# BharathMasetty/DPG-SLAM

Hardware: AMD Instinct MI355X
Metric: ICP edges/sec + ms/GN-iter on 5k-node/20k-edge synthetic graph, 1->8 GPU (higher is better)
Workload: dtype fp32 (ICP) + fp64 (GN)

## Files before the change

dpg-slam_amd/csrc/dpg_chol.h:

```cpp
#ifndef DPG_CHOL_H
#define DPG_CHOL_H

#include <stdint.h>

#include <vector>

struct dpg_chol_opts {
    int32_t max_supernode_cols = 64;
    double relax_fraction = 0.3;
    int32_t order = 0;
    int32_t merge_single = 0;
    int32_t fused = 1;
    int32_t solve_stage = -1;
    int32_t solve_maxseg = -1;
    int32_t solve_dinv = 0;
    int32_t solve_inv_cols = 0;
};

struct dpg_chol_sym {
    int64_t n = 0;
    int32_t ns = 0;
    int32_t n_levels = 0;
    int32_t max_front = 0;
    double flops = 0.0;
    std::vector<int32_t> perm, pos;
    std::vector<int32_t> sn_c0;
    std::vector<int32_t> sn_of;
    std::vector<int64_t> sn_rows_ptr;
    std::vector<int32_t> sn_rows;
    std::vector<int32_t> sn_parent;
    std::vector<int32_t> sn_level;
    std::vector<int32_t> level_ptr;
    std::vector<int32_t> level_list;
    std::vector<int64_t> child_ptr;
    std::vector<int32_t> child_list;
    std::vector<int32_t> relmap;
    std::vector<int64_t> front_off;
};

int dpg_chol_symbolic(int64_t n, const int32_t* pair_lo, const int32_t* pair_hi, int64_t n_pairs,
                      const dpg_chol_opts* opts, dpg_chol_sym* S);
int dpg_chol_order(int64_t n, const int32_t* pair_lo, const int32_t* pair_hi, int64_t n_pairs,
                   std::vector<int32_t>& perm, std::vector<std::vector<int32_t>>& pat, bool md = false);
int dpg_chol_order_nd(int64_t n, const int32_t* pair_lo, const int32_t* pair_hi, int64_t n_pairs, int32_t leaf,
                      std::vector<int32_t>& perm, std::vector<std::vector<int32_t>>& pat);
int dpg_chol_order_nd_sep(int64_t n, const int32_t* pair_lo, const int32_t* pair_hi, int64_t n_pairs, int32_t leaf,
                          int32_t starts, int32_t bal, int32_t score, bool cover, std::vector<int32_t>& perm,
                          std::vector<std::vector<int32_t>>& pat, bool par = false, int32_t refine = 0);
int dpg_chol_nd_refine(int64_t n, const int32_t* pair_lo, const int32_t* pair_hi, int64_t n_pairs, int32_t bal,
                       int32_t score, int32_t refine, std::vector<int32_t>& side);
int dpg_chol_sym_from_patterns(int64_t n, const std::vector<int32_t>& perm, const std::vector<std::vector<int32_t>>& pat,
                               const dpg_chol_opts* opts, dpg_chol_sym* S);
double dpg_chol_critical_path_us(const dpg_chol_sym& S);
int dpg_chol_sym_from_csr(int64_t n, const int32_t* perm, const int64_t* cp, const int32_t* prow,
                          const dpg_chol_opts* opts, dpg_chol_sym* S);

struct dpg_chol_incsym {
    int64_t n = 0, words = 0;
    std::vector<int32_t> perm, pos;
    std::vector<uint64_t> bits;
    int64_t swords = 0;
    std::vector<uint64_t> summ;
    std::vector<int32_t> parent;
    int64_t nnz = 0;
    std::vector<int64_t> cp;
    std::vector<int32_t> rows, rows_tmp;
    std::vector<std::pair<int32_t, int32_t>> added;
};
int dpg_incsym_reset(dpg_chol_incsym* I, int64_t n, const int32_t* pair_lo, const int32_t* pair_hi, int64_t n_pairs,
                     const dpg_chol_opts* opts = nullptr);
int dpg_incsym_order(int64_t n, const int32_t* pair_lo, const int32_t* pair_hi, int64_t n_pairs,
                     std::vector<int32_t>& perm, std::vector<std::vector<int32_t>>& pat,
                     const dpg_chol_opts* opts = nullptr, bool concurrent = false);
void dpg_incsym_init(dpg_chol_incsym* I, int64_t n, std::vector<int32_t>& perm, std::vector<std::vector<int32_t>>& pat);
void dpg_incsym_append(dpg_chol_incsym* I, int64_t k);
int64_t dpg_incsym_add_edge(dpg_chol_incsym* I, int32_t a, int32_t b);
int dpg_incsym_derive(dpg_chol_incsym* I, const dpg_chol_opts* opts, dpg_chol_sym* S);


int dpg_chol_create_sym(void** h, int64_t n, const int32_t* pair_lo, const int32_t* pair_hi, int64_t n_pairs,
                        dpg_chol_sym* S, const dpg_chol_opts* opts = nullptr);
int dpg_chol_create_sym_plan(void** h, int64_t n, const int32_t* pair_lo, const int32_t* pair_hi, int64_t n_pairs,
                             dpg_chol_sym* S, const dpg_chol_opts* opts = nullptr);
int dpg_chol_create_sym_upload(void** h);
int dpg_chol_plan_blocks(void** h, int64_t n, const int32_t* pos, const int32_t* perm, const int32_t* pair_lo,
                         const int32_t* pair_hi, int64_t n_pairs);
void dpg_chol_blocks_invalidate(void* h);
void dpg_chol_build_times(void* h, double out[2]);
int dpg_chol_fused(void* h);
int dpg_chol_plan_host(int64_t n, const int32_t* pair_lo, const int32_t* pair_hi, int64_t n_pairs,
                       const dpg_chol_sym* S, const dpg_chol_opts* opts, double* ms);

#endif
```

dpg-slam_amd/csrc/dpg_chol.hip:

```cpp
#include "dpg_chol_dev.h"

using namespace dpg_chol;

namespace {
void take_sym(CholDev* c, dpg_chol_sym* S) {
    c->has_factor = false;
    if (c->track && c->sym_is_fac) {
        std::swap(c->fac_sym, c->sym);
        c->fac_G.swap(c->plan.cur_G);
        c->sym_is_fac = false;
    }
    std::swap(c->sym, *S);
}

int chol_upload(CholDev* c) {
    const dpg_chol_sym& S = c->sym;
    const CholPlan& H = c->plan;
    const int64_t n = H.n;
    ++c->build_gen;
    c->has_factor = false;
    auto al = [](size_t b) { return (b + 255) & ~size_t(255); };
    struct Piece { void** d; const void* h; size_t bytes; };
    Piece pieces[24];
    int np = 0;
// ... 16 lines not shown
    add(&c->segs, H.segs);
    add(&c->dblocks, H.dblocks);
    add(&c->inv_tasks, H.inv_t);
    if (!H.fused) {
        add(&c->asm_tasks, H.asm_t);
        add(&c->asm_child, H.asm_c);
        add(&c->panel_tasks, H.panel_t);
        add(&c->upd_tasks, H.upd_t);
    }
    size_t total = 0;
    for (int i = 0; i < np; ++i) total += al(std::max<size_t>(pieces[i].bytes, 1));
    if (c->stage.reserve_amortised(total) || c->arena.reserve_amortised(total)) return DPG_ERR_HIP;
    size_t off = 0;
    for (int i = 0; i < np; ++i) {
        if (pieces[i].bytes) memcpy(c->stage.p + off, pieces[i].h, pieces[i].bytes);
        *pieces[i].d = c->arena.p + off;
        off += al(std::max<size_t>(pieces[i].bytes, 1));
    }
    int rc = hipMemcpyAsync(c->arena.p, c->stage.p, total, hipMemcpyHostToDevice, nullptr) != hipSuccess;
    const size_t cap0[3] = {c->fronts.cap, c->acc.cap, c->ysol.cap};
    rc |= c->sync.reserve_amortised(H.sync_bytes / sizeof(int32_t));
    rc |= c->fronts.reserve_amortised((size_t)S.front_off[(size_t)S.ns]);
    rc |= c->acc.reserve_amortised((size_t)H.acc_total);
    rc |= c->ysol.reserve_amortised((size_t)(3 * n));
    if (rc || cap0[0] != c->fronts.cap || cap0[1] != c->acc.cap || cap0[2] != c->ysol.cap) c->fac_valid = false;
    rc |= c->xsol.reserve_amortised((size_t)(3 * n));
    rc |= c->status.reserve_amortised(1);
    rc |= c->dinv.reserve_amortised((size_t)(3 * n) * kSB);
    rc |= c->linv.reserve_amortised((size_t)std::max<int64_t>(H.linv_total, 1));
    if (!rc) rc |= hipMemsetAsync(c->status.p, 0, sizeof(int32_t), nullptr) != hipSuccess;
    rc |= hipStreamSynchronize(nullptr) != hipSuccess;
    return rc ? DPG_ERR_HIP : DPG_OK;
}

int chol_build_plan(CholDev* c, int64_t n, const int32_t* pair_lo, const int32_t* pair_hi, int64_t n_pairs) {
    const double t_b0 = now_ms();
    const int rc = dpg_chol_plan_build(c->plan, c->sym, c->opts, c->track, n, pair_lo, pair_hi, n_pairs);
    c->t_build[0] = now_ms() - t_b0;
    return rc;
}
int chol_build_upload(CholDev* c) {
    const double t_b1 = now_ms();
    const int rc = chol_upload(c);
    c->t_build[1] = now_ms() - t_b1;
    return rc;
}
int chol_build(CholDev* c, int64_t n, const int32_t* pair_lo, const int32_t* pair_hi, int64_t n_pairs) {
    const int rc = chol_build_plan(c, n, pair_lo, pair_hi, n_pairs);
    return rc ? rc : chol_build_upload(c);
}

CholDev* chol_take(void** h, dpg_chol_sym* S, const dpg_chol_opts* opts) {
    CholDev* c = *h ? reinterpret_cast<CholDev*>(*h) : new CholDev();
    if (opts) c->opts = *opts;
    take_sym(c, S);
    return c;
}
int chol_built(void** h, CholDev* c, int rc) {
    if (rc) dpg_chol_destroy(c);
    *h = rc ? nullptr : c;
    return rc;
}
}

extern "C" void dpg_chol_destroy(void* h) {
    CholDev* c = reinterpret_cast<CholDev*>(h);
    if (!c) return;
    if (c->aux.s) (void)hipStreamSynchronize(c->aux.s);
    delete c;
}

extern "C" int dpg_chol_create(void** out, int64_t n, const int32_t* pair_lo, const int32_t* pair_hi,
                               int64_t n_pairs, const dpg_chol_opts* opts) {
    *out = nullptr;
    CholDev* c = new CholDev();
    if (opts) c->opts = *opts;
    if (dpg_chol_symbolic(n, pair_lo, pair_hi, n_pairs, &c->opts, &c->sym)) {
        delete c;
        return DPG_ERR_NUMERIC;
    }
    return chol_built(out, c, chol_build(c, n, pair_lo, pair_hi, n_pairs));
}

int dpg_chol_create_sym(void** h, int64_t n, const int32_t* pair_lo, const int32_t* pair_hi, int64_t n_pairs,
                        dpg_chol_sym* S, const dpg_chol_opts* opts) {
    CholDev* c = chol_take(h, S, opts);
    return chol_built(h, c, chol_build(c, n, pair_lo, pair_hi, n_pairs));
}

int dpg_chol_create_sym_plan(void** h, int64_t n, const int32_t* pair_lo, const int32_t* pair_hi, int64_t n_pairs,
                             dpg_chol_sym* S, const dpg_chol_opts* opts) {
    CholDev* c = chol_take(h, S, opts);
    return chol_built(h, c, chol_build_plan(c, n, pair_lo, pair_hi, n_pairs));
}
int dpg_chol_create_sym_upload(void** h) {
    CholDev* c = reinterpret_cast<CholDev*>(*h);
    return c ? chol_built(h, c, chol_build_upload(c)) : DPG_ERR_STATE;
}
int dpg_chol_plan_blocks(void** h, int64_t n, const int32_t* pos, const int32_t* perm, const int32_t* pair_lo,
                         const int32_t* pair_hi, int64_t n_pairs) {
    if (!h || n <= 0 || !pos || !perm || n_pairs < 0 || (n_pairs > 0 && (!pair_lo || !pair_hi))) return DPG_ERR_ARG;
    CholDev* c = *h ? reinterpret_cast<CholDev*>(*h) : new CholDev();
    *h = c;
    dpg_chol_plan_prebucket(c->plan, n, pos, perm, pair_lo, pair_hi, n_pairs);
    return DPG_OK;
}
void dpg_chol_blocks_invalidate(void* h) {
    if (h) reinterpret_cast<CholDev*>(h)->plan.blocks_ready = false;
}
int dpg_chol_fused(void* h) { return h && reinterpret_cast<const CholDev*>(h)->plan.fused ? 1 : 0; }

void dpg_chol_build_times(void* h, double out[2]) {
    const CholDev* c = reinterpret_cast<const CholDev*>(h);
    out[0] = c ? c->t_build[0] : 0.0;
    out[1] = c ? c->t_build[1] : 0.0;
}

static void note_factored(CholDev* c, int64_t refactored, int64_t kept, int64_t moved, int64_t pick_ns = 0) {
    c->pstats[0] = refactored;
    c->pstats[1] = kept;
    c->pstats[2] = moved;
    c->pstats[3] = pick_ns;
    c->has_factor = true;
    if (!c->track) return;
    c->fac_valid = true;
    c->fac_ptr = c->fronts.p;
    c->fac_ysol = c->ysol.p;
    c->fac_acc = c->acc.p;
    c->sym_is_fac = true;
    c->fac_db = c->plan.fused_db;
}

extern "C" int dpg_chol_solve(void* h, const double* hb, void* stream) {
    CholDev* c = reinterpret_cast<CholDev*>(h);
    const CholPlan& P = c->plan;
    note_factored(c, c->sym.ns, 0, 0);
    hipStream_t st = reinterpret_cast<hipStream_t>(stream);
    if (hipMemsetAsync(c->status.p, 0, sizeof(int32_t), st) != hipSuccess) return DPG_ERR_HIP;
    if (P.fused) {
        if (hipMemsetAsync(c->sync.p, 0, P.sync_bytes, st) != hipSuccess) return DPG_ERR_HIP;
        launch_factor(c, st, hb, nullptr, nullptr);
    } else {
        launch_levels(c, st, hb);
        if (hipMemsetAsync(c->sync.p, 0, P.sync_bytes, st) != hipSuccess) return DPG_ERR_HIP;
    }
    const double* di = launch_inv_diag(c, st);
    if (!P.fused) launch_forward(c, st, hb, di, nullptr, nullptr);
    launch_backward(c, st, di, nullptr, nullptr, nullptr, nullptr);
    c->inv_valid = c->keep_inv && P.n_inv_tasks > 0;
    if (c->inv_valid) launch_inv(c, st, nullptr);
    return hipGetLastError() == hipSuccess ? DPG_OK : DPG_ERR_HIP;
}

extern "C" void dpg_chol_track_factor(void* h, int on) {
    CholDev* c = reinterpret_cast<CholDev*>(h);
    if (!c || c->track == (on != 0)) return;
    c->track = on != 0;
    c->fac_valid = false;
    c->sym_is_fac = false;
    c->plan.cur_G.clear();
}
extern "C" void dpg_chol_forget_factor(void* h) {
    if (!h) return;
    reinterpret_cast<CholDev*>(h)->fac_valid = false;
    reinterpret_cast<CholDev*>(h)->has_factor = false;
}
extern "C" void dpg_chol_partial_stats(void* h, int64_t out[4]) {
    const CholDev* c = reinterpret_cast<const CholDev*>(h);
    for (int k = 0; k < 4; ++k) out[k] = c ? c->pstats[k] : 0;
}

extern "C" int dpg_chol_solve_partial(void* h, const double* hb, const int32_t* dirty_nodes, int64_t n_dirty,
                                      void* stream) {
    CholDev* c = reinterpret_cast<CholDev*>(h);
    const dpg_chol_sym& S = c->sym;
    const dpg_chol_sym& O = c->fac_sym;
    const CholPlan& P = c->plan;
    const bool usable = c->track && c->fac_valid && !c->sym_is_fac && c->fac_ptr == c->fronts.p &&
                        c->fac_ysol == c->ysol.p && c->fac_acc == c->acc.p && P.fused &&
                        !(P.use_dinv && P.n_dblocks > 0) && c->fac_db == P.fused_db && O.ns > 0 && O.n <= S.n &&
                        (int64_t)c->fac_G.size() == (int64_t)O.ns && (int64_t)P.cur_G.size() == (int64_t)S.ns &&
                        std::equal(O.perm.begin(), O.perm.end(), S.perm.begin());
    const double t_pick = now_ms();
    PartialPick& K = c->pick;
    if (!usable || !dpg_chol_plan_partial(K, S, O, P.cur_G, c->fac_G, dirty_nodes, n_dirty)) return dpg_chol_solve(h, hb, stream);
    const int32_t ns = S.ns;
    const int64_t nruns = (int64_t)K.runs.size() / 4;
    hipStream_t st = reinterpret_cast<hipStream_t>(stream);
    const size_t keep_bytes = ((size_t)ns + 15) & ~size_t(15);
    const size_t run_bytes = sizeof(int64_t) * 4 * (size_t)nruns;
    const size_t bytes = keep_bytes + 2 * run_bytes;
    if (c->pev_set && hipEventSynchronize(c->pev.e) != hipSuccess) return DPG_ERR_HIP;
    if (c->pstage.reserve_amortised(bytes) || c->dpart.reserve_amortised(bytes) ||
        (K.moved > 0 && c->scratch.reserve_amortised((size_t)K.moved)))
        return DPG_ERR_HIP;
    memcpy(c->pstage.p, K.keep.data(), (size_t)ns);
    int64_t* gat = reinterpret_cast<int64_t*>(c->pstage.p + keep_bytes);
    int64_t* sca = gat + 4 * nruns;
    for (int64_t r = 0, off = 0; r < nruns; ++r) {
        const int64_t* q = K.runs.data() + 4 * r;
        const int64_t g4[4] = {q[0], off, q[2], q[3]}, s4[4] = {off, q[1], q[2], q[3]};
        std::copy(g4, g4 + 4, gat + 4 * r);
        std::copy(s4, s4 + 4, sca + 4 * r);
        off += q[2];
    }
    if (c->pev.ensure(hipEventDisableTiming)) return DPG_ERR_HIP;
    if (hipMemcpyAsync(c->dpart.p, c->pstage.p, bytes, hipMemcpyHostToDevice, st) != hipSuccess ||
        hipEventRecord(c->pev.e, st) != hipSuccess)
        return DPG_ERR_HIP;
    c->pev_set = true;
    const uint8_t* keep_dev = reinterpret_cast<const uint8_t*>(c->dpart.p);
    const int64_t* gat_dev = reinterpret_cast<const int64_t*>(c->dpart.p + keep_bytes);
    launch_copy_runs(c, st, gat_dev, gat_dev + 4 * nruns, nruns, K.max_run);
    if (hipMemsetAsync(c->status.p, 0, sizeof(int32_t), st) != hipSuccess ||
        hipMemsetAsync(c->sync.p, 0, P.sync_bytes, st) != hipSuccess)
        return DPG_ERR_HIP;
    launch_factor(c, st, hb, nullptr, keep_dev);
    launch_backward(c, st, nullptr, nullptr, nullptr, nullptr, nullptr);
    note_factored(c, ns - K.kept, K.kept, K.moved, (int64_t)((now_ms() - t_pick) * 1e6));
    c->inv_valid = false;
    return hipGetLastError() == hipSuccess ? DPG_OK : DPG_ERR_HIP;
}

extern "C" int dpg_chol_resolve(void* h, const double* hb, void* stream) {
    CholDev* c = reinterpret_cast<CholDev*>(h);
    hipStream_t st = reinterpret_cast<hipStream_t>(stream);
    if (hipMemsetAsync(c->sync.p, 0, c->plan.sync_bytes, st) != hipSuccess) return DPG_ERR_HIP;
    const double* di = c->plan.use_dinv ? c->dinv.p : nullptr;
    const double* li = c->inv_valid ? c->linv.p : nullptr;
    launch_forward(c, st, hb, di, nullptr, li);
    launch_backward(c, st, di, nullptr, nullptr, nullptr, li);
    return hipGetLastError() == hipSuccess ? DPG_OK : DPG_ERR_HIP;
}

extern "C" int dpg_chol_gated_ok(void* h) {
    const CholDev* c = reinterpret_cast<const CholDev*>(h);
    return c && c->plan.fused && !(c->plan.use_dinv && c->plan.n_dblocks > 0) ? 1 : 0;
}

extern "C" void dpg_chol_sync_dev(void* h, int32_t** sync, int64_t* n_words) {
    CholDev* c = reinterpret_cast<CholDev*>(h);
    *sync = c->sync.p;
    *n_words = (int64_t)(c->plan.sync_bytes / sizeof(int32_t));
}

extern "C" int dpg_chol_solve_gated(void* h, const double* hb, const int32_t* gate, int prezeroed, double* X,
                                    double* max_out, void* stream) {
    CholDev* c = reinterpret_cast<CholDev*>(h);
    if (!dpg_chol_gated_ok(h)) return DPG_ERR_STATE;
    c->fac_valid = false;
    c->has_factor = true;
    hipStream_t st = reinterpret_cast<hipStream_t>(stream);
    if (!prezeroed && (hipMemsetAsync(c->status.p, 0, sizeof(int32_t), st) != hipSuccess ||
                       hipMemsetAsync(c->sync.p, 0, c->plan.sync_bytes, st) != hipSuccess))
        return DPG_ERR_HIP;
    const bool inv = c->plan.n_inv_tasks > 0;
    if (inv) {
        if (!c->aux.s) {
            if (hipStreamCreateWithFlags(&c->aux.s, hipStreamNonBlocking) != hipSuccess ||
                c->ev_fac.ensure(hipEventDisableTiming) || c->ev_inv[0].ensure(hipEventDisableTiming) ||
                c->ev_inv[1].ensure(hipEventDisableTiming) || hipEventRecord(c->ev_inv[0].e, c->aux.s) != hipSuccess ||
                hipEventRecord(c->ev_inv[1].e, c->aux.s) != hipSuccess)
                return DPG_ERR_HIP;
        }
        if (hipStreamWaitEvent(st, c->ev_inv[c->inv_par ^ 1].e, 0) != hipSuccess) return DPG_ERR_HIP;
    }
    launch_factor(c, st, hb, gate, nullptr);
    if (inv) {
        if (hipEventRecord(c->ev_fac.e, st) != hipSuccess || hipStreamWaitEvent(c->aux.s, c->ev_fac.e, 0) != hipSuccess)
            return DPG_ERR_HIP;
        launch_inv(c, c->aux.s, gate);
        if (hipEventRecord(c->ev_inv[c->inv_par].e, c->aux.s) != hipSuccess) return DPG_ERR_HIP;
        c->inv_par ^= 1;
    }
    launch_forward(c, st, hb, nullptr, gate, c->linv.p);
    launch_backward(c, st, nullptr, gate, X, max_out, c->linv.p);
    return hipGetLastError() == hipSuccess ? DPG_OK : DPG_ERR_HIP;
}

extern "C" void dpg_chol_keep_inverse(void* h, int on) {
    if (h) reinterpret_cast<CholDev*>(h)->keep_inv = on != 0;
}

extern "C" int dpg_chol_join_aux(void* h, void* stream) {
    CholDev* c = reinterpret_cast<CholDev*>(h);
    if (!c || !c->aux.s) return DPG_OK;
    return hipStreamWaitEvent(reinterpret_cast<hipStream_t>(stream), c->ev_inv[c->inv_par ^ 1].e, 0) == hipSuccess ? DPG_OK
                                                                                                       : DPG_ERR_HIP;
}

extern "C" const int32_t* dpg_chol_pos_dev(void* h) { return reinterpret_cast<CholDev*>(h)->pos; }
extern "C" const double* dpg_chol_x_dev(void* h) { return reinterpret_cast<CholDev*>(h)->xsol.p; }
extern "C" const int32_t* dpg_chol_status_dev(void* h) { return reinterpret_cast<CholDev*>(h)->status.p; }
extern "C" void dpg_chol_stats(void* h, double out[6]) {
    const dpg_chol_sym& S = reinterpret_cast<CholDev*>(h)->sym;
    out[0] = S.ns;
    out[1] = S.n_levels;
    out[2] = S.max_front;
    out[3] = S.flops;
    out[4] = (double)S.front_off[(size_t)S.ns] * 8.0;
    out[5] = (double)S.n;
}

#ifdef DPG_CHOL_TIMING
extern "C" void dpg_chol_tree(void* h, int32_t* parent, int32_t* m3, int32_t* k3) {
    const dpg_chol_sym& S = reinterpret_cast<CholDev*>(h)->sym;
    for (int32_t s = 0; s < S.ns; ++s) {
        parent[s] = S.sn_parent[(size_t)s];
        k3[s] = 3 * (S.sn_c0[(size_t)s + 1] - S.sn_c0[(size_t)s]);
        m3[s] = k3[s] + 3 * (int32_t)(S.sn_rows_ptr[(size_t)s + 1] - S.sn_rows_ptr[(size_t)s]);
    }
}
#endif
```

dpg-slam_amd/csrc/dpg_chol_factor.hip:

```cpp
#include "dpg_chol_dev.h"

using namespace dpg_chol;

#define FT_MARK(s, k) DPG_STAMP(threadIdx.x == 0 && (s) < 16384, g_front[(s) * 8 + (k)])
#define PN_MARK(s, p, k) DPG_STAMP(threadIdx.x == 0 && (s) < 16384 && (p) < 16, g_panel[((s) * 16 + (p)) * 8 + (k)])
#ifdef DPG_CHOL_TIMING
__device__ unsigned long long g_front[16384 * 8], g_panel[16384 * 16 * 8];
extern "C" int dpg_chol_front_dump(unsigned long long* out, int n) {
    return hipMemcpyFromSymbol(out, HIP_SYMBOL(g_front), sizeof(unsigned long long) * 8 * (size_t)n) == hipSuccess ? 0 : -1;
}
extern "C" int dpg_chol_panel_dump(unsigned long long* out, int n) {
    return hipMemcpyFromSymbol(out, HIP_SYMBOL(g_panel), sizeof(unsigned long long) * 16 * 8 * (size_t)n) == hipSuccess ? 0 : -1;
}
#endif

namespace {
constexpr int kPF = (kSmall * (kSmall + 1) / 2 + kFT - 1) / kFT;
constexpr int kPFL = 4;

__device__ __forceinline__ void tri_ij(int e, int n, int& i, int& j) {
    const float b = 2.0f * (float)n + 1.0f;
    int jj = (int)((b - sqrtf(b * b - 8.0f * (float)e)) * 0.5f);
    jj = max(0, min(jj, n - 1));
    while (jj > 0 && jj * n - jj * (jj - 1) / 2 > e) --jj;
    while (jj + 1 < n && (jj + 1) * n - (jj + 1) * jj / 2 <= e) ++jj;
    j = jj;
    i = jj + e - (jj * n - jj * (jj - 1) / 2);
}

__device__ __forceinline__ void small_front(int s, const SnDev& S, int32_t* sync, int32_t* status, const SnDev* __restrict__ sns,
                            const OEnt* __restrict__ omap, const int32_t* __restrict__ relmap,
                            const int32_t* __restrict__ child_list, const double* __restrict__ hb,
                            const double* __restrict__ g, const int32_t* __restrict__ perm, double* fronts,
                            double* __restrict__ ysol, double* acc, double* sm) {
    const int tid = threadIdx.x;
    const int k3 = 3 * S.k, r3 = 3 * S.r, m3 = k3 + r3;
    double* F = fronts + S.front_off;
    double* A = sm;
    double* bv = A + m3 * m3;
    ChMeta* chm = reinterpret_cast<ChMeta*>(bv + m3);
    int32_t* crm = reinterpret_cast<int32_t*>(chm + kMaxCh);
    const int nch = S.nchild;
    for (int e = tid; e < m3 * m3; e += kFT) A[e] = 0.0;
    for (int t = tid; t < m3; t += kFT) bv[t] = t < k3 ? -g[3 * perm[S.c0 + t / 3] + t % 3] : 0.0;
    if (tid < nch) {
        const SnDev C = sns[child_list[S.child_off + tid]];
        chm[tid] = ChMeta{C.front_off, C.acc_off, C.rows_off, C.k, C.r};
        for (int q = 0; q < C.r; ++q) crm[tid * (kSmall / 3) + q] = relmap[C.rows_off + q];
    }
    __syncthreads();
    for (int q = tid; q < S.omap_n * 9; q += kFT) {
        const OEnt o = omap[S.omap_off + q / 9];
        const int ii = (q % 9) / 3, jj = q % 3;
        const int row = 3 * o.a + ii, col = 3 * o.b + jj;
        if (row < col) continue;
        const double* B = hb + 9 * (int64_t)o.u;
        A[col * m3 + row] = o.tr ? B[3 * jj + ii] : B[3 * ii + jj];
    }
    if (nch > 0) {
        if (tid == 0) wait_geq_sc1(sync + s, S.need, status);
        asm volatile("s_waitcnt vmcnt(0)" ::: "memory");
    }
    __syncthreads();
    FT_MARK(s, 1);
    auto load_child = [&](int ci, double (&v)[kPF], double& va) {
        const ChMeta C = chm[ci];
        const int n = 3 * C.r, tri = n * (n + 1) / 2, m3c = 3 * (C.k + C.r), k3c = 3 * C.k;
        double* Fc = fronts + C.front_off + (int64_t)k3c * m3c + k3c;
#pragma unroll
        for (int q = 0; q < kPF; ++q) {
            const int e = tid + kFT * q;
            v[q] = 0.0;
            if (e < tri) {
                int i, j;
                tri_ij(e, n, i, j);
                v[q] = ld_agent(Fc + (int64_t)j * m3c + i);
            }
        }
        va = tid < n ? ld_agent(acc + C.acc_off + tid) : 0.0;
    };
    auto add_child = [&](int ci, const double (&v)[kPF], double va) {
        const ChMeta C = chm[ci];
        const int n = 3 * C.r, tri = n * (n + 1) / 2;
        const int32_t* rm = crm + ci * (kSmall / 3);
#pragma unroll
        for (int q = 0; q < kPF; ++q) {
            const int e = tid + kFT * q;
            if (e < tri) {
                int i, j;
                tri_ij(e, n, i, j);
                const int pj = 3 * rm[j / 3] + j % 3, pi = 3 * rm[i / 3] + i % 3;
                A[pj * m3 + pi] += v[q];
            }
        }
        if (tid < n) bv[3 * rm[tid / 3] + tid % 3] -= va;
    };
    if (nch > 0) {
        double va_[kPF], vb_[kPF], aa = 0.0, ab = 0.0;
        load_child(0, va_, aa);
        for (int ci = 0; ci < nch; ci += 2) {
            if (ci + 1 < nch) load_child(ci + 1, vb_, ab);
            add_child(ci, va_, aa);
            __syncthreads();
            if (ci + 1 < nch) {
                if (ci + 2 < nch) load_child(ci + 2, va_, aa);
                add_child(ci + 1, vb_, ab);
                __syncthreads();
            }
        }
    }
    FT_MARK(s, 2);
    bool bad = false;
    for (int c0 = 0; c0 < k3; c0 += 3) {
        const double* C0 = A + c0 * m3;
        const double* C1 = C0 + m3;
        const double* C2 = C1 + m3;
        double d00 = C0[c0], d10 = C0[c0 + 1], d20 = C0[c0 + 2], d11 = C1[c0 + 1], d21 = C1[c0 + 2], d22 = C2[c0 + 2];
        if (!(d00 > 0.0)) { bad = true; d00 = 1.0; }
        const double i00 = rsqrt_nr(d00), l00 = d00 * i00;
        const double l10 = d10 * i00, l20 = d20 * i00;
        double e11 = d11 - l10 * l10;
        if (!(e11 > 0.0)) { bad = true; e11 = 1.0; }
        const double i11 = rsqrt_nr(e11), l11 = e11 * i11;
        const double l21 = (d21 - l20 * l10) * i11;
        double e22 = d22 - l20 * l20 - l21 * l21;
        if (!(e22 > 0.0)) { bad = true; e22 = 1.0; }
        const double i22 = rsqrt_nr(e22), l22 = e22 * i22;
        const double y0 = bv[c0] * i00;
        const double y1 = (bv[c0 + 1] - l10 * y0) * i11;
        const double y2 = (bv[c0 + 2] - l20 * y0 - l21 * y1) * i22;
        for (int i = c0 + 3 + tid; i < m3; i += kFT) {
            const double x0 = C0[i] * i00;
            const double x1 = (C1[i] - x0 * l10) * i11;
            const double x2 = (C2[i] - x0 * l20 - x1 * l21) * i22;
            A[c0 * m3 + i] = x0;
            A[(c0 + 1) * m3 + i] = x1;
            A[(c0 + 2) * m3 + i] = x2;
            bv[i] -= x0 * y0 + x1 * y1 + x2 * y2;
        }
        __syncthreads();
        if (tid == 0) {
            A[c0 * m3 + c0] = l00; A[c0 * m3 + c0 + 1] = l10; A[c0 * m3 + c0 + 2] = l20;
            A[(c0 + 1) * m3 + c0 + 1] = l11; A[(c0 + 1) * m3 + c0 + 2] = l21; A[(c0 + 2) * m3 + c0 + 2] = l22;
            bv[c0] = y0; bv[c0 + 1] = y1; bv[c0 + 2] = y2;
        }
        const int b0 = c0 + 3, nr = m3 - b0;
        for (int e = tid; e < nr * nr; e += kFT) {
            const int l = b0 + e / nr, i = b0 + e % nr;
            if (i < l) continue;
            double v = A[l * m3 + i];
            v = fma(-C0[i], C0[l], v);
            v = fma(-C1[i], C1[l], v);
            v = fma(-C2[i], C2[l], v);
            A[l * m3 + i] = v;
        }
        __syncthreads();
    }
    if (bad && tid == 0) atomicExch(status, 1);
    FT_MARK(s, 3);
    for (int e = tid; e < k3 * m3; e += kFT) {
        const int j = e / m3, i = e - j * m3;
        if (i >= j) F[(int64_t)j * m3 + i] = A[e];
    }
    for (int t = tid; t < k3; t += kFT) ysol[3 * (int64_t)S.c0 + t] = bv[t];
    if (S.parent >= 0) {
        const auto rs = front_rsrc(F, m3);
        const int npc = (r3 + 2) >> 1;
        for (int e = tid; e < r3 * npc; e += kFT) {
            const int jj = e / npc, k = e - jj * npc, j = k3 + jj;
            const uint32_t a = (uint32_t)(j * m3 + k3);
            const int i0 = 2 * k - (int)(a & 1u);
            if (i0 + 1 < jj || i0 >= r3) continue;
            const double* Aj = A + j * m3 + k3;
            st2_sc1(rs, (a & ~1u) + 2u * k, i0 >= jj ? Aj[i0] : 0.0, i0 + 1 < r3 ? Aj[i0 + 1] : 0.0);
        }
        for (int t = tid; t < r3; t += kFT) st_agent(acc + S.acc_off + t, -bv[k3 + t]);
    }
    asm volatile("s_waitcnt vmcnt(0)" ::: "memory");
    __syncthreads();
    FT_MARK(s, 4);
    if (tid == 0 && S.parent >= 0)
        __hip_atomic_fetch_add(sync + S.parent, 1, __ATOMIC_RELAXED, __HIP_MEMORY_SCOPE_AGENT);
}

struct Tiles {
    int k3, m3, np, nt;
    __device__ int c0(int t) const { return t < np ? kFNB * t : k3 + kFNB * (t - np); }
    __device__ int c1(int t) const { return t < np ? min(kFNB * t + kFNB, k3) : min(k3 + kFNB * (t - np + 1), m3); }
};

struct PanelFrame {
    int m3, j0, w, R, off, Rp, npc;
    __device__ __forceinline__ PanelFrame(const Tiles& T, int q)
        : m3(T.m3), j0(kFNB * q), w(min(kFNB, T.k3 - j0)), R(T.m3 - j0), off((4 - (w & 3)) & 3), Rp(fused_rp(R, off)),
          npc((R + 2) >> 1) {}
    struct Pair { int c, i0; uint32_t addr; };
    __device__ __forceinline__ Pair pair(int e) const {
        const int c = e / npc, k = e - c * npc;
        const uint32_t a = (uint32_t)((j0 + c) * m3 + j0);
        return Pair{c, 2 * k - (int)(a & 1u), (a & ~1u) + 2u * k};
    }
};

__device__ void factor_lds(int q, int s, const Tiles& T, double* P, double* scr, bool& bad) {
    const int tid = threadIdx.x, lane = tid & 63, wave = __builtin_amdgcn_readfirstlane(tid >> 6);
    const PanelFrame f(T, q);
    const int w = f.w, R = f.R, off = f.off, Rp = f.Rp;
    double* Lt = scr;
    double* rdg = Lt + kFNB * kFNB;
    int* flg = reinterpret_cast<int*>(rdg + 8 * (kFNB / 3));
    PN_MARK(s, q, 5);
    {
        const int i = lane, cv = 3 * wave, ep = q + 1;
        if (cv < w) {
            double col[3];
#pragma unroll
            for (int r = 0; r < 3; ++r) {
                const int c = cv + r;
                col[r] = (i < w && i >= c) ? P[c * Rp + off + i] : 0.0;
            }
            for (int st = 0; st < wave; ++st) {
                while (__builtin_amdgcn_readfirstlane(__hip_atomic_load(flg + st, __ATOMIC_RELAXED, __HIP_MEMORY_SCOPE_WORKGROUP)) < ep)
                    __builtin_amdgcn_s_sleep(0);
                __builtin_amdgcn_fence(__ATOMIC_ACQUIRE, "workgroup");
                const int c0 = 3 * st;
                const int ii = i < kFNB ? i : 0;
                const double x0 = Lt[c0 * kFNB + ii], x1 = Lt[(c0 + 1) * kFNB + ii], x2 = Lt[(c0 + 2) * kFNB + ii];
#pragma unroll
                for (int r = 0; r < 3; ++r) {
                    const int c = cv + r;
                    const double y0 = Lt[c0 * kFNB + c], y1 = Lt[(c0 + 1) * kFNB + c], y2 = Lt[(c0 + 2) * kFNB + c];
                    const double v = fma(-x2, y2, fma(-x1, y1, fma(-x0, y0, col[r])));
                    col[r] = (i >= c && i < w) ? v : col[r];
                }
            }
            const double d00 = rdlane(col[0], cv), d10 = rdlane(col[0], cv + 1), d20 = rdlane(col[0], cv + 2);
            const double d11 = rdlane(col[1], cv + 1), d21 = rdlane(col[1], cv + 2), d22 = rdlane(col[2], cv + 2);
            const Chol3 L = chol3(d00, d10, d11, d20, d21, d22, bad);
            double x0 = col[0] * L.m00;
            double x1 = fma(col[0], L.m10, col[1] * L.m11);
            double x2 = fma(col[0], L.m20, fma(col[1], L.m21, col[2] * L.m22));
            if (i == cv) { x0 = L.l00; x1 = 0.0; x2 = 0.0; }
            else if (i == cv + 1) { x0 = L.l10; x1 = L.l11; x2 = 0.0; }
            else if (i == cv + 2) { x0 = L.l20; x1 = L.l21; x2 = L.l22; }
            if (i < kFNB) {
                Lt[cv * kFNB + i] = (i >= cv && i < w) ? x0 : 0.0;
                Lt[(cv + 1) * kFNB + i] = (i >= cv + 1 && i < w) ? x1 : 0.0;
                Lt[(cv + 2) * kFNB + i] = (i >= cv + 2 && i < w) ? x2 : 0.0;
            }
            if (i == 0) {
                double* mi = rdg + 2 * cv;
                mi[0] = L.m00; mi[1] = L.m10; mi[2] = L.m11; mi[3] = L.m20; mi[4] = L.m21; mi[5] = L.m22;
            }
            __builtin_amdgcn_fence(__ATOMIC_RELEASE, "workgroup");
            if (i == 0) __hip_atomic_store(flg + wave, ep, __ATOMIC_RELAXED, __HIP_MEMORY_SCOPE_WORKGROUP);
        } else if (cv < kFNB) {
            for (int r = 0; r < 3; ++r)
                if (i < kFNB) Lt[(cv + r) * kFNB + i] = 0.0;
        }
    }
    __syncthreads();
    PN_MARK(s, q, 6);
    for (int i = w + tid; i < R; i += kFT) {
        double a[kFNB];
#pragma unroll
        for (int c = 0; c < kFNB; ++c) a[c] = c < w ? P[c * Rp + off + i] : 0.0;
#pragma unroll
        for (int b = 0; b < kFNB; b += 3) {
            if (b < w) {
                const double* mi = rdg + 2 * b;
                const double x0 = a[b] * mi[0];
                const double x1 = fma(a[b], mi[1], a[b + 1] * mi[2]);
                const double x2 = fma(a[b], mi[3], fma(a[b + 1], mi[4], a[b + 2] * mi[5]));
                a[b] = x0; a[b + 1] = x1; a[b + 2] = x2;
#pragma unroll
                for (int cc = b + 3; cc < kFNB; ++cc)
                    a[cc] = fma(-x2, Lt[(b + 2) * kFNB + cc], fma(-x1, Lt[(b + 1) * kFNB + cc], fma(-x0, Lt[b * kFNB + cc], a[cc])));
            }
        }
#pragma unroll
        for (int c = 0; c < kFNB; ++c)
            if (c < w) P[c * Rp + off + i] = a[c];
    }
    __syncthreads();
    PN_MARK(s, q, 7);
    for (int e = tid; e < w * w; e += kFT) {
        const int c = e / w, r = e - c * w;
        if (r >= c) P[c * Rp + off + r] = Lt[c * kFNB + r];
    }
    __syncthreads();
    PN_MARK(s, q, 3);
}

__device__ void publish_panel(int q, int s, const Tiles& T, double* F, const double* P, int32_t* pflag) {
    const int tid = threadIdx.x;
    const PanelFrame f(T, q);
    const int R = f.R;
    const auto rs = front_rsrc(F, T.m3);
    for (int e = tid; e < f.w * f.npc; e += kFT) {
        const PanelFrame::Pair pr = f.pair(e);
        const int c = pr.c, i0 = pr.i0;
        if (i0 + 1 < c || i0 >= R) continue;
        const double* pc = P + c * f.Rp + f.off;
        st2_sc1(rs, pr.addr, i0 >= c ? pc[i0] : 0.0, i0 + 1 < R ? pc[i0 + 1] : 0.0);
    }
    asm volatile("s_waitcnt vmcnt(0)" ::: "memory");
    __syncthreads();
    if (tid == 0) __hip_atomic_store(pflag + s, q + 1, __ATOMIC_RELAXED, __HIP_MEMORY_SCOPE_AGENT);
    PN_MARK(s, q, 4);
}

template <bool SC1>
__device__ void load_panel(int p, const Tiles& T, double* F, double* P) {
    const int tid = threadIdx.x;
    const PanelFrame f(T, p);
    const int j0 = f.j0, w = f.w, R = f.R, off = f.off, Rp = f.Rp;
    if (SC1) {
        const auto rs = front_rsrc(F, T.m3);
        const int tot = w * f.npc;
        constexpr int kB2 = 8;
        for (int e0 = 0; e0 < tot; e0 += kFT * kB2) {
            double2 v[kB2];
#pragma unroll
            for (int q = 0; q < kB2; ++q) {
                const int e = e0 + tid + kFT * q;
                const PanelFrame::Pair pr = f.pair(e);
                v[q] = make_double2(0.0, 0.0);
                if (e < tot && pr.i0 < R && pr.i0 + 1 >= pr.c) v[q] = ld2_sc1(rs, pr.addr);
            }
#pragma unroll
            for (int q = 0; q < kB2; ++q) {
                const int e = e0 + tid + kFT * q;
                const PanelFrame::Pair pr = f.pair(e);
                const int c = pr.c, i0 = pr.i0;
                if (e < tot) {
                    double* pc = P + c * Rp + off;
                    if (i0 >= 0 && i0 < R) pc[i0] = i0 >= c ? v[q].x : 0.0;
                    if (i0 + 1 < R) pc[i0 + 1] = i0 + 1 >= c ? v[q].y : 0.0;
                }
            }
        }
        return;
    }
    constexpr int kB = 16;
    for (int e0 = 0; e0 < w * R; e0 += kFT * kB) {
        double v[kB];
#pragma unroll
        for (int q = 0; q < kB; ++q) {
            const int e = e0 + tid + kFT * q;
            const int c = e / R, i = e - c * R;
            double* a = F + (uint32_t)((j0 + c) * T.m3 + j0 + i);
            v[q] = (e < w * R && i >= c) ? (SC1 ? ld_agent(a) : *a) : 0.0;
        }
#pragma unroll
        for (int q = 0; q < kB; ++q) {
            const int e = e0 + tid + kFT * q;
            const int c = e / R, i = e - c * R;
            if (e < w * R) P[c * Rp + off + i] = v[q];
        }
    }
}

template <bool WT, bool SC1 = false>
__device__ void update_tile(int t, int p, const Tiles& T, double* F, const double* P) {
    const int tid = threadIdx.x;
    const PanelFrame f(T, p);
    const int m3 = f.m3, j0 = f.j0, w = f.w, R = f.R, off = f.off, Rp = f.Rp;
    const int l0 = T.c0(t) - j0, l1 = T.c1(t) - j0;
    const int g0 = ((l0 + off) & ~3) - off;
    const int ncg = (l1 - g0 + 3) >> 2, nrg = (R - g0 + 3) >> 2;
    for (int q = tid; q < nrg * ncg; q += kFT) {
        const int ib = g0 + 4 * (q % nrg), lb = g0 + 4 * (q / nrg);
        if (ib + 3 < lb) continue;
        double ac[4][4];
#pragma unroll
        for (int a = 0; a < 4; ++a)
#pragma unroll
            for (int b = 0; b < 4; ++b) ac[a][b] = 0.0;
#pragma unroll 1
        for (int c = 0; c < w; ++c) {
            const double2* pc = reinterpret_cast<const double2*>(P + c * Rp);
            const double2 i01 = pc[(off + ib) >> 1], i23 = pc[((off + ib) >> 1) + 1];
            const double2 l01 = pc[(off + lb) >> 1], l23 = pc[((off + lb) >> 1) + 1];
            const double vi[4] = {i01.x, i01.y, i23.x, i23.y};
            const double vl[4] = {l01.x, l01.y, l23.x, l23.y};
#pragma unroll
            for (int a = 0; a < 4; ++a)
#pragma unroll
                for (int b = 0; b < 4; ++b) ac[a][b] = fma(vi[a], vl[b], ac[a][b]);
        }
#pragma unroll
        for (int b = 0; b < 4; ++b) {
            const uint32_t o = (uint32_t)((j0 + min(max(lb + b, l0), l1 - 1)) * m3 + j0);
#pragma unroll
            for (int a = 0; a < 4; ++a) {
                double* src = F + o + (uint32_t)min(ib + a, R - 1);
                ac[a][b] = (SC1 ? ld_agent(src) : *src) - ac[a][b];
            }
        }
#pragma unroll
        for (int b = 0; b < 4; ++b) {
            const int l = lb + b;
            const uint32_t o = (uint32_t)((j0 + l) * m3 + j0);
#pragma unroll
            for (int a = 0; a < 4; ++a) {
                const int i = ib + a;
                if (l >= l0 && l < l1 && i < R && i >= l) {
                    if (WT) st_agent(F + o + (uint32_t)i, ac[a][b]);
                    else F[o + (uint32_t)i] = ac[a][b];
                }
            }
        }
    }
}

__device__ void update_next_lds(int p, const Tiles& T, const double* Pc, double* Pn) {
    const int tid = threadIdx.x;
    const int j0 = kFNB * p, R = T.m3 - j0, Rp = fused_rp(R, 0);
    const int j1 = j0 + kFNB, w1 = min(kFNB, T.k3 - j1), R1 = R - kFNB;
    const int off1 = (4 - (w1 & 3)) & 3, Rp1 = fused_rp(R1, off1);
    const int ncg = (w1 + 3) >> 2, nrg = (R1 + 3) >> 2;
    for (int q = tid; q < nrg * ncg; q += kFT) {
        const int ib = 4 * (q % nrg), lb = 4 * (q / nrg);
        if (ib + 3 < lb) continue;
        double ac[4][4];
#pragma unroll
        for (int a = 0; a < 4; ++a)
#pragma unroll
            for (int b = 0; b < 4; ++b) ac[a][b] = 0.0;
#pragma unroll 2
        for (int c = 0; c < kFNB; ++c) {
            const double2* pc = reinterpret_cast<const double2*>(Pc + c * Rp + kFNB);
            const double2 i01 = pc[ib >> 1], i23 = pc[(ib >> 1) + 1];
            const double2 l01 = pc[lb >> 1], l23 = pc[(lb >> 1) + 1];
            const double vi[4] = {i01.x, i01.y, i23.x, i23.y};
            const double vl[4] = {l01.x, l01.y, l23.x, l23.y};
#pragma unroll
            for (int a = 0; a < 4; ++a)
#pragma unroll
                for (int b = 0; b < 4; ++b) ac[a][b] = fma(vi[a], vl[b], ac[a][b]);
        }
#pragma unroll
        for (int b = 0; b < 4; ++b) {
            const int l = lb + b;
#pragma unroll
            for (int a = 0; a < 4; ++a) {
                const int i = ib + a;
                if (l < w1 && i < R1 && i >= l) Pn[l * Rp1 + off1 + i] -= ac[a][b];
            }
        }
    }
}

__device__ void rhs_panel(int p, const Tiles& T, const double* P, double* bv) {
    const int tid = threadIdx.x, lane = tid & 63, wave = tid >> 6;
    const PanelFrame f(T, p);
    const int j0 = f.j0, w = f.w, R = f.R, off = f.off, Rp = f.Rp;
    if (wave == 0) {
        double bl = lane < w ? bv[j0 + lane] : 0.0;
        for (int c = 0; c < w; ++c) {
            const double yc = __shfl(bl, c, 64) / P[c * Rp + off + c];
            if (lane == c) bl = yc;
            else if (lane > c && lane < w) bl = fma(-P[c * Rp + off + lane], yc, bl);
        }
        if (lane < w) bv[j0 + lane] = bl;
    }
    __syncthreads();
    for (int i = w + tid; i < R; i += kFT) {
        double sacc = 0.0;
        for (int c = 0; c < w; ++c) sacc = fma(P[c * Rp + off + i], bv[j0 + c], sacc);
        bv[j0 + i] -= sacc;
    }
    __syncthreads();
}

__device__ __forceinline__ int tile_owner(int t, int G) { return t == 0 || G == 1 ? 0 : 1 + (t - 1) % (G - 1); }

__device__ __forceinline__ void large_front(int s, int mem, const SnDev& S, int32_t* sync, int32_t* pflag,
                            int32_t* tready, int32_t* status,
                            const SnDev* __restrict__ sns, const OEnt* __restrict__ omap,
                            const int32_t* __restrict__ relmap, const int32_t* __restrict__ child_list,
                            const FTask* __restrict__ ftasks, const FChild* __restrict__ fchild,
                            const double* __restrict__ hb, const double* __restrict__ g,
                            const int32_t* __restrict__ perm, double* fronts, double* __restrict__ ysol,
                            double* acc, double* sm, int db) {
    const int tid = threadIdx.x;
    const int k3 = 3 * S.k, r3 = 3 * S.r, m3 = k3 + r3, G = S.G;
    double* F = fronts + S.front_off;
    Tiles T{k3, m3, (k3 + kFNB - 1) / kFNB, 0};
    T.nt = T.np + (r3 + kFNB - 1) / kFNB;
    int32_t* trdy = tready + S.ftask;
    const bool has_b = mem == tile_owner(T.nt - 1, G);
    const int t_first = mem, t_step = mem == 0 ? T.nt : G - 1;
    double* bv = sm;
    double* scr = bv + ((m3 + 1) & ~1);
    double* PA = scr + kFScr;
    double* PB = db ? PA + (size_t)kFNB * fused_rp(m3, 3) : PA;
    if (has_b)
        for (int t = tid; t < m3; t += kFT) bv[t] = t < k3 ? -g[3 * perm[S.c0 + t / 3] + t % 3] : 0.0;
    bool waited = S.need == 0;
    for (int t = t_first; t < T.nt; t += t_step) {
        const FTask tk = ftasks[S.ftask + t];
        const int cs = T.c0(t), nc = T.c1(t) - cs;
        double* Tl = PA;
        for (int e = tid; e < nc * m3; e += kFT) Tl[e] = 0.0;
        __syncthreads();
        for (int q = tid; q < (tk.om_e - tk.om_b) * 9; q += kFT) {
            const OEnt o = omap[tk.om_b + q / 9];
            const int ii = (q % 9) / 3, jj = q % 3;
            const int row = 3 * o.a + ii, col = 3 * o.b + jj;
            if (col < cs || col >= cs + nc || row < col) continue;
            const double* B = hb + 9 * (int64_t)o.u;
            Tl[(col - cs) * m3 + row] = o.tr ? B[3 * jj + ii] : B[3 * ii + jj];
        }
        if (!waited) {
            if (tid == 0) wait_geq_sc1(sync + s, S.need, status);
            asm volatile("s_waitcnt vmcnt(0)" ::: "memory");
            waited = true;
            FT_MARK(s, 1);
        }
        for (int cq = 0; cq < tk.ch_cnt; ++cq) {
            __syncthreads();
            const FChild C = fchild[tk.ch_off + cq];
            const int n = 3 * C.r, m3c = 3 * (C.k + C.r), k3c = 3 * C.k, nj = C.jb - C.ja;
            const auto rs = front_rsrc(fronts + C.front_off, m3c);
            const int32_t* rm = relmap + C.rows_off;
            const int npc = (n + 2) >> 1, tot = nj * npc;
            for (int e0 = 0; e0 < tot; e0 += kFT * kPFL) {
                double2 v[kPFL];
                int d0[kPFL], d1[kPFL];
#pragma unroll
                for (int q = 0; q < kPFL; ++q) {
                    const int e = e0 + tid + kFT * q;
                    const int jj = e / npc, k = e - jj * npc, j = C.ja + jj;
                    const uint32_t a = (uint32_t)((k3c + j) * m3c + k3c);
                    const int i0 = 2 * k - (int)(a & 1u);
                    d0[q] = -1;
                    d1[q] = -1;
                    v[q] = make_double2(0.0, 0.0);
                    if (e < tot && i0 + 1 >= j && i0 < n) {
                        v[q] = ld2_sc1(rs, (a & ~1u) + 2u * k);
                        const int cj = (3 * rm[j / 3] + j % 3 - cs) * m3;
                        if (i0 >= j) d0[q] = cj + 3 * rm[i0 / 3] + i0 % 3;
                        if (i0 + 1 < n) d1[q] = cj + 3 * rm[(i0 + 1) / 3] + (i0 + 1) % 3;
                    }
                }
#pragma unroll
                for (int q = 0; q < kPFL; ++q) {
                    if (d0[q] >= 0) Tl[d0[q]] += v[q].x;
                    if (d1[q] >= 0) Tl[d1[q]] += v[q].y;
                }
            }
        }
        __syncthreads();
        if (t == 0 && mem == 0 && db) {
            const int off = (4 - (nc & 3)) & 3, Rp = fused_rp(m3, off);
            for (int e = tid; e < nc * m3; e += kFT) {
                const int c = e / m3, i = e - c * m3;
                PB[c * Rp + off + i] = i >= c ? Tl[e] : 0.0;
            }
            __syncthreads();
            continue;
        }
        const bool handoff = t == 1 && mem != 0;
        for (int e = tid; e < nc * m3; e += kFT) {
            const int col = cs + e / m3, row = e % m3;
            if (row >= col) {
                if (handoff) st_agent(F + (uint32_t)(col * m3 + row), Tl[e]);
                else F[(uint32_t)(col * m3 + row)] = Tl[e];
            }
        }
        if (handoff) asm volatile("s_waitcnt vmcnt(0)" ::: "memory");
        __syncthreads();
        if (handoff && tid == 0) __hip_atomic_store(trdy + 1, 1, __ATOMIC_RELAXED, __HIP_MEMORY_SCOPE_AGENT);
    }
    if (!waited) {
        if (tid == 0) wait_geq_sc1(sync + s, S.need, status);
        asm volatile("s_waitcnt vmcnt(0)" ::: "memory");
        __syncthreads();
    }
    if (has_b) {
        for (int ci = 0; ci < S.nchild; ++ci) {
            const SnDev C = sns[child_list[S.child_off + ci]];
            const int32_t* rm = relmap + C.rows_off;
            for (int t = tid; t < 3 * C.r; t += kFT) bv[3 * rm[t / 3] + t % 3] -= ld_agent(acc + C.acc_off + t);
            __syncthreads();
        }
    }
    FT_MARK(s, 2);

    bool bad = false;
    if (mem == 0) {
        double* cur = db ? PB : PA;
        if (tid < kFNB / 3) reinterpret_cast<int*>(scr + kFNB * kFNB + 8 * (kFNB / 3))[tid] = 0;
        if (!db) load_panel<false>(0, T, F, cur);
        __syncthreads();
        factor_lds(0, s, T, cur, scr, bad);
        publish_panel(0, s, T, F, cur, pflag);
        for (int p = 0; p < T.np; ++p) {
            double* nxt = cur == PA ? PB : PA;
            if (has_b && !db) rhs_panel(p, T, cur, bv);
            if (p + 1 < T.np) {
                const int t = p + 1;
                PN_MARK(s, t, 0);
                if (tile_owner(t, G) != 0) {
                    if (tid == 0) wait_geq_sc1(trdy + t, 1, status);
                    asm volatile("s_waitcnt vmcnt(0)" ::: "memory");
                    __syncthreads();
                }
                if (db) {
                    load_panel<true>(t, T, F, nxt);
                    __syncthreads();
                    PN_MARK(s, t, 1);
                    update_next_lds(p, T, cur, nxt);
                } else {
                    PN_MARK(s, t, 1);
                    update_tile<true, true>(t, p, T, F, cur);
                    asm volatile("s_waitcnt vmcnt(0)" ::: "memory");
                    __syncthreads();
                    load_panel<true>(t, T, F, nxt);
                }
                __syncthreads();
                PN_MARK(s, t, 2);
                factor_lds(t, s, T, nxt, scr, bad);
                publish_panel(t, s, T, F, nxt, pflag);
            }
            if (has_b && db) rhs_panel(p, T, cur, bv);
            cur = nxt;
        }
    } else {
        double* P = PA;
        for (int p = 0; p < T.np; ++p) {
            bool need = false;
            for (int t = t_first; t < T.nt; t += t_step) need |= t > p && !(t == p + 1 && t < T.np);
            if (!need && !has_b) break;
            if (tid == 0) wait_geq_sc1(pflag + s, p + 1, status);
            asm volatile("s_waitcnt vmcnt(0)" ::: "memory");
            __syncthreads();
            load_panel<true>(p, T, F, P);
            __syncthreads();
            const int tc = p + 2;
            const bool mine = tc < T.np && tile_owner(tc, G) == mem;
            if (mine) {
                update_tile<true>(tc, p, T, F, P);
                asm volatile("s_waitcnt vmcnt(0)" ::: "memory");
                __syncthreads();
                if (tid == 0) __hip_atomic_store(trdy + tc, 1, __ATOMIC_RELAXED, __HIP_MEMORY_SCOPE_AGENT);
            }
            const bool fin = p == T.np - 1 && S.parent >= 0;
            for (int t = t_first; t < T.nt; t += t_step)
                if (t > p && !(t == p + 1 && t < T.np) && !(mine && t == tc)) {
                    if (fin) update_tile<true>(t, p, T, F, P);
                    else update_tile<false>(t, p, T, F, P);
                }
            __syncthreads();
            if (has_b) rhs_panel(p, T, P, bv);
        }
    }
    if (bad && (tid & 63) == 0) atomicExch(status, 1);
    if (has_b) {
        for (int t = tid; t < k3; t += kFT) ysol[3 * (int64_t)S.c0 + t] = bv[t];
        if (S.parent >= 0)
            for (int t = tid; t < r3; t += kFT) st_agent(acc + S.acc_off + t, -bv[k3 + t]);
    }
    FT_MARK(s, 3);
    asm volatile("s_waitcnt vmcnt(0)" ::: "memory");
    __syncthreads();
    if (mem == 0) FT_MARK(s, 4);
    if (tid == 0 && S.parent >= 0)
        __hip_atomic_fetch_add(sync + S.parent, 1, __ATOMIC_RELAXED, __HIP_MEMORY_SCOPE_AGENT);
}

__global__ __launch_bounds__(kFT, 2) void chol_factor_dag(const int32_t* __restrict__ order, int32_t* sync,
                                                       int32_t* status, const SnDev* __restrict__ sns,
                                                       const OEnt* __restrict__ omap,
                                                       const int32_t* __restrict__ relmap,
                                                       const int32_t* __restrict__ child_list,
                                                       const FTask* __restrict__ ftasks,
                                                       const FChild* __restrict__ fchild,
                                                       const double* __restrict__ hb, const double* __restrict__ g,
                                                       const int32_t* __restrict__ perm, double* fronts,
                                                       double* __restrict__ ysol, double* acc, int ns, int db,
                                                       const int32_t* gate, const uint8_t* __restrict__ keep) {
    extern __shared__ __attribute__((aligned(16))) double smem_f[];
    double* sm = smem_f + 2;
    if (gate_off(gate, 1)) return;
    __builtin_amdgcn_s_setprio(2);
    const int code = claim_lds(order, sync, reinterpret_cast<int*>(smem_f));
    const int s = code >> 6, mem = code & 63;
    const SnDev S = sns[s];
    if (keep && keep[s]) {
        if (threadIdx.x == 0 && S.parent >= 0)
            __hip_atomic_fetch_add(sync + 1 + S.parent, 1, __ATOMIC_RELAXED, __HIP_MEMORY_SCOPE_AGENT);
        return;
    }
    if (mem == 0) FT_MARK(s, 0);
    if (S.G == 1 && 3 * (S.k + S.r) <= kSmall && S.nchild <= kMaxCh)
        small_front(s, S, sync + 1, status, sns, omap, relmap, child_list, hb, g, perm, fronts, ysol, acc, sm);
    else
        large_front(s, mem, S, sync + 1, sync + 1 + ns, sync + 2 + 3 * ns, status, sns, omap, relmap, child_list,
                    ftasks, fchild, hb, g, perm, fronts, ysol, acc, sm, db);
}

__global__ __launch_bounds__(256) void chol_copy_runs(const double* __restrict__ src0, const double* __restrict__ src1,
                                                      double* __restrict__ dst0, double* __restrict__ dst1,
                                                      const int64_t* __restrict__ runs) {
    const int64_t* r = runs + 4 * blockIdx.y;
    const int64_t s0 = r[0], d0 = r[1], n = r[2];
    const double* src = r[3] ? src1 : src0;
    double* dst = r[3] ? dst1 : dst0;
    for (int64_t i = (int64_t)blockIdx.x * blockDim.x + threadIdx.x; i < n; i += (int64_t)gridDim.x * blockDim.x)
        dst[d0 + i] = src[s0 + i];
}

}

void dpg_chol::launch_factor(CholDev* c, hipStream_t st, const double* hb, const int32_t* gate, const uint8_t* keep) {
    const CholPlan& P = c->plan;
    hipLaunchKernelGGL(chol_factor_dag, dim3((unsigned)P.n_tickets), dim3(kFT), P.lds_fused, st, c->order_fac, sync_forward(c),
                       c->status.p, c->sns, c->omap, c->relmap, c->child_list, c->ftasks, c->fchild, hb, hb + 9 * P.nnzb_upper,
                       c->perm, c->fronts.p, c->ysol.p, c->acc.p, c->sym.ns, P.fused_db ? 1 : 0, gate, keep);
}

void dpg_chol::launch_copy_runs(CholDev* c, hipStream_t st, const int64_t* gather, const int64_t* scatter, int64_t nruns,
                                int64_t max_run) {
    if (nruns == 0) return;
    const dim3 grid((unsigned)std::min<int64_t>(64, std::max<int64_t>(1, (max_run + 2047) / 2048)), (unsigned)nruns);
    hipLaunchKernelGGL(chol_copy_runs, grid, dim3(256), 0, st, c->fronts.p, c->acc.p, c->scratch.p, c->scratch.p, gather);
    hipLaunchKernelGGL(chol_copy_runs, grid, dim3(256), 0, st, c->scratch.p, c->scratch.p, c->fronts.p, c->acc.p, scatter);
}
```

dpg-slam_amd/csrc/dpg_ctx.hip:

```cpp

#include <stdarg.h>
#include <stdio.h>
#include <string.h>

#include <string>

#include "dpg_ctx.h"

namespace {
thread_local std::string g_err;
}

int fail(int code, const char* fmt, ...) {
    char buf[512];
    va_list ap;
    va_start(ap, fmt);
    vsnprintf(buf, sizeof(buf), fmt, ap);
    va_end(ap);
    g_err = buf;
    return code;
}

dpg_ctx* g_default_ctx = nullptr;

static dpg_ctx* no_ctx(int) { return nullptr; }

extern "C" {

const char* dpg_last_error(void) { return g_err.c_str(); }

int dpg_set_error(int code, const char* msg) { return fail(code, "%s", msg); }
const char* dpg_version(void) { return "dpg-mi355x 0.1 (gfx950)"; }

int dpg_shard_plan(const float* cost, int64_t ne, int32_t world, int32_t* owner, int64_t* dispatch, int64_t* counts) {
    if (ne < 0 || world < 1 || (ne > 0 && (!owner || !dispatch)) || !counts) return fail(DPG_ERR_ARG, "dpg_shard_plan: bad arguments");
    std::vector<std::vector<int64_t>> disp((size_t)world);
    if (cost) {
        std::vector<int64_t> ord((size_t)ne);
        for (int64_t e = 0; e < ne; ++e) ord[(size_t)e] = e;
        std::stable_sort(ord.begin(), ord.end(), [&](int64_t a, int64_t b) { return cost[a] > cost[b]; });
        std::vector<double> load((size_t)world, 0.0);
        for (int64_t e : ord) {
            int r = 0;
            for (int q = 1; q < world; ++q)
                if (load[(size_t)q] < load[(size_t)r]) r = q;
            owner[e] = r;
            load[(size_t)r] += cost[e];
            disp[(size_t)r].push_back(e);
        }
    } else {
        for (int64_t e = 0; e < ne; ++e) {
            owner[e] = (int32_t)(e % world);
            disp[(size_t)(e % world)].push_back(e);
        }
    }
    int64_t o = 0;
    for (int r = 0; r < world; ++r) {
        counts[r] = (int64_t)disp[(size_t)r].size();
        for (int64_t e : disp[(size_t)r]) dispatch[o++] = e;
    }
    return DPG_OK;
}

int dpg_shard_reassemble(const int32_t* owner, int64_t ne, int32_t world, int64_t slice, int64_t rec_bytes,
                         const void* gathered, void* out) {
    if (ne < 0 || world < 1 || slice < 0 || rec_bytes <= 0 || (ne > 0 && (!owner || !gathered || !out)))
        return fail(DPG_ERR_ARG, "dpg_shard_reassemble: bad arguments");
    std::vector<int64_t> pos((size_t)world, 0);
    const char* g = static_cast<const char*>(gathered);
    char* o = static_cast<char*>(out);
    for (int64_t e = 0; e < ne; ++e) {
        const int32_t r = owner[e];
        if (r < 0 || r >= world || pos[(size_t)r] >= slice) return fail(DPG_ERR_ARG, "dpg_shard_reassemble: edge %lld owner %d out of range", (long long)e, r);
        memcpy(o + e * rec_bytes, g + (r * slice + pos[(size_t)r]++) * rec_bytes, (size_t)rec_bytes);
    }
    return DPG_OK;
}

dpg_ctx* dpg_ctx_create(int device) {
    int n = 0;
    if (hipGetDeviceCount(&n) != hipSuccess || n <= 0) return no_ctx(fail(DPG_ERR_HIP, "no HIP device available"));
    if (device < 0 || device >= n) return no_ctx(fail(DPG_ERR_ARG, "device %d out of range (%d devices)", device, n));
    if (hipSetDevice(device) != hipSuccess) return no_ctx(fail(DPG_ERR_HIP, "hipSetDevice(%d) failed", device));
    dpg_ctx* c = new dpg_ctx();
    c->device = device;
    if (hipStreamCreateWithFlags(&c->own.s, hipStreamNonBlocking) != hipSuccess) {
        delete c;
        return no_ctx(fail(DPG_ERR_HIP, "hipStreamCreate failed"));
    }
    c->stream = c->own.s;
    if (hipStreamCreateWithFlags(&c->aux.s, hipStreamNonBlocking) != hipSuccess) c->aux.s = nullptr;
    for (auto& e : c->ev) (void)e.ensure(hipEventDefault);
    dpg_gn_params_default(&c->gp);
    return c;
}

dpg_ctx* dpg_ctx_create_multi(int32_t n_gpus, const int32_t* devices) {
    int n = 0;
    if (hipGetDeviceCount(&n) != hipSuccess || n <= 0) return no_ctx(fail(DPG_ERR_HIP, "no HIP device available"));
    if (n_gpus < 1 || n_gpus > n)
        return no_ctx(fail(DPG_ERR_ARG, "dpg_ctx_create_multi: %d GPUs asked, %d present", n_gpus, n));
    std::vector<int> dl((size_t)n_gpus);
    for (int k = 0; k < n_gpus; ++k) {
        dl[(size_t)k] = devices ? devices[k] : k;
        for (int j = 0; j < k; ++j)
            if (dl[(size_t)j] == dl[(size_t)k])
                return no_ctx(fail(DPG_ERR_ARG, "dpg_ctx_create_multi: device %d listed twice", dl[(size_t)k]));
    }
    dpg_ctx* c = dpg_ctx_create(dl[0]);
    if (!c) return nullptr;
    for (int k = 1; k < n_gpus; ++k) {
        dpg_ctx* q = dpg_ctx_create(dl[(size_t)k]);
        if (!q) {
            dpg_ctx_destroy(c);
            return nullptr;
        }
        q->rank = k;
        c->peers.push_back(q);
    }
    c->comms.assign((size_t)n_gpus, nullptr);
    const ncclResult_t r = ncclCommInitAll(c->comms.data(), n_gpus, dl.data());
    if (r != ncclSuccess) {
        c->comms.clear();
        dpg_ctx_destroy(c);
        return no_ctx(fail(DPG_ERR_HIP, "ncclCommInitAll over %d devices failed: %s", n_gpus, ncclGetErrorString(r)));
    }
    c->coll = kCollRccl;
    c->world = n_gpus;
    (void)hipSetDevice(c->device);
    return c;
}

dpg_ctx* dpg_ctx_create_virtual(int32_t k, int32_t device) {
    if (k < 1 || k > kMaxVirtual)
        return no_ctx(fail(DPG_ERR_ARG, "dpg_ctx_create_virtual: %d virtual devices (1 .. %d)", k, kMaxVirtual));
    dpg_ctx* c = dpg_ctx_create(device);
    if (!c) return nullptr;
    for (int r = 1; r < k; ++r) {
        dpg_ctx* q = dpg_ctx_create(device);
        if (!q) {
            dpg_ctx_destroy(c);
            return nullptr;
        }
        q->own.release();
        q->stream = c->stream;
        q->rank = r;
        c->peers.push_back(q);
    }
    c->coll = kCollVirtual;
    c->world = k;
    return c;
}

int dpg_nccl_unique_id(void* id_out) {
    if (!id_out) return fail(DPG_ERR_ARG, "dpg_nccl_unique_id: NULL");
    static_assert(sizeof(ncclUniqueId) == DPG_NCCL_ID_BYTES, "ncclUniqueId size");
    ncclUniqueId id;
    const ncclResult_t r = ncclGetUniqueId(&id);
    if (r != ncclSuccess) return fail(DPG_ERR_HIP, "ncclGetUniqueId failed: %s", ncclGetErrorString(r));
    memcpy(id_out, &id, sizeof(id));
    return DPG_OK;
}

dpg_ctx* dpg_ctx_create_rank(int32_t device, const void* nccl_id, int32_t rank, int32_t world) {
    if (!nccl_id || world < 1 || rank < 0 || rank >= world)
        return no_ctx(fail(DPG_ERR_ARG, "dpg_ctx_create_rank: rank %d of %d", rank, world));
    dpg_ctx* c = dpg_ctx_create(device);
    if (!c) return nullptr;
    ncclUniqueId id;
    memcpy(&id, nccl_id, sizeof(id));
    ncclComm_t comm = nullptr;
    const ncclResult_t r = ncclCommInitRank(&comm, world, id, rank);
    if (r != ncclSuccess) {
        dpg_ctx_destroy(c);
        return no_ctx(fail(DPG_ERR_HIP, "ncclCommInitRank(rank %d of %d) failed: %s", rank, world, ncclGetErrorString(r)));
    }
    c->comms.assign(1, comm);
    c->coll = kCollRccl;
    c->world = world;
    c->rank0 = rank;
    c->rank = rank;
    return c;
}

dpg_ctx* dpg_ctx_create_rank_ops(int32_t device, const dpg_coll_ops* ops, int32_t rank, int32_t world) {
    if (!ops || !ops->allreduce_sum_f64 || !ops->allreduce_sum_f32 || !ops->allgather || world < 1 || rank < 0 ||
        rank >= world)
        return no_ctx(fail(DPG_ERR_ARG, "dpg_ctx_create_rank_ops: rank %d of %d (all three collectives are required)", rank, world));
    dpg_ctx* c = dpg_ctx_create(device);
    if (!c) return nullptr;
    c->host_ops = *ops;
    c->coll = kCollHost;
    c->world = world;
    c->rank0 = rank;
    c->rank = rank;
    return c;
}

int32_t dpg_ctx_num_gpus(dpg_ctx* c) { return c ? n_dev(c) : -1; }
int32_t dpg_ctx_rank(dpg_ctx* c) { return c ? c->rank0 : -1; }

int32_t dpg_ctx_num_ranks(dpg_ctx* c) {
    if (!c) return -1;
    if (c->coll == kCollRccl) {
        int n = -1;
        if (ncclCommCount(c->comms[0], &n) != ncclSuccess) return fail(DPG_ERR_HIP, "ncclCommCount failed");
        return n;
    }
    return c->world;
}

void dpg_solver_options_default(dpg_solver_options* o) {
    if (!o) return;
    const dpg_chol_opts d;
    memset(o, 0, sizeof(*o));
    o->order = d.order;
    o->fused = d.fused;
    o->solve_stage = d.solve_stage;
    o->solve_maxseg = d.solve_maxseg;
    o->solve_dinv = d.solve_dinv;
    o->merge_single = d.merge_single;
    o->max_supernode_cols = d.max_supernode_cols;
    o->relax_fraction = d.relax_fraction;
    o->solve_inv_cols = d.solve_inv_cols;
}

int dpg_ctx_set_solver_options(dpg_ctx* c, const dpg_solver_options* o) {
    if (!c || !o || o->order < DPG_ORDER_AUTO || o->order > DPG_ORDER_ND || o->max_supernode_cols < 1 || o->solve_inv_cols < 0 ||
        !(o->relax_fraction >= 0.0))
        return fail(DPG_ERR_ARG, "bad solver options");
    for (int k = 0; k < n_dev(c); ++k) {
        dpg_chol_opts& d = dev_ctx(c, k)->copts;
        d.order = o->order;
        d.fused = o->fused ? 1 : 0;
        d.solve_stage = o->solve_stage;
        d.solve_maxseg = o->solve_maxseg;
        d.solve_dinv = o->solve_dinv ? 1 : 0;
        d.merge_single = o->merge_single ? 1 : 0;
        d.max_supernode_cols = o->max_supernode_cols;
        d.relax_fraction = o->relax_fraction;
        d.solve_inv_cols = o->solve_inv_cols;
    }
    return DPG_OK;
}

int dpg_ctx_set_icp_schedule(dpg_ctx* c, int32_t schedule) {
    if (!c || (schedule != DPG_ICP_SCHEDULE_CALLER && schedule != DPG_ICP_SCHEDULE_MEASURED))
        return fail(DPG_ERR_ARG, "bad ICP schedule");
    c->schedule = schedule;
    return DPG_OK;
}

int dpg_ctx_set_icp_variant(dpg_ctx* c, int32_t variant) {
    if (!c || (variant != DPG_ICP_ANGULAR && variant != DPG_ICP_KDTREE && variant != DPG_ICP_GRID))
        return fail(DPG_ERR_ARG, "bad ICP variant");
    for (int k = 0; k < n_dev(c); ++k) {
        if (dev_ctx(c, k)->icp_variant != variant) dev_ctx(c, k)->idx_valid = 0;
        dev_ctx(c, k)->icp_variant = variant;
    }
    return DPG_OK;
}

int dpg_ctx_set_icp_defer_cap(dpg_ctx* c, int32_t cap) {
    if (!c || cap < 0) return fail(DPG_ERR_ARG, "bad defer cap");
    for (int k = 0; k < n_dev(c); ++k) dev_ctx(c, k)->defer_cap = cap;
    return DPG_OK;
}

int dpg_ctx_set_cov_workgroups(dpg_ctx* c, int32_t n) {
    if (!c || n < 0) return fail(DPG_ERR_ARG, "bad covariance workgroup count");
    for (int k = 0; k < n_dev(c); ++k) dev_ctx(c, k)->cov_wg = n;
    return DPG_OK;
}

int dpg_ctx_set_icp_kernel_variant(dpg_ctx* c, int32_t v) {
    if (!c || v < 0) return fail(DPG_ERR_ARG, "bad kernel variant");
    for (int k = 0; k < n_dev(c); ++k) {
        if ((dev_ctx(c, k)->kernel_variant == 2) != (v == 2)) dev_ctx(c, k)->idx_valid = 0;
        dev_ctx(c, k)->kernel_variant = v;
    }
    return DPG_OK;
}

void dpg_ctx_adopt(dpg_ctx* c, void* child, void (*destroy)(void*)) {
    if (c && child) c->children.emplace_back(child, destroy);
}
void dpg_ctx_release_child(dpg_ctx* c, void* child) {
    if (!c) return;
    for (size_t k = 0; k < c->children.size(); ++k)
        if (c->children[k].first == child) {
            c->children.erase(c->children.begin() + (std::ptrdiff_t)k);
            return;
        }
}

void dpg_ctx_destroy(dpg_ctx* c) {
    if (!c) return;
    while (!c->children.empty()) {
        const auto ch = c->children.back();
        ch.second(ch.first);
        if (!c->children.empty() && c->children.back().first == ch.first) c->children.pop_back();
    }
    if (c->coll == kCollVirtual) (void)hipStreamSynchronize(c->stream);
    for (dpg_ctx* q : c->peers) dpg_ctx_destroy(q);
    c->peers.clear();
    for (ncclComm_t m : c->comms)
        if (m) (void)ncclCommDestroy(m);
    c->comms.clear();
    (void)hipSetDevice(c->device);
    (void)join_cov(c);
    (void)hipStreamSynchronize(c->stream);
    c->hc.reset();
    if (c == g_default_ctx) g_default_ctx = nullptr;
    delete c;
}

int dpg_ctx_set_stream(dpg_ctx* c, void* s) {
    if (!c) return fail(DPG_ERR_ARG, "ctx is NULL");
    if (join_cov(c)) return fail(DPG_ERR_HIP, "stream wait failed");
    HIP_TRY(hipStreamSynchronize(c->stream));
    c->own.release();
    c->stream = reinterpret_cast<hipStream_t>(s);
    if (c->coll == kCollVirtual)
        for (dpg_ctx* q : c->peers) q->stream = c->stream;
    return DPG_OK;
}

int dpg_ctx_synchronize(dpg_ctx* c) {
    if (!c) return fail(DPG_ERR_ARG, "ctx is NULL");
    for (int k = 0; k < n_dev(c); ++k) {
        HIP_TRY(hipSetDevice(dev_ctx(c, k)->device));
        if (join_cov(dev_ctx(c, k))) return fail(DPG_ERR_HIP, "stream wait failed");
        HIP_TRY(hipStreamSynchronize(dev_ctx(c, k)->stream));
    }
    HIP_TRY(hipSetDevice(c->device));
    return DPG_OK;
}

}
```

dpg-slam_amd/csrc/dpg_gn_api.hip:

```cpp

#include <string.h>

#include <chrono>
#include <cmath>

#include "dpg_ctx.h"

static int gn_setup_1(dpg_ctx* c, int64_t V, const dpg_factor* F, int64_t nf, int64_t b, int64_t e,
                      const dpg_gn_params* gp) {
    HIP_TRY(hipSetDevice(c->device));
    GnGraph ng;
    int rc = ng.build(V, F, nf, b, e, &c->copts, c->stream);
    if (rc) return fail(rc, "pose-graph setup failed (invalid factor or out of memory)");
    c->gn = std::move(ng);
    c->gn_ready = true;
    c->gn_pairs_valid = false;
    c->gp = or_default(gp, dpg_gn_params_default);
    return DPG_OK;
}

static int gn_set_poses_1(dpg_ctx* c, const double* poses) {
    if (!c->gn_ready) return fail(DPG_ERR_STATE, "graph not set up");
    HIP_TRY(hipSetDevice(c->device));
    HIP_TRY(hipMemcpyAsync(c->gn.v.poses, poses, sizeof(double) * 3 * (size_t)c->gn.v.n_nodes, hipMemcpyHostToDevice,
// ... 391 lines not shown
                break;
            }
            cur = nw;
        }
    }
    if (multi && (rc = dpg_ctx_synchronize(c))) return rc;
    if (poses && (rc = dpg_gn_get_poses(c, poses))) return rc;
    if (!poses) {
        HIP_TRY(hipSetDevice(c->device));
        HIP_TRY(hipStreamSynchronize(c->stream));
    }
    const double t2 = now_ms();
    S.iterations = it;
    S.final_error = nw;
    S.last_delta_inf = dinf;
    S.ms_total = t2 - t0;
    S.ms_per_iteration = it ? (t2 - t1) / it : 0.0;
    if (st) *st = S;
    return DPG_OK;
}

static int gn_marginals_state(dpg_ctx* c, const char* fn) {
    if (!c || !c->gn_ready) return fail(DPG_ERR_STATE, "%s: graph not set up", fn);
    if (is_multi(c)) return fail(DPG_ERR_STATE, "%s: marginals are single-device (this context has several ranks)", fn);
    if (c->gp.linear_solver != DPG_SOLVER_CHOLESKY || !c->gn.v.chol)
        return fail(DPG_ERR_STATE, "%s: the graph has no Cholesky factorization (linear_solver)", fn);
    return DPG_OK;
}

static int gn_factor_at_current_poses(dpg_ctx* c, const char* fn, bool timed) {
    HIP_TRY(hipSetDevice(c->device));
    dpg_gn_dev* g = &c->gn.v;
    int rc;
    if (timed) HIP_TRY(hipEventRecord(c->ev[3].e, c->stream));
    if ((rc = dpg_gn_dev_assemble(g, g->hb_own, c->stream))) return fail(rc, "%s: assembly launch failed", fn);
    if (timed) HIP_TRY(hipEventRecord(c->ev[4].e, c->stream));
    if ((rc = dpg_chol_solve(g->chol, g->hb_own, c->stream))) return fail(rc, "%s: factorization launch failed", fn);
    if (timed) HIP_TRY(hipEventRecord(c->ev[5].e, c->stream));
    return DPG_OK;
}

static int gn_marginals_blocks(dpg_ctx* c, const char* fn, const int32_t* nodes, int64_t n, const int32_t* pairs,
                               int64_t n_pairs, double* out, double* ms) {
    int rc = gn_marginals_state(c, fn);
    if (rc) return rc;
    if (!out || n < 0 || n_pairs < 0) return fail(DPG_ERR_ARG, "%s: bad arguments", fn);
    if (dpg_chol_selinv_check(c->gn.v.chol, nodes, n, pairs, n_pairs))
        return fail(DPG_ERR_ARG, "%s: a node is out of range or a pair's block is outside the factor's pattern", fn);
    if ((rc = gn_factor_at_current_poses(c, fn, ms != nullptr))) return rc;
    rc = dpg_chol_marginals(c->gn.v.chol, nodes, n, pairs, n_pairs, out, c->stream);
    if (rc == DPG_ERR_NUMERIC) return fail(rc, "%s: H is not positive definite", fn);
    if (rc) return fail(rc, "%s: selected inversion failed", fn);
    if (ms) {
        float a = 0.f, f = 0.f;
        HIP_TRY(hipEventElapsedTime(&a, c->ev[3].e, c->ev[4].e));
        HIP_TRY(hipEventElapsedTime(&f, c->ev[4].e, c->ev[5].e));
        ms[0] = a;
        ms[1] = f;
    }
    return DPG_OK;
}

static int gn_pairs_share_factor(dpg_ctx* c, const int32_t* pairs, int64_t n) {
    const dpg_gn_dev& g = c->gn.v;
    if (!c->gn_pairs_valid) {
        HIP_TRY(hipSetDevice(c->device));
        std::vector<dpg_factor> F((size_t)g.n_factors);
        if (g.n_factors > 0) {
            HIP_TRY(hipMemcpyAsync(F.data(), g.factors, sizeof(dpg_factor) * F.size(), hipMemcpyDeviceToHost, c->stream));
            HIP_TRY(hipStreamSynchronize(c->stream));
        }
        c->gn_pairs.clear();
        for (const dpg_factor& f : F)
            if (f.kind == DPG_FACTOR_BETWEEN && f.i != f.j)
                c->gn_pairs.push_back((uint64_t)(uint32_t)std::min(f.i, f.j) << 32 | (uint32_t)std::max(f.i, f.j));
        std::sort(c->gn_pairs.begin(), c->gn_pairs.end());
        c->gn_pairs.erase(std::unique(c->gn_pairs.begin(), c->gn_pairs.end()), c->gn_pairs.end());
        c->gn_pairs_valid = true;
    }
    for (int64_t q = 0; q < n; ++q) {
        const int32_t i = pairs[2 * q], j = pairs[2 * q + 1];
        if (i < 0 || j < 0 || i >= g.n_nodes || j >= g.n_nodes)
            return fail(DPG_ERR_ARG, "dpg_gn_marginal_pairs: pair %lld has a node out of range", (long long)q);
        if (i != j && !std::binary_search(c->gn_pairs.begin(), c->gn_pairs.end(),
                                          (uint64_t)(uint32_t)std::min(i, j) << 32 | (uint32_t)std::max(i, j)))
            return fail(DPG_ERR_ARG, "dpg_gn_marginal_pairs: nodes %d and %d share no factor", i, j);
    }
    return DPG_OK;
}

static int gn_joint_blocks(dpg_ctx* c, const char* fn, int by_nodes, const int32_t* idx, int64_t n, double* out, float* ms) {
    int rc = gn_marginals_state(c, fn);
    if (rc) return rc;
    if (n < 0 || (n > 0 && (!idx || !out))) return fail(DPG_ERR_ARG, "%s: bad arguments", fn);
    for (int64_t q = 0, e = by_nodes ? n : 2 * n; q < e; ++q)
        if (idx[q] < 0 || idx[q] >= c->gn.v.n_nodes) return fail(DPG_ERR_ARG, "%s: node %d is out of range", fn, idx[q]);
    if (n == 0) return DPG_OK;
    if ((rc = gn_factor_at_current_poses(c, fn, false))) return rc;
    rc = dpg_chol_joint(c->gn.v.chol, by_nodes, idx, n, out, c->stream, ms);
    if (rc == DPG_ERR_NUMERIC) return fail(rc, "%s: H is not positive definite", fn);
    if (rc) return fail(rc, "%s: the path solve failed", fn);
    return DPG_OK;
}

extern "C" {

int dpg_gn_setup(dpg_ctx* c, int64_t V, const dpg_factor* F, int64_t nf, int64_t b, int64_t e,
                 const dpg_gn_params* gp) {
    if (!c || !F || V <= 0 || nf < 0) return fail(DPG_ERR_ARG, "dpg_gn_setup: bad arguments");
    if (!is_multi(c)) return gn_setup_1(c, V, F, nf, b, e, gp);
    if (b != 0 || e != nf) return fail(DPG_ERR_ARG, "dpg_gn_setup: a multi-device context shards the factors itself (0, n_factors)");
    for (int k = 0; k < n_dev(c); ++k) {
        dpg_ctx* q = dev_ctx(c, k);
        int rc = gn_setup_1(q, V, F, nf, 0, nf, gp);
        if (!rc && (rc = dpg_gn_dev_set_ownership(&q->gn, c->world, q->rank, q->stream)))
            rc = fail(rc, "pose-graph ownership setup failed");
        if (rc) return rc;
    }
    HIP_TRY(hipSetDevice(c->device));
    return DPG_OK;
}

int dpg_gn_take_icp_measurements(dpg_ctx* c, int64_t first, int64_t count, int64_t n_always,
                                 const dpg_icp_params* p) {
    if (!c || !c->gn_ready || !p) return fail(DPG_ERR_STATE, "graph not set up");
    const double ix = 1.0 / (double)p->laser_x_variance, iy = 1.0 / (double)p->laser_y_variance,
                 ith = 1.0 / (double)p->laser_theta_variance;
    if (!is_multi(c)) {
        if (count > c->n_edges) return fail(DPG_ERR_ARG, "only %lld ICP results available", (long long)c->n_edges);
        int rc = dpg_gn_dev_icp_to_factors(&c->gn.v, c->res.p, first, count, n_always, ix, iy, ith, c->stream);
        return rc ? fail(rc, "dpg_gn_take_icp_measurements failed") : DPG_OK;
    }
    if (count != (int64_t)c->batch.size())
        return fail(DPG_ERR_ARG, "a multi-device context takes the whole batch (%lld results), not %lld",
                    (long long)c->batch.size(), (long long)count);
    for (int k = 0; k < n_dev(c); ++k) {
        dpg_ctx* q = dev_ctx(c, k);
        HIP_TRY(hipSetDevice(q->device));
        if (!q->gn_ready || !q->gn.v.mine) return fail(DPG_ERR_STATE, "graph not set up on device %d", k);
        const int64_t nl = (int64_t)c->shard[(size_t)k].size();
        const int rc = dpg_gn_dev_icp_to_factors_scatter(&q->gn.v, q->res.p, q->shard_idx.p, nl, first, count, n_always,
                                                         ix, iy, ith, q->stream);
        if (rc) return fail(rc, "dpg_gn_take_icp_measurements failed");
    }
    HIP_TRY(hipSetDevice(c->device));
    return DPG_OK;
}

int64_t dpg_gn_hb_size(dpg_ctx* c) { return (c && c->gn_ready) ? dpg_gn_dev_hb_size(&c->gn.v) : -1; }

int dpg_gn_setup_profile(dpg_ctx* c, double out[5]) {
    if (!c || !c->gn_ready || !out) return fail(DPG_ERR_STATE, "graph not set up");
    for (int k = 0; k < 5; ++k) out[k] = c->gn.v.setup_ms[k];
    return DPG_OK;
}

int dpg_gn_set_poses(dpg_ctx* c, const double* poses) {
    if (!c || !c->gn_ready || !poses) return fail(DPG_ERR_STATE, "graph not set up");
    for (int k = 0; k < n_dev(c); ++k) {
        const int rc = gn_set_poses_1(dev_ctx(c, k), poses);
        if (rc) return rc;
    }
    HIP_TRY(hipSetDevice(c->device));
    return DPG_OK;
}

int dpg_gn_get_poses(dpg_ctx* c, double* poses) {
    if (!c || !c->gn_ready || !poses) return fail(DPG_ERR_STATE, "graph not set up");
    HIP_TRY(hipSetDevice(c->device));
    HIP_TRY(hipMemcpyAsync(poses, c->gn.v.poses, sizeof(double) * 3 * (size_t)c->gn.v.n_nodes, hipMemcpyDeviceToHost,
                           c->stream));
    HIP_TRY(hipStreamSynchronize(c->stream));
    return DPG_OK;
}

int dpg_gn_assemble(dpg_ctx* c, double* hb_dev) {
    DPG_STEP_API_1(c);
    if (!hb_dev) hb_dev = c->gn.v.hb_own;
    HIP_TRY(hipEventRecord(c->ev[3].e, c->stream));
    int rc = dpg_gn_dev_assemble(&c->gn.v, hb_dev, c->stream);
    if (rc) return fail(rc, "assembly launch failed");
    HIP_TRY(hipEventRecord(c->ev[4].e, c->stream));
    return DPG_OK;
}

int dpg_gn_solve_retract(dpg_ctx* c, const double* hb_dev, double* delta_inf, double* error, int32_t* pcg_iters) {
    DPG_STEP_API_1(c);
    if (!hb_dev) hb_dev = c->gn.v.hb_own;
    int rc = dpg_gn_dev_solve(&c->gn.v, hb_dev, &c->gp, c->stream, delta_inf, error, pcg_iters);
    if (rc) return fail(rc, "PCG solve failed: %s", hipGetErrorString(hipGetLastError()));
    HIP_TRY(hipEventRecord(c->ev[5].e, c->stream));
    float a = 0.f, s = 0.f;
    if (hipEventSynchronize(c->ev[5].e) == hipSuccess) {
        (void)hipEventElapsedTime(&a, c->ev[3].e, c->ev[4].e);
        (void)hipEventElapsedTime(&s, c->ev[4].e, c->ev[5].e);
    }
    c->asm_ms = a;
    c->solve_ms = s;
    return DPG_OK;
}

int dpg_gn_solve_retract_async(dpg_ctx* c, const double* hb_dev) {
    DPG_STEP_API_1(c);
    return solve_retract_async_1(c, hb_dev);
}

int32_t dpg_gn_factorizations(dpg_ctx* c) { return (c && c->gn_ready) ? c->gn.v.n_factorizations : -1; }

int dpg_gn_fetch(dpg_ctx* c, const double* hb_dev, double out[3]) {
    DPG_STEP_API_1(c);
    if (!out) return fail(DPG_ERR_ARG, "dpg_gn_fetch: out is NULL");
    return fetch_1(c, hb_dev, out);
}

float dpg_gn_last_assemble_ms(dpg_ctx* c) { return c ? c->asm_ms : -1.f; }
float dpg_gn_last_solve_ms(dpg_ctx* c) { return c ? c->solve_ms : -1.f; }

int dpg_gn_run(dpg_ctx* c, double* poses_out, dpg_gn_stats* st) {
    if (!c || !c->gn_ready) return fail(DPG_ERR_STATE, "dpg_gn_run: graph not set up");
    HIP_TRY(hipSetDevice(c->device));
    const double t0 = now_ms();
    return gn_loop(c, c->gp, poses_out, t0, t0, st);
}

int dpg_optimize_graph(dpg_ctx* c, double* poses, int64_t V, const dpg_factor* F, int64_t nf, const dpg_gn_params* gp,
                       dpg_gn_stats* st) {
    const double t0 = now_ms();
    const dpg_gn_params P = or_default(gp, dpg_gn_params_default);
    if (!c || !F || !poses || V <= 0 || nf < 0) return fail(DPG_ERR_ARG, "dpg_optimize_graph: bad arguments");
    int rc = dpg_gn_setup(c, V, F, nf, 0, nf, &P);
    if (rc) return rc;
    if ((rc = dpg_gn_set_poses(c, poses))) return rc;
    return gn_loop(c, P, poses, t0, now_ms(), st);
}

int dpg_gn_marginals(dpg_ctx* c, const int32_t* nodes, int64_t n, double* cov_out) {
    if (c && c->gn_ready && !nodes && n != c->gn.v.n_nodes)
        return fail(DPG_ERR_ARG, "dpg_gn_marginals: nodes == NULL asks for every node (n = %lld)", (long long)c->gn.v.n_nodes);
    return gn_marginals_blocks(c, "dpg_gn_marginals", nodes, n, nullptr, 0, cov_out, nullptr);
}

int dpg_gn_marginal_pairs(dpg_ctx* c, const int32_t* pairs, int64_t n, double* cov_out) {
    if (n > 0 && !pairs) return fail(DPG_ERR_ARG, "dpg_gn_marginal_pairs: pairs is NULL");
    int rc = gn_marginals_state(c, "dpg_gn_marginal_pairs");
    if (rc) return rc;
    if (n < 0 || !cov_out) return fail(DPG_ERR_ARG, "dpg_gn_marginal_pairs: bad arguments");
    if ((rc = gn_pairs_share_factor(c, pairs, n))) return rc;
    return gn_marginals_blocks(c, "dpg_gn_marginal_pairs", nullptr, 0, pairs, n, cov_out, nullptr);
}

int dpg_gn_cross_covariances(dpg_ctx* c, const int32_t* pairs, int64_t n, double* cov_out) {
    return gn_joint_blocks(c, "dpg_gn_cross_covariances", 0, pairs, n, cov_out, nullptr);
}

int dpg_gn_joint_marginal(dpg_ctx* c, const int32_t* nodes, int64_t n, double* cov_out) {
    return gn_joint_blocks(c, "dpg_gn_joint_marginal", 1, nodes, n, cov_out, nullptr);
}

int dpg_gn_relative_covariances(dpg_ctx* c, const int32_t* pairs, int64_t n, double* cov_out) {
    const char* fn = "dpg_gn_relative_covariances";
    int rc = gn_marginals_state(c, fn);
    if (rc) return rc;
    if (n < 0 || (n > 0 && (!pairs || !cov_out))) return fail(DPG_ERR_ARG, "%s: bad arguments", fn);
    if (n == 0) return DPG_OK;
    for (int64_t q = 0; q < 2 * n; ++q)
        if (pairs[q] < 0 || pairs[q] >= c->gn.v.n_nodes) return fail(DPG_ERR_ARG, "%s: node %d is out of range", fn, pairs[q]);
    std::vector<int32_t> tri((size_t)(6 * n));
    dpg_relative_triples(pairs, n, tri.data());
    std::vector<double> blocks((size_t)(27 * n)), X((size_t)(3 * c->gn.v.n_nodes));
    if ((rc = gn_joint_blocks(c, fn, 0, tri.data(), 3 * n, blocks.data(), nullptr))) return rc;
    if ((rc = dpg_gn_get_poses(c, X.data()))) return rc;
    dpg_relative_from_blocks(pairs, n, X.data(), blocks.data(), cov_out);
    return DPG_OK;
}

int dpg_gn_joint_profile(dpg_ctx* c, const int32_t* pairs, int64_t n, double* out, int64_t cap) {
    if (!out || cap < 4 || n <= 0) return fail(DPG_ERR_ARG, "dpg_gn_joint_profile: bad arguments");
    std::vector<double> cov((size_t)(9 * n));
    float ms[2] = {0.f, 0.f};
    const int rc = gn_joint_blocks(c, "dpg_gn_joint_profile", 0, pairs, n, cov.data(), ms);
    if (rc) return rc;
    int64_t st[2];
    dpg_chol_path_stats(c->gn.v.chol, st);
    out[0] = ms[0];
    out[1] = ms[1];
    out[2] = (double)st[0];
    out[3] = (double)st[1];
    return DPG_OK;
}

int dpg_marginal_covariances(dpg_ctx* c, const double* poses, int64_t V, const dpg_factor* F, int64_t nf,
                             const int32_t* nodes, int64_t n, double* cov_out) {
    if (!c || !F || !poses || !cov_out || V <= 0 || nf < 0 || n < 0 || (!nodes && n != V))
        return fail(DPG_ERR_ARG, "dpg_marginal_covariances: bad arguments");
    if (is_multi(c)) return fail(DPG_ERR_STATE, "dpg_marginal_covariances: marginals are single-device");
    for (int64_t q = 0; nodes && q < n; ++q)
        if (nodes[q] < 0 || nodes[q] >= V) return fail(DPG_ERR_ARG, "dpg_marginal_covariances: node %lld out of range", (long long)q);
    int rc = dpg_gn_setup(c, V, F, nf, 0, nf, nullptr);
    if (rc) return rc;
    if ((rc = dpg_gn_set_poses(c, poses))) return rc;
    return dpg_gn_marginals(c, nodes, n, cov_out);
}

int64_t dpg_gn_marginals_profile(dpg_ctx* c, double* out, int64_t cap) {
    int rc = gn_marginals_state(c, "dpg_gn_marginals_profile");
    if (rc) return rc;
    if (!out || cap < 4) return fail(DPG_ERR_ARG, "dpg_gn_marginals_profile: bad arguments");
    std::vector<double> cov((size_t)(9 * c->gn.v.n_nodes));
    double ms[2];
    if ((rc = gn_marginals_blocks(c, "dpg_gn_marginals_profile", nullptr, c->gn.v.n_nodes, nullptr, 0, cov.data(), ms)))
        return rc;
    double st[6];
    dpg_chol_stats(c->gn.v.chol, st);
    const int nl = (int)st[1];
    std::vector<float> lv((size_t)nl, 0.f);
    if ((rc = dpg_chol_selinv_timed(c->gn.v.chol, c->stream, lv.data(), nl))) return fail(rc, "selected inversion failed");
    out[0] = ms[0];
    out[1] = ms[1];
    out[2] = nl;
    out[3] = (double)dpg_chol_selinv_bytes(c->gn.v.chol);
    int64_t k = 4;
    for (int q = 0; q < nl && k < cap; ++q) out[k++] = lv[(size_t)q];
    return k;
}

}
```

dpg-slam_amd/csrc/dpg_internal.h:

```cpp
#ifndef DPG_INTERNAL_H
#define DPG_INTERNAL_H

#include <stdint.h>

#include "../../include/dpg_slam_c.h"

#ifdef __cplusplus
extern "C" {
#endif

int dpg_set_error(int code, const char* msg);
dpg_ctx* dpg_inc_ctx(dpg_inc* g);
int dpg_inc_prepare(dpg_inc* g, int64_t n_new, const int32_t* pairs, int64_t n_pairs);
int dpg_inc_abort_prepare(dpg_inc* g);
int dpg_scans_export(dpg_ctx* c, int64_t* n_nodes, int32_t* ratio, int64_t* off, float* pts);
int dpg_scans_index_all(dpg_ctx* c);
void dpg_ctx_adopt(dpg_ctx* c, void* child, void (*destroy)(void*));
void dpg_ctx_release_child(dpg_ctx* c, void* child);
int dpg_launch_host_wait(const uint32_t* flag, uint32_t tag, uint32_t* timed_out, void* stream);

typedef struct dpg_icp_edge {
    int32_t src_ds_off, n_src_ds;
    int32_t tgt_ds_off, n_tgt_ds;
    int32_t src_full_off, n_src_full;
    int32_t tgt_full_off, n_tgt_full;
    float guess[6];
    int32_t src_node, tgt_node;
    int32_t pad[2];
} dpg_icp_edge;

typedef struct dpg_icp_kparams {
    double r2;
    double eps;
    double rot_thr;
    double mse_abs;
    float r2_f;
    float h_min;
    int32_t max_iter;
    int32_t min_corr;
    int32_t reciprocal;
    int32_t cells_max;
    int32_t lds_tgt;
    int32_t trace_iters;
    int32_t trace_stride;
    int32_t defer_cap;
    int32_t kernel_variant;
} dpg_icp_kparams;

int dpg_launch_icp(const float* ds_pts_dev, const dpg_icp_edge* edges_dev, int64_t n_edges,
                   const dpg_icp_kparams* kp, int32_t max_points, dpg_icp_result* results_dev,
                   int32_t* trace_dev, void* stream);
int dpg_launch_cov(const float* full_pts_dev, const dpg_icp_edge* edges_dev, int64_t n_edges,
                   const dpg_icp_result* results_dev, double* hess_dev, int32_t max_workgroups, void* stream);
size_t dpg_icp_lds_bytes(int32_t lds_tgt, int32_t cells_max);
int dpg_launch_cov6(const float* pts_dev, int32_t n_data, int32_t n_model, const float* T6_dev, double* out_dev,
                    void* stream);
__attribute__((visibility("hidden"))) int dpg_cov6_from_sums(const double* sm, int64_t nh, int64_t nb, double cov6[36]);
int dpg_launch_kdtree_build(const float* ds_pts_dev, const int64_t* ds_off_dev, int64_t n_nodes,
                            int32_t max_points, float* tree_pts_dev, uint16_t* tree_idx_dev, void* stream);
int dpg_launch_icp_kd(const float* ds_pts_dev, const float* tree_pts_dev, const uint16_t* tree_idx_dev,
                      const dpg_icp_edge* edges_dev, int64_t n_edges, const dpg_icp_kparams* kp,
                      int32_t max_points, dpg_icp_result* results_dev, int32_t* trace_dev, void* stream);
size_t dpg_icp_kd_lds_bytes(int32_t cap);
int32_t dpg_angle_buckets(void);
int dpg_launch_lc_count(const float* poses_dev, const int32_t* pass_dev, int64_t V, float within, float across,
                        int32_t* count_dev, void* stream);
int dpg_launch_lc_write(const float* poses_dev, const int32_t* pass_dev, int64_t V, float within, float across,
                        const int64_t* off_dev, int32_t* pairs_dev, void* stream);
int dpg_launch_map_points(const float* pts_dev, const int64_t* off_dev, const float* frames_dev, int64_t V,
                          int32_t fraction, float* out_dev, void* stream);
int dpg_launch_angle_index(const float* ds_pts_dev, const int64_t* ds_off_dev, int64_t n_nodes,
                           int32_t max_points, float* idx_pts_dev, uint16_t* idx_orig_dev,
                           uint16_t* buckets_dev, int32_t bitonic, void* stream);
int dpg_launch_icp_ang(const float* ds_pts_dev, const float* idx_pts_dev, const uint16_t* idx_orig_dev,
                       const uint16_t* buckets_dev, const dpg_icp_edge* edges_dev, int64_t n_edges,
                       const dpg_icp_kparams* kp, int32_t max_points, dpg_icp_result* results_dev,
                       int32_t* trace_dev, void* scratch, size_t scratch_bytes, void* stream);
size_t dpg_icp_ang_lds_bytes(int32_t cap);
size_t dpg_icp_ang_scratch_per_edge(int32_t cap);

typedef struct dpg_csm_pair {
    int32_t tgt_off, n_tgt;
    int32_t src_off, n_src;
    float tx, ty;
    int32_t pad[2];
} dpg_csm_pair;

typedef struct dpg_gn_dev {
    int64_t n_nodes, n_factors, nnzb_upper, nnzb_full;
    int64_t shard_begin, shard_end;
    dpg_factor* factors;
    int32_t* up_cptr;
    int32_t* up_clist;
    int32_t* rowptr;
    int32_t* colidx;
    int32_t* src_up;
    double* bsr;
    double* minv;
    double* poses;
    double* x, *r, *z, *p0, *p1, *q;
    double* partials;
    double* scal;
    double* hb_own;
    void* chol;
    double* scal3;
    double* scal3_host;
    int32_t n_blocks_rows;
    int32_t last_pcg_iters;
    int32_t last_used_chol;
    double last_delta_inf;
    double prev_delta_inf;
    int32_t have_factor;
    int32_t last_was_chord;
    int32_t n_factorizations;
    uint8_t* mine;
    double* hb_part;
    int32_t world, rank;
    int32_t n_vote;
    double setup_ms[5];
} dpg_gn_dev;

struct dpg_chol_opts;
int dpg_chol_create(void** chol, int64_t n, const int32_t* pair_lo, const int32_t* pair_hi, int64_t n_pairs,
                    const struct dpg_chol_opts* opts);
void dpg_chol_destroy(void* chol);
int dpg_chol_solve(void* chol, const double* hb, void* stream);
int dpg_chol_resolve(void* chol, const double* hb, void* stream);
void dpg_chol_keep_inverse(void* chol, int on);
void dpg_chol_track_factor(void* chol, int on);
void dpg_chol_forget_factor(void* chol);
int dpg_chol_solve_partial(void* chol, const double* hb, const int32_t* dirty_nodes, int64_t n_dirty, void* stream);
void dpg_chol_partial_stats(void* chol, int64_t out[4]);
const int32_t* dpg_chol_pos_dev(void* chol);
const double* dpg_chol_x_dev(void* chol);
const int32_t* dpg_chol_status_dev(void* chol);
void dpg_chol_stats(void* chol, double out[6]);
int dpg_chol_selinv(void* chol, void* stream);
int dpg_chol_selinv_timed(void* chol, void* stream, float* level_ms, int cap);
int dpg_chol_selinv_check(void* chol, const int32_t* nodes, int64_t n, const int32_t* pairs, int64_t n_pairs);
int dpg_chol_selinv_gather(void* chol, const int32_t* nodes, int64_t n, const int32_t* pairs, int64_t n_pairs,
                           double* out_dev, void* stream);
int dpg_chol_marginals(void* chol, const int32_t* nodes, int64_t n, const int32_t* pairs, int64_t n_pairs,
                       double* host_out, void* stream);
int64_t dpg_chol_selinv_bytes(void* chol);
int dpg_chol_joint(void* chol, int by_nodes, const int32_t* idx, int64_t n, double* host_out, void* stream, float* ms);
void dpg_chol_path_stats(void* chol, int64_t out[2]);
void dpg_relative_covariance(const double xi[3], const double xj[3], const double* Sii, const double* Sij,
                             const double* Sjj, double out[9]);
void dpg_relative_triples(const int32_t* pairs, int64_t n, int32_t* tri);
void dpg_relative_from_blocks(const int32_t* pairs, int64_t n, const double* X, const double* blocks, double* out);

__attribute__((visibility("hidden"))) void dpg_contribution_lists(const dpg_factor* factors, int64_t n_factors, int64_t n,
                                                                  const int32_t* pair, int64_t n_pairs, int32_t* cptr,
                                                                  int32_t* clist);
int64_t dpg_gn_dev_hb_size(const dpg_gn_dev* g);
int64_t dpg_gn_dev_vote_offset(const dpg_gn_dev* g);
int dpg_gn_dev_assemble(dpg_gn_dev* g, double* hb_dev, void* stream);
int dpg_gn_dev_solve_async(dpg_gn_dev* g, const double* hb_dev, const dpg_gn_params* gp, void* stream);
int dpg_gn_dev_fetch(dpg_gn_dev* g, const double* hb_dev, void* stream, double out[3]);
int dpg_gn_dev_solve(dpg_gn_dev* g, const double* hb_dev, const dpg_gn_params* gp, void* stream,
                     double* delta_inf, double* error, int32_t* pcg_iters);
int dpg_gn_dev_icp_to_factors(dpg_gn_dev* g, const dpg_icp_result* results_dev, int64_t first,
                              int64_t count, int64_t n_always, double info_x, double info_y,
                              double info_th, void* stream);
struct GnGraph;
int dpg_gn_dev_set_ownership(struct GnGraph* g, int32_t world, int32_t rank, void* stream);
int dpg_gn_dev_icp_to_factors_scatter(dpg_gn_dev* g, const dpg_icp_result* results_dev, const int32_t* idx_dev,
                                      int64_t n_local, int64_t first, int64_t count, int64_t n_always, double info_x,
                                      double info_y, double info_th, void* stream);
int dpg_gn_dev_assemble_part(dpg_gn_dev* g, const int32_t* gate, void* stream);
int dpg_launch_vsum(const double* const* parts, double* const* outs, int32_t k, int64_t n, void* stream);

#ifdef __cplusplus
}
#endif
#endif
```

dpg-slam_amd/dpgslam/_abi.py:

```python
from __future__ import annotations

import ctypes as C
import os

import numpy as np

_HERE = os.path.dirname(os.path.abspath(__file__))
LIB_PATH = os.environ.get("DPGSLAM_LIB") or os.path.join(os.path.dirname(_HERE), "lib", "libdpg.so")

DPG_OK = 0
DPG_FACTOR_PRIOR = 0
DPG_FACTOR_BETWEEN = 1
DPG_ICP_OK = 0
DPG_ICP_TOO_FEW_CORR = 1
DPG_ICP_LANES = 512


class IcpParams(C.Structure):

    _fields_ = [
        ("icp_maximum_iterations", C.c_int32),
        ("icp_use_reciprocal_correspondences", C.c_int32),
        ("icp_maximum_transformation_epsilon", C.c_double),
        ("icp_max_correspondence_distance", C.c_double),
# ... 19 lines not shown
        ("fitness", C.c_double),
    ]


class Factor(C.Structure):
    _fields_ = [
        ("kind", C.c_int32),
        ("i", C.c_int32),
        ("j", C.c_int32),
        ("pad", C.c_int32),
        ("z", C.c_double * 3),
        ("info", C.c_double * 3),
    ]


class GnParams(C.Structure):
    _fields_ = [
        ("max_iterations", C.c_int32),
        ("use_error_criteria", C.c_int32),
        ("delta_tol", C.c_double),
        ("relative_error_tol", C.c_double),
        ("absolute_error_tol", C.c_double),
        ("pcg_rel_tol", C.c_double),
        ("pcg_max_iterations", C.c_int32),
        ("pcg_check_every", C.c_int32),
        ("linear_solver", C.c_int32),
        ("reuse_factorization", C.c_int32),
        ("refactor_delta", C.c_double),
    ]


DPG_SOLVER_CHOLESKY = 0
DPG_SOLVER_PCG = 1


class GnStats(C.Structure):
    _fields_ = [
        ("iterations", C.c_int32),
        ("pcg_iterations", C.c_int32),
        ("initial_error", C.c_double),
        ("final_error", C.c_double),
        ("last_delta_inf", C.c_double),
        ("ms_total", C.c_double),
        ("ms_per_iteration", C.c_double),
    ]


class ReoptParams(C.Structure):
    _fields_ = [
        ("max_node_dist_within_pass", C.c_float),
        ("max_node_dist_across_passes", C.c_float),
        ("new_pass_std_dev", C.c_float * 3),
        ("motion_model", C.c_float * 4),
        ("odometry_constraints", C.c_int32),
    ]


class ReoptStats(C.Structure):
    _fields_ = [
        ("n_factors", C.c_int64),
        ("n_icp_edges", C.c_int64),
        ("n_candidates", C.c_int64),
        ("n_loop_closures", C.c_int64),
        ("ms_candidates", C.c_double),
        ("ms_icp", C.c_double),
        ("ms_gn", C.c_double),
        ("gn", GnStats),
    ]


DPG_INC_ISAM2 = 0
DPG_INC_BATCH = 1


class IncParams(C.Structure):

    _fields_ = [
        ("mode", C.c_int32),
        ("relinearize_skip", C.c_int32),
        ("relinearize_threshold", C.c_double),
        ("duplicate_factors", C.c_int32),
        ("reorder_every", C.c_int32),
        ("reorder_lead", C.c_int32),
        ("full_refactor", C.c_int32),
        ("gn", GnParams),
    ]


class SolverOptions(C.Structure):

    _fields_ = [(n, C.c_int32) for n in ("order", "fused", "solve_stage", "solve_maxseg", "solve_dinv",
                                          "merge_single", "max_supernode_cols", "solve_inv_cols")] + [("relax_fraction", C.c_double)]


class IncStats(C.Structure):
    _fields_ = [
        ("n_nodes", C.c_int64),
        ("n_factors", C.c_int64),
        ("nnz_l", C.c_int64),
        ("reordered", C.c_int32),
        ("relinearized", C.c_int32),
        ("gn_iterations", C.c_int32),
        ("fronts_kept", C.c_int32),
        ("error", C.c_double),
        ("last_delta_inf", C.c_double),
        ("ms_total", C.c_double),
        ("ms_symbolic", C.c_double),
        ("ms_numeric", C.c_double),
    ]


class AddNodeStats(C.Structure):
    _fields_ = [
        ("n_icp_edges", C.c_int64),
        ("n_loop_closures", C.c_int64),
        ("ms_icp", C.c_double),
        ("update", IncStats),
    ]


RESULT_DTYPE = np.dtype(
    [("T", "<f4", (6,)), ("z", "<f4", (3,)), ("converged", "<i4"), ("iterations", "<i4"),
     ("n_corr", "<i4"), ("status", "<i4"), ("pad", "<i4"), ("fitness", "<f8")], align=True)
FACTOR_DTYPE = np.dtype(
    [("kind", "<i4"), ("i", "<i4"), ("j", "<i4"), ("pad", "<i4"), ("z", "<f8", (3,)),
     ("info", "<f8", (3,))], align=True)
assert RESULT_DTYPE.itemsize == C.sizeof(IcpResult) == 64
assert FACTOR_DTYPE.itemsize == C.sizeof(Factor) == 64

P = C.c_void_p
F32P = C.POINTER(C.c_float)
F64P = C.POINTER(C.c_double)
I32P = C.POINTER(C.c_int32)
I64P = C.POINTER(C.c_int64)
U8P = C.POINTER(C.c_uint8)
I8P = C.POINTER(C.c_int8)


class ChangeParams(C.Structure):

    _fields_ = [
        ("num_sectors", C.c_int32),
        ("current_pose_chain_len", C.c_int32),
        ("num_bins_for_change_detection", C.c_int32),
        ("pad", C.c_int32),
        ("delta_change_threshold", C.c_double),
        ("current_pose_graph_coverage_threshold", C.c_double),
        ("occ_grid_resolution", C.c_double),
        ("minimum_percent_active_sectors", C.c_float),
        ("distance_threshold_for_local_submap_nodes", C.c_float),
        ("laser", C.c_float * 3),
        ("pad2", C.c_float),
    ]


class ChangeStats(C.Structure):

    _fields_ = [(n, C.c_int64) for n in (
        "n_chain", "n_candidates", "n_submap_nodes", "n_chain_cells", "n_uncovered", "n_added", "n_removed",
        "n_committed", "n_sectors_deactivated", "n_nodes_deactivated", "grid_cells", "n_samples")] + [
        ("ms_total", C.c_double), ("ms_kernels", C.c_double)]

    COUNTERS = ("n_chain", "n_candidates", "n_submap_nodes", "n_chain_cells", "n_uncovered", "n_added",
                "n_removed", "n_committed", "n_sectors_deactivated", "n_nodes_deactivated")

    def counters(self) -> dict:
        return {k: int(getattr(self, k)) for k in self.COUNTERS}


class GridParams(C.Structure):

    _fields_ = [("resolution", C.c_double), ("max_cells", C.c_int64), ("margin_cells", C.c_int32), ("pad", C.c_int32)]


class GridInfo(C.Structure):

    _fields_ = [(n, C.c_int32) for n in ("x0", "y0", "w", "h")] + [("resolution", C.c_double)] + [
        (n, C.c_int64) for n in ("n_nodes_used", "n_beams_used", "n_hits", "n_samples", "n_oob")] + [
        ("ms_total", C.c_double), ("ms_kernels", C.c_double), ("n_direct", C.c_int64), ("n_flushed", C.c_int64)]

    def as_dict(self) -> dict:
        return {n: getattr(self, n) for n, _ in self._fields_}


class CsmParams(C.Structure):

    _fields_ = [("resolution", C.c_float), ("sigma", C.c_float), ("kernel_radius", C.c_int32),
                ("half_cells", C.c_int32), ("half_x", C.c_int32), ("half_y", C.c_int32), ("half_a", C.c_int32),
                ("angle_step", C.c_float)]


class CsmResult(C.Structure):

    _fields_ = [("guess", C.c_float * 6), ("score", C.c_int32), ("score_at_guess", C.c_int32), ("n_src", C.c_int32),
                ("best_a", C.c_int32), ("best_dx", C.c_int32), ("best_dy", C.c_int32), ("status", C.c_int32),
                ("pad", C.c_int32 * 3)]


CSM_RESULT_DTYPE = np.dtype(
    [("guess", "<f4", (6,)), ("score", "<i4"), ("score_at_guess", "<i4"), ("n_src", "<i4"), ("best_a", "<i4"),
     ("best_dx", "<i4"), ("best_dy", "<i4"), ("status", "<i4"), ("pad", "<i4", (3,))], align=True)
assert CSM_RESULT_DTYPE.itemsize == C.sizeof(CsmResult) == 64 and C.sizeof(CsmParams) == 32
DPG_CSM_OK = 0
DPG_CSM_NO_OVERLAP = 1


class LocParams(C.Structure):

    _fields_ = [("resolution", C.c_double), ("max_cells", C.c_int64), ("margin_cells", C.c_int32), ("sigma", C.c_float),
                ("kernel_radius", C.c_int32), ("occupied_min", C.c_int32), ("half_x", C.c_int32), ("half_y", C.c_int32),
                ("half_a", C.c_int32), ("angle_step", C.c_float), ("coarse_shift", C.c_int32),
                ("max_refine_blocks", C.c_int32)]


class LocResult(C.Structure):

    _fields_ = [("pose", C.c_float * 3), ("rot", C.c_float * 2), ("score", C.c_int32), ("score_at_guess", C.c_int32),
                ("n_pts", C.c_int32), ("best_a", C.c_int32), ("best_dx", C.c_int32), ("best_dy", C.c_int32),
                ("status", C.c_int32), ("n_seeds", C.c_int32), ("box", C.c_int32 * 4), ("pad", C.c_int32),
                ("n_blocks", C.c_int64), ("n_frontier", C.c_int64), ("n_refined_candidates", C.c_int64),
                ("ms_kernels", C.c_double), ("ms_field", C.c_double), ("ms_bound", C.c_double), ("ms_fine", C.c_double)]


LOC_RESULT_DTYPE = np.dtype(
    [("pose", "<f4", (3,)), ("rot", "<f4", (2,)), ("score", "<i4"), ("score_at_guess", "<i4"), ("n_pts", "<i4"),
     ("best_a", "<i4"), ("best_dx", "<i4"), ("best_dy", "<i4"), ("status", "<i4"), ("n_seeds", "<i4"),
     ("box", "<i4", (4,)), ("pad", "<i4"), ("n_blocks", "<i8"), ("n_frontier", "<i8"), ("n_refined_candidates", "<i8"),
     ("ms_kernels", "<f8"), ("ms_field", "<f8"), ("ms_bound", "<f8"), ("ms_fine", "<f8")], align=True)
assert LOC_RESULT_DTYPE.itemsize == C.sizeof(LocResult) == 128 and C.sizeof(LocParams) == 56
LOC_RESULT_EXACT = tuple(n for n in LOC_RESULT_DTYPE.names if not n.startswith("ms_"))
DPG_LOC_OK = 0
DPG_LOC_NO_OVERLAP = 1
DPG_LOC_UNPROVEN = 2


ALLREDUCE_F64 = C.CFUNCTYPE(C.c_int, C.c_void_p, C.POINTER(C.c_double), C.c_int64)
ALLREDUCE_F32 = C.CFUNCTYPE(C.c_int, C.c_void_p, C.POINTER(C.c_float), C.c_int64)
ALLGATHER = C.CFUNCTYPE(C.c_int, C.c_void_p, C.c_void_p, C.c_void_p, C.c_int64)


class CollOps(C.Structure):

    _fields_ = [("user", C.c_void_p), ("allreduce_sum_f64", ALLREDUCE_F64), ("allreduce_sum_f32", ALLREDUCE_F32),
                ("allgather", ALLGATHER)]


SIGNATURES = {
    "dpg_last_error": (C.c_char_p, []),
    "dpg_version": (C.c_char_p, []),
    "dpg_icp_params_default": (None, [C.POINTER(IcpParams)]),
    "dpg_gn_params_default": (None, [C.POINTER(GnParams)]),
    "dpg_ctx_create": (P, [C.c_int]),
    "dpg_ctx_create_multi": (P, [C.c_int32, I32P]),
    "dpg_ctx_num_gpus": (C.c_int32, [P]),
    "dpg_ctx_create_virtual": (P, [C.c_int32, C.c_int32]),
    "dpg_ctx_create_rank": (P, [C.c_int32, P, C.c_int32, C.c_int32]),
    "dpg_ctx_create_rank_ops": (P, [C.c_int32, C.POINTER(CollOps), C.c_int32, C.c_int32]),
    "dpg_shard_plan": (C.c_int, [F32P, C.c_int64, C.c_int32, I32P, I64P, I64P]),
    "dpg_shard_reassemble": (C.c_int, [I32P, C.c_int64, C.c_int32, C.c_int64, C.c_int64, P, P]),
    "dpg_nccl_unique_id": (C.c_int, [P]),
    "dpg_ctx_num_ranks": (C.c_int32, [P]),
    "dpg_ctx_rank": (C.c_int32, [P]),
    "dpg_ctx_set_icp_schedule": (C.c_int, [P, C.c_int32]),
    "dpg_solver_options_default": (None, [C.POINTER(SolverOptions)]),
    "dpg_ctx_set_solver_options": (C.c_int, [P, C.POINTER(SolverOptions)]),
    "dpg_ctx_destroy": (None, [P]),
    "dpg_ctx_set_stream": (C.c_int, [P, P]),
    "dpg_ctx_synchronize": (C.c_int, [P]),
    "dpg_scan_to_cloud": (C.c_int64, [F32P, C.c_int64, C.c_float, C.c_float, C.c_float, C.c_float,
                                      C.c_float, C.c_float, F32P]),
    "dpg_scans_to_clouds": (C.c_int64, [F32P, C.c_int64, C.c_int64, C.c_float, C.c_float, C.c_float,
                                        C.c_float, C.c_float, C.c_float, F32P, I64P]),
    "dpg_downsample_cloud": (C.c_int64, [F32P, C.c_int64, C.c_int32, F32P]),
    "dpg_inverse_transform_point": (None, [F32P, F32P, F32P]),
    "dpg_transform_point": (None, [F32P, F32P, F32P]),
    "dpg_icp_guess": (None, [F32P, F32P, F32P]),
    "dpg_odometry_factors": (C.c_int, [F32P, C.c_int64, I32P, I32P, C.c_int64, C.c_float, C.c_float, C.c_float,
                                      C.c_float, C.c_void_p]),
    "dpg_odometry_factor": (C.c_int, [F32P, F32P, C.c_int32, C.c_int32, C.c_float, C.c_float, C.c_float,
                                      C.c_float, C.POINTER(Factor)]),
    "dpg_icp_factor": (None, [C.POINTER(IcpResult), C.c_int32, C.c_int32, C.POINTER(IcpParams),
                              C.POINTER(Factor)]),
    "dpg_synth_world": (C.c_int64, [C.c_uint64, C.c_float, F32P, C.c_int64]),
    "dpg_synth_trajectory": (C.c_int, [C.c_uint64, C.c_int64, F32P, C.c_int64, C.c_float, C.c_float, F64P]),
    "dpg_synth_scans": (C.c_int, [F64P, C.c_int64, F32P, C.c_int64, C.c_int32, C.c_float, C.c_float,
                                  C.c_float, C.c_float, C.c_float, C.c_float, C.c_float, C.c_uint64,
                                  C.c_int32, F32P]),
    "dpg_run_icp": (C.c_int, [P, F32P, C.c_int64, F32P, C.c_int64, F32P, F32P, C.POINTER(IcpParams),
                              C.POINTER(IcpResult), F64P, F64P]),
    "dpg_scans_upload": (C.c_int, [P, F32P, I64P, C.c_int64, C.c_int32]),
    "dpg_icp_batch_prepare": (C.c_int, [P, I32P, C.c_int64, F32P, C.POINTER(IcpParams)]),
    "dpg_icp_batch_run": (C.c_int, [P, C.c_int32, C.c_int32]),
    "dpg_icp_batch_fetch": (C.c_int, [P, P, F64P, C.c_int64]),
    "dpg_icp_batch_fetch_trace": (C.c_int, [P, I32P, C.c_int64, I64P]),
    "dpg_icp_batch_size": (C.c_int64, [P]),
    "dpg_icp_batch_kernel_ms": (C.c_float, [P]),
    "dpg_cov_batch_kernel_ms": (C.c_float, [P]),
    "dpg_cov_batch_overlapped": (C.c_int32, [P]),
    "dpg_kdtree_build_ms": (C.c_float, [P]),
    "dpg_ctx_set_icp_variant": (C.c_int, [P, C.c_int32]),
    "dpg_ctx_set_icp_defer_cap": (C.c_int, [P, C.c_int32]),
    "dpg_ctx_set_cov_workgroups": (C.c_int, [P, C.c_int32]),
    "dpg_ctx_set_icp_kernel_variant": (C.c_int, [P, C.c_int32]),
    "dpg_icp_batch_algorithmic_bytes": (C.c_double, [P]),
    "dpg_optimize_graph": (C.c_int, [P, F64P, C.c_int64, P, C.c_int64, C.POINTER(GnParams),
                                     C.POINTER(GnStats)]),
    "dpg_gn_setup": (C.c_int, [P, C.c_int64, P, C.c_int64, C.c_int64, C.c_int64, C.POINTER(GnParams)]),
    "dpg_gn_take_icp_measurements": (C.c_int, [P, C.c_int64, C.c_int64, C.c_int64, C.POINTER(IcpParams)]),
    "dpg_gn_hb_size": (C.c_int64, [P]),
    "dpg_gn_setup_profile": (C.c_int, [P, F64P]),
    "dpg_gn_set_poses": (C.c_int, [P, F64P]),
    "dpg_gn_get_poses": (C.c_int, [P, F64P]),
    "dpg_gn_assemble": (C.c_int, [P, P]),
    "dpg_gn_solve_retract": (C.c_int, [P, P, F64P, F64P, I32P]),
    "dpg_gn_solve_retract_async": (C.c_int, [P, P]),
    "dpg_gn_fetch": (C.c_int, [P, P, F64P]),
    "dpg_gn_factorizations": (C.c_int32, [P]),
    "dpg_gn_run": (C.c_int, [P, F64P, C.POINTER(GnStats)]),
    "dpg_gn_last_assemble_ms": (C.c_float, [P]),
    "dpg_gn_last_solve_ms": (C.c_float, [P]),
    "dpg_gn_marginals": (C.c_int, [P, I32P, C.c_int64, F64P]),
    "dpg_gn_marginal_pairs": (C.c_int, [P, I32P, C.c_int64, F64P]),
    "dpg_gn_cross_covariances": (C.c_int, [P, I32P, C.c_int64, F64P]),
    "dpg_gn_joint_marginal": (C.c_int, [P, I32P, C.c_int64, F64P]),
    "dpg_gn_relative_covariances": (C.c_int, [P, I32P, C.c_int64, F64P]),
    "dpg_gn_joint_profile": (C.c_int, [P, I32P, C.c_int64, F64P, C.c_int64]),
    "dpg_marginal_covariances": (C.c_int, [P, F64P, C.c_int64, P, C.c_int64, I32P, C.c_int64, F64P]),
    "dpg_gn_marginals_profile": (C.c_int64, [P, F64P, C.c_int64]),
    "icp_cov_calculate": (C.c_int, [P, F32P, C.c_int64, F32P, C.c_int64, F32P, C.c_float, C.c_float,
                                    C.c_float, F64P, F64P]),
    "icp_cov_sandwich": (C.c_int, [P, F32P, C.c_int64, F32P, C.c_int64, F32P, F64P, F64P]),
    "dpg_reopt_params_default": (None, [C.POINTER(ReoptParams)]),
    "dpg_get_map": (C.c_int64, [P, F32P, C.c_int32, F32P, C.c_int64]),
    "dpg_get_map_kernel_ms": (C.c_float, [P]),
    "dpg_loop_closure_candidates": (C.c_int64, [P, C.c_int64, I32P, F32P, C.c_float, C.c_float, I32P, C.c_int64]),
    "dpg_change_params_default": (None, [C.POINTER(ChangeParams)]),
    "dpg_dpg_create": (P, [P, C.c_int64, I64P, F32P, F32P, C.POINTER(ChangeParams)]),
    "dpg_dpg_destroy": (None, [P]),
    "dpg_dpg_append": (C.c_int, [P, C.c_int64, I64P, F32P, F32P]),
    "dpg_execute_dpg": (C.c_int, [P, C.c_int64, C.c_int64, F32P, C.POINTER(ChangeStats)]),
    "dpg_execute_dpg_chain": (C.c_int, [P, C.c_int64, C.c_int64, F32P, F32P, C.POINTER(ChangeStats)]),
    "dpg_dpg_fetch": (C.c_int, [P, U8P, U8P, U8P]),
    "dpg_dpg_load": (C.c_int, [P, U8P, U8P, U8P]),
    "dpg_active_dynamic_points": (C.c_int64, [P, C.c_int64, F32P, F32P, C.c_int64, I64P]),
    "dpg_grid_params_default": (None, [C.POINTER(GridParams)]),
    "dpg_occupancy_grid": (C.c_int, [P, C.c_int64, F32P, C.POINTER(GridParams), I32P, I32P, I8P, C.c_int64,
                                     C.POINTER(GridInfo)]),
    "dpg_dpg_beam_geometry": (C.c_int, [P, C.c_int64, F32P, F32P, F32P, C.c_int64]),
    "dpg_occupancy_from_counts": (None, [I32P, I32P, C.c_int64, I8P]),
    "dpg_grid_box": (C.c_int, [F32P, F32P, U8P, C.c_int64, C.c_double, C.c_int32, I32P]),
    "dpg_csm_params_default": (None, [C.POINTER(CsmParams)]),
    "dpg_csm_lds_bytes": (C.c_int64, [C.POINTER(CsmParams)]),
    "dpg_csm_lut": (C.c_int, [C.POINTER(CsmParams), U8P]),
    "dpg_csm_rotations": (C.c_int, [F32P, C.POINTER(CsmParams), F32P]),
    "dpg_csm_batch": (C.c_int, [P, I32P, C.c_int64, F32P, F32P, C.POINTER(CsmParams), P, C.c_int64]),
    "dpg_csm_table": (C.c_int, [P, C.c_int32, C.POINTER(CsmParams), U8P, C.c_int64]),
    "dpg_csm_scores": (C.c_int, [P, C.c_int32, C.c_int32, F32P, C.POINTER(CsmParams), I32P, C.c_int64]),
    "dpg_csm_kernel_ms": (C.c_float, [P]),
    "dpg_icp_batch_prepare_guess": (C.c_int, [P, I32P, C.c_int64, F32P, C.POINTER(IcpParams)]),
    "dpg_loc_params_default": (None, [C.POINTER(LocParams)]),
    "dpg_loc_params_check": (C.c_int, [C.POINTER(LocParams)]),
    "dpg_loc_rotations": (C.c_int, [C.c_float, C.POINTER(LocParams), F32P]),
    "dpg_map_localize": (C.c_int, [P, C.c_int64, F32P, F32P, C.c_int64, F32P, C.POINTER(LocParams),
                                   C.POINTER(LocResult)]),
    "dpg_map_field": (C.c_int, [P, C.c_int64, F32P, C.POINTER(LocParams), C.c_int32, U8P, C.c_int64, I32P]),
    "dpg_map_localize_bounds": (C.c_int, [P, C.c_int64, F32P, F32P, C.c_int64, F32P, C.POINTER(LocParams), I32P,
                                          C.c_int64]),
    "dpg_map_localize_scores": (C.c_int, [P, C.c_int64, F32P, F32P, C.c_int64, F32P, C.POINTER(LocParams), I32P,
                                          C.c_int64]),
    "dpg_reoptimize": (C.c_int, [P, C.c_int64, I32P, F32P, F32P, C.POINTER(IcpParams), C.POINTER(GnParams),
                                 C.POINTER(ReoptParams), F64P, C.POINTER(ReoptStats)]),
    "dpg_reoptimize_inc": (C.c_int, [P, C.c_int64, I32P, F32P, F32P, C.POINTER(IcpParams), C.POINTER(ReoptParams),
                                     F64P, C.POINTER(ReoptStats)]),
    "dpg_inc_params_default": (None, [C.POINTER(IncParams)]),
    "dpg_inc_create": (P, [P, C.POINTER(IncParams)]),
    "dpg_inc_destroy": (None, [P]),
    "dpg_inc_reset": (C.c_int, [P]),
    "dpg_inc_update": (C.c_int, [P, C.c_int64, F64P, P, C.c_int64, C.POINTER(IncStats)]),
    "dpg_inc_num_nodes": (C.c_int64, [P]),
    "dpg_inc_get_poses": (C.c_int, [P, F64P, C.c_int64]),
    "dpg_inc_marginals": (C.c_int, [P, I32P, C.c_int64, F64P]),
    "dpg_inc_cross_covariances": (C.c_int, [P, I32P, C.c_int64, F64P]),
    "dpg_inc_joint_marginal": (C.c_int, [P, I32P, C.c_int64, F64P]),
    "dpg_inc_relative_covariances": (C.c_int, [P, I32P, C.c_int64, F64P]),
    "dpg_inc_save": (C.c_int, [P, C.c_char_p]),
    "dpg_inc_load": (P, [P, C.c_char_p]),
    "dpg_inc_export": (C.c_int64, [P, I64P, P, I32P, C.c_int64, F64P, F64P, F64P]),
    "dpg_scans_append": (C.c_int, [P, F32P, I64P, C.c_int64, C.c_int32]),
    "dpg_add_node": (C.c_int, [P, F32P, C.c_int64, I32P, F32P, P, C.c_int64, C.POINTER(IcpParams),
                               C.POINTER(ReoptParams), C.c_int32, C.POINTER(AddNodeStats)]),
    "dpg_add_node_pairs": (C.c_int, [P, F32P, C.c_int64, F32P, P, C.c_int64, I32P, C.c_int64, C.c_int32,
                                     C.POINTER(IcpParams), C.POINTER(AddNodeStats)]),
}


def default_inc_params() -> IncParams:
    p = IncParams()
    lib().dpg_inc_params_default(C.byref(p))
    return p


def default_solver_options() -> SolverOptions:
    o = SolverOptions()
    lib().dpg_solver_options_default(C.byref(o))
    return o


def default_reopt_params() -> ReoptParams:
    p = ReoptParams()
    lib().dpg_reopt_params_default(C.byref(p))
    return p

_LIB = None


def lib() -> C.CDLL:
    global _LIB
    if _LIB is None:
        if not os.path.exists(LIB_PATH):
            raise RuntimeError(f"{LIB_PATH} is not built; run `make -C dpg-slam_amd` or __graft_entry__.build()")
        try:
            import torch
        except ImportError:
            pass
        L = C.CDLL(LIB_PATH)
        for name, (res, args) in SIGNATURES.items():
            fn = getattr(L, name)
            fn.restype = res
            fn.argtypes = args
        _LIB = L
    return _LIB


def ptr(a: np.ndarray, ctype):
    if a is None:
        return None
    assert a.flags["C_CONTIGUOUS"], "array must be C-contiguous"
    return a.ctypes.data_as(C.POINTER(ctype))


def vptr(a: np.ndarray):
    if a is None:
        return None
    assert a.flags["C_CONTIGUOUS"]
    return C.c_void_p(a.ctypes.data)


class DpgError(RuntimeError):
    pass


def check(rc: int, what: str = "dpg call"):
    if rc != DPG_OK:
        msg = lib().dpg_last_error()
        raise DpgError(f"{what} failed ({rc}): {msg.decode() if msg else ''}")


def default_icp_params() -> IcpParams:
    p = IcpParams()
    lib().dpg_icp_params_default(C.byref(p))
    return p


def default_change_params() -> ChangeParams:
    p = ChangeParams()
    lib().dpg_change_params_default(C.byref(p))
    return p


default_change_params_host = default_change_params


def default_grid_params() -> GridParams:
    p = GridParams()
    lib().dpg_grid_params_default(C.byref(p))
    return p


def default_csm_params() -> CsmParams:
    p = CsmParams()
    lib().dpg_csm_params_default(C.byref(p))
    return p


def default_loc_params() -> LocParams:
    p = LocParams()
    lib().dpg_loc_params_default(C.byref(p))
    return p


def default_gn_params() -> GnParams:
    p = GnParams()
    lib().dpg_gn_params_default(C.byref(p))
    return p
```

dpg-slam_amd/dpgslam/api.py:

```python
from __future__ import annotations

import ctypes as C
import os
import weakref
from dataclasses import dataclass

import numpy as np

from . import _abi
from ._abi import (FACTOR_DTYPE, RESULT_DTYPE, F32P, F64P, I32P, I64P, check, lib, ptr, vptr)


@dataclass
class Node:

    pose: np.ndarray
    cloud: np.ndarray


def _f32(a) -> np.ndarray:
    return np.ascontiguousarray(np.asarray(a, dtype=np.float32))


def _f64(a) -> np.ndarray:
    return np.ascontiguousarray(np.asarray(a, dtype=np.float64))


def _node_list(nodes, what="nodes"):
    if nodes is None:
        return None
    a = np.asarray(nodes)
    if a.ndim != 1 or (a.size and not np.issubdtype(a.dtype, np.integer)):
        raise ValueError(f"{what}: expected a 1-D sequence of node indices, got shape {a.shape} dtype {a.dtype}")
    return np.ascontiguousarray(a, np.int32)


def _pair_list(pairs):
    a = np.asarray(pairs)
    if a.ndim != 2 or a.shape[1] != 2 or (a.size and not np.issubdtype(a.dtype, np.integer)):
        raise ValueError(f"pairs: expected integer node pairs of shape [n, 2], got shape {a.shape} dtype {a.dtype}")
    return np.ascontiguousarray(a, np.int32)


def _joint_pairs(name, handle, pairs):
    pr = _pair_list(pairs)
    out = np.empty((len(pr), 3, 3), np.float64)
    check(getattr(lib(), name)(handle, ptr(pr, C.c_int32), len(pr), ptr(out, C.c_double)), name)
    return out


def _joint_nodes(name, handle, nodes):
    nd = _node_list(nodes)
    if nd is None:
        raise ValueError("nodes: expected a 1-D sequence of node indices, got None")
    out = np.empty((3 * len(nd), 3 * len(nd)), np.float64)
    check(getattr(lib(), name)(handle, ptr(nd, C.c_int32), len(nd), ptr(out, C.c_double)), name)
    return out


def scan_to_cloud(ranges, angle_min, angle_max, range_max, laser=(0.2, 0.0, 0.0)) -> np.ndarray:
    r = _f32(ranges)
    out = np.empty((max(r.size, 1), 2), np.float32)
    n = lib().dpg_scan_to_cloud(ptr(r, C.c_float), r.size, angle_min, angle_max, range_max,
                                laser[0], laser[1], laser[2], ptr(out, C.c_float))
    return out[:n].copy()


def scans_to_clouds(ranges, angle_min, angle_max, range_max, laser=(0.2, 0.0, 0.0)):
    r = _f32(ranges)
    V, nb = r.shape
    pts = np.empty((V * nb, 2), np.float32)
    offs = np.empty(V + 1, np.int64)
    tot = lib().dpg_scans_to_clouds(ptr(r, C.c_float), V, nb, angle_min, angle_max, range_max,
                                    laser[0], laser[1], laser[2], ptr(pts, C.c_float), ptr(offs, C.c_int64))
    return pts[:tot].copy(), offs


def downsample(cloud, ratio: int) -> np.ndarray:
    c = _f32(cloud)
    out = np.empty((max(len(c), 1), 2), np.float32)
    n = lib().dpg_downsample_cloud(ptr(c, C.c_float), len(c), ratio, ptr(out, C.c_float))
    return out[:n].copy()


def inverse_transform_point(a, b) -> np.ndarray:
    a, b, o = _f32(a), _f32(b), np.empty(3, np.float32)
    lib().dpg_inverse_transform_point(ptr(a, C.c_float), ptr(b, C.c_float), ptr(o, C.c_float))
    return o


def transform_point(p, frame) -> np.ndarray:
    p, f, o = _f32(p), _f32(frame), np.empty(3, np.float32)
    lib().dpg_transform_point(ptr(p, C.c_float), ptr(f, C.c_float), ptr(o, C.c_float))
    return o


def icp_guess(pose_src, pose_tgt) -> np.ndarray:
    a, b, o = _f32(pose_src), _f32(pose_tgt), np.empty(6, np.float32)
    lib().dpg_icp_guess(ptr(a, C.c_float), ptr(b, C.c_float), ptr(o, C.c_float))
    return o


def csm_lut(params=None) -> np.ndarray:
    p = params or _abi.default_csm_params()
    out = np.zeros(max(int(p.kernel_radius), 0) ** 2 + 1, np.uint8)
    check(lib().dpg_csm_lut(C.byref(p), ptr(out, C.c_uint8)), "dpg_csm_lut")
    return out


def csm_rotations(guess, params=None) -> np.ndarray:
    p = params or _abi.default_csm_params()
    g = _f32(guess).reshape(6)
    out = np.zeros((2 * max(int(p.half_a), 0) + 1, 2), np.float32)
    check(lib().dpg_csm_rotations(ptr(g, C.c_float), C.byref(p), ptr(out, C.c_float)), "dpg_csm_rotations")
    return out


def loc_rotations(guess_theta, params=None) -> np.ndarray:
    p = params or _abi.default_loc_params()
    out = np.zeros((2 * min(max(int(p.half_a), 0), 1024) + 1, 2), np.float32)
    check(lib().dpg_loc_rotations(float(np.float32(guess_theta)), C.byref(p), ptr(out, C.c_float)), "dpg_loc_rotations")
    return out


def loc_params_valid(params) -> bool:
    return lib().dpg_loc_params_check(C.byref(params)) == _abi.DPG_OK


def csm_lds_bytes(params=None) -> int:
    p = params or _abi.default_csm_params()
    n = int(lib().dpg_csm_lds_bytes(C.byref(p)))
    if n < 0:
        raise _abi.DpgError(f"dpg_csm_lds_bytes failed ({n}): invalid parameters or above the LDS budget")
    return n


def odometry_factor(odom_prev, odom_cur, i_prev, i_cur, motion=(0.4, 0.4, 0.4, 0.4)):
    a, b = _f32(odom_prev), _f32(odom_cur)
    f = _abi.Factor()
    rc = lib().dpg_odometry_factor(ptr(a, C.c_float), ptr(b, C.c_float), i_prev, i_cur, *motion, C.byref(f))
    check(rc, "dpg_odometry_factor")
    return f


def odometry_factors(odom: np.ndarray, i_prev, i_cur, motion=(0.4, 0.4, 0.4, 0.4)) -> np.ndarray:
    o = _f32(odom).reshape(-1, 3)
    a = np.ascontiguousarray(i_prev, np.int32)
    b = np.ascontiguousarray(i_cur, np.int32)
    out = np.zeros(len(a), FACTOR_DTYPE)
    if len(a):
        check(lib().dpg_odometry_factors(ptr(o, C.c_float), len(o), ptr(a, C.c_int32), ptr(b, C.c_int32), len(a),
                                         *motion, vptr(out)), "dpg_odometry_factors")
    return out


def prior_factors(nodes, sigmas=(0.2, 0.2, 0.15)) -> np.ndarray:
    n = np.asarray(nodes, np.int32).reshape(-1)
    f = np.zeros(len(n), FACTOR_DTYPE)
    f["kind"] = _abi.DPG_FACTOR_PRIOR
    f["i"] = n
    s = np.asarray(sigmas, np.float32).astype(np.float64)
    f["info"] = 1.0 / (s * s)
    return f


def prior_factor(node: int, pose=(0.0, 0.0, 0.0), sigmas=(0.2, 0.2, 0.15)) -> np.ndarray:
    f = np.zeros(1, FACTOR_DTYPE)
    f["kind"] = _abi.DPG_FACTOR_PRIOR
    f["i"] = node
    f["z"] = pose
    s = np.asarray(sigmas, np.float32).astype(np.float64)
    f["info"] = 1.0 / (s * s)
    return f


def between_factor(i, j, z, sigmas=None, info=None) -> np.ndarray:
    f = np.zeros(1, FACTOR_DTYPE)
    f["kind"] = _abi.DPG_FACTOR_BETWEEN
    f["i"], f["j"], f["z"] = i, j, z
    if info is None:
        s = np.asarray(sigmas, np.float64)
        info = 1.0 / (s * s)
    f["info"] = info
    return f


def calculate_ICP_COV(data_pi, model_qi, transform, laser_x_variance=0.5, laser_y_variance=0.5,
                      laser_theta_variance=0.3, ctx: "Context | None" = None, with_hessian=True):
    d, m = _f32(data_pi).reshape(-1, 2), _f32(model_qi).reshape(-1, 2)
    T = _f32(transform).reshape(4, 4)
    cov = np.zeros(9, np.float64)
    hess = np.zeros(9, np.float64) if with_hessian else None
    rc = lib().icp_cov_calculate(ctx.handle if ctx else None, ptr(d, C.c_float), len(d), ptr(m, C.c_float),
                                 len(m), ptr(T, C.c_float), laser_x_variance, laser_y_variance,
                                 laser_theta_variance, ptr(cov, C.c_double), ptr(hess, C.c_double))
    check(rc, "icp_cov_calculate")
    return cov.reshape(3, 3), (hess.reshape(3, 3) if hess is not None else None)


def icp_cov_sandwich(data_pi, model_qi, transform, ctx: "Context | None" = None):
    d, m = _f32(data_pi).reshape(-1, 2), _f32(model_qi).reshape(-1, 2)
    T = _f32(transform).reshape(4, 4)
    cov6, cov3 = np.zeros(36, np.float64), np.zeros(9, np.float64)
    check(lib().icp_cov_sandwich(ctx.handle if ctx else None, ptr(d, C.c_float), len(d), ptr(m, C.c_float), len(m),
                                 ptr(T, C.c_float), ptr(cov6, C.c_double), ptr(cov3, C.c_double)), "icp_cov_sandwich")
    return cov6.reshape(6, 6), cov3.reshape(3, 3)


def results_array(n: int) -> np.ndarray:
    return np.zeros(n, RESULT_DTYPE)


def shard_plan(n_edges: int, world: int, cost=None):
    owner = np.zeros(max(n_edges, 1), np.int32)
    disp = np.zeros(max(n_edges, 1), np.int64)
    counts = np.zeros(world, np.int64)
    c = None if cost is None else _f32(cost)
    check(lib().dpg_shard_plan(ptr(c, C.c_float) if c is not None else None, n_edges, world, ptr(owner, C.c_int32),
                               ptr(disp, C.c_int64), ptr(counts, C.c_int64)), "dpg_shard_plan")
    return owner[:n_edges], disp[:n_edges], counts


def shard_reassemble(owner: np.ndarray, world: int, slice_: int, gathered: np.ndarray, rec_bytes: int) -> np.ndarray:
    owner = np.ascontiguousarray(owner, np.int32)
    g = np.ascontiguousarray(gathered).view(np.uint8)
    out = np.zeros(len(owner) * rec_bytes, np.uint8)
    check(lib().dpg_shard_reassemble(ptr(owner, C.c_int32), len(owner), world, slice_, rec_bytes, vptr(g), vptr(out)),
          "dpg_shard_reassemble")
    return out


NCCL_ID_BYTES = 128


def nccl_unique_id() -> bytes:
    buf = C.create_string_buffer(NCCL_ID_BYTES)
    check(lib().dpg_nccl_unique_id(C.cast(buf, C.c_void_p)), "dpg_nccl_unique_id")
    return buf.raw


class Context:

    def __init__(self, device: int = 0, n_gpus: int | None = None, virtual: int | None = None,
                 rank: tuple | None = None, rank_ops: tuple | None = None):
        self._coll = None
        if virtual is not None:
            self.handle = lib().dpg_ctx_create_virtual(int(virtual), device)
        elif rank_ops is not None:
            coll, r, w = rank_ops
            self._coll = coll
            self.handle = lib().dpg_ctx_create_rank_ops(device, C.byref(coll.ops), int(r), int(w))
        elif rank is not None:
            nid, r, w = rank
            buf = C.create_string_buffer(bytes(nid), NCCL_ID_BYTES)
            self.handle = lib().dpg_ctx_create_rank(device, C.cast(buf, C.c_void_p), int(r), int(w))
        elif n_gpus is None:
            self.handle = lib().dpg_ctx_create(device)
        else:
            devs = np.arange(device, device + int(n_gpus), dtype=np.int32)
            self.handle = lib().dpg_ctx_create_multi(int(n_gpus), ptr(devs, C.c_int32))
        if not self.handle:
            raise _abi.DpgError("dpg_ctx_create failed: " + (lib().dpg_last_error() or b"").decode())
        self.device = device
        self.n_gpus = int(lib().dpg_ctx_num_gpus(self.handle))
        self.n_ranks = int(lib().dpg_ctx_num_ranks(self.handle))
        self.rank = int(lib().dpg_ctx_rank(self.handle))
        self.n_edges = 0
        self.V = 0
        self._children = weakref.WeakSet()

    def close(self):
        if self.handle:
            for ch in list(getattr(self, "_children", ())):
                ch.close()
            lib().dpg_ctx_destroy(self.handle)
            self.handle = None

    def __enter__(self):
        return self

    def __exit__(self, *a):
        self.close()

    def __del__(self):
        try:
            self.close()
        except Exception:
            pass

    def set_stream(self, stream_handle: int):
        check(lib().dpg_ctx_set_stream(self.handle, C.c_void_p(stream_handle)), "dpg_ctx_set_stream")

    def synchronize(self):
        check(lib().dpg_ctx_synchronize(self.handle), "dpg_ctx_synchronize")

    def set_icp_variant(self, variant: str):
        v = {"angular": 3, "kdtree": 2, "grid": 1}[variant]
        check(lib().dpg_ctx_set_icp_variant(self.handle, v), "dpg_ctx_set_icp_variant")

    def set_icp_defer_cap(self, cap: int):
        check(lib().dpg_ctx_set_icp_defer_cap(self.handle, int(cap)), "dpg_ctx_set_icp_defer_cap")

    def set_cov_workgroups(self, n: int):
        check(lib().dpg_ctx_set_cov_workgroups(self.handle, int(n)), "dpg_ctx_set_cov_workgroups")

    def set_solver_options(self, **kw):
        o = _abi.default_solver_options()
        for k, v in kw.items():
            if k == "order" and isinstance(v, str):
                v = {"auto": 0, "md": 1, "nd": 2}[v]
            setattr(o, k, v)
        check(lib().dpg_ctx_set_solver_options(self.handle, C.byref(o)), "dpg_ctx_set_solver_options")

    def set_icp_schedule(self, schedule: str):
        v = {"caller": 0, "measured": 1}[schedule]
        check(lib().dpg_ctx_set_icp_schedule(self.handle, v), "dpg_ctx_set_icp_schedule")

    def set_icp_kernel_variant(self, v: int):
        check(lib().dpg_ctx_set_icp_kernel_variant(self.handle, int(v)), "dpg_ctx_set_icp_kernel_variant")

    def kdtree_build_ms(self) -> float:
        return float(lib().dpg_kdtree_build_ms(self.handle))

    def run_icp(self, node_1: Node, node_2: Node, params=None, with_hessian=False):
        p = params or _abi.default_icp_params()
        s, t = _f32(node_2.cloud).reshape(-1, 2), _f32(node_1.cloud).reshape(-1, 2)
        ps, pt = _f32(node_2.pose), _f32(node_1.pose)
        res = _abi.IcpResult()
        cov = np.zeros(9, np.float64)
        hess = np.zeros(9, np.float64) if with_hessian else None
        rc = lib().dpg_run_icp(self.handle, ptr(s, C.c_float), len(s), ptr(t, C.c_float), len(t),
                               ptr(ps, C.c_float), ptr(pt, C.c_float), C.byref(p), C.byref(res),
                               ptr(cov, C.c_double), ptr(hess, C.c_double))
        check(rc, "dpg_run_icp")
        ok = bool(res.converged) and res.status == _abi.DPG_ICP_OK
        z = ((float(res.z[0]), float(res.z[1])), float(res.z[2]))
        return ok, z, cov.reshape(3, 3), res, (hess.reshape(3, 3) if hess is not None else None)

    def upload_scans(self, pts: np.ndarray, offsets: np.ndarray, ratio: int = 5):
        pts, offs = _f32(pts).reshape(-1, 2), np.ascontiguousarray(offsets, np.int64)
        check(lib().dpg_scans_upload(self.handle, ptr(pts, C.c_float), ptr(offs, C.c_int64), len(offs) - 1,
                                     ratio), "dpg_scans_upload")
        self.V = len(offs) - 1

    def icp_prepare(self, edges: np.ndarray, poses: np.ndarray, params=None):
        p = params or _abi.default_icp_params()
        e = np.ascontiguousarray(edges, np.int32).reshape(-1, 2)
        ps = _f32(poses).reshape(-1, 3)
        check(lib().dpg_icp_batch_prepare(self.handle, ptr(e, C.c_int32), len(e), ptr(ps, C.c_float), C.byref(p)),
              "dpg_icp_batch_prepare")
        self.n_edges = len(e)

    def icp_run(self, compute_cov=True, trace_iters=0):
        check(lib().dpg_icp_batch_run(self.handle, int(compute_cov), int(trace_iters)), "dpg_icp_batch_run")

    def icp_fetch(self, with_hessian=True):
        n = int(lib().dpg_icp_batch_size(self.handle))
        if n < 0:
            check(n, "dpg_icp_batch_size")
        self.n_edges = n
        res = results_array(n)
        hess = np.zeros((n, 9), np.float64) if with_hessian else None
        check(lib().dpg_icp_batch_fetch(self.handle, vptr(res), ptr(hess, C.c_double), n), "dpg_icp_batch_fetch")
        return res, (hess.reshape(-1, 3, 3) if hess is not None else None)

    def icp_fetch_trace(self, iters: int) -> np.ndarray:
        ms = C.c_int64(0)
        check(lib().dpg_icp_batch_fetch_trace(self.handle, None, 0, C.byref(ms)), "trace size")
        tr = np.empty((self.n_edges, iters, ms.value), np.int32)
        check(lib().dpg_icp_batch_fetch_trace(self.handle, ptr(tr, C.c_int32), tr.size, C.byref(ms)), "trace fetch")
        return tr

    def icp_batch(self, edges, poses, params=None, compute_cov=True, trace_iters=0):
        self.icp_prepare(edges, poses, params)
        self.icp_run(compute_cov, trace_iters)
        return self.icp_fetch(compute_cov)

    def icp_prepare_guess(self, edges: np.ndarray, guesses: np.ndarray, params=None):
        p = params or _abi.default_icp_params()
        e = np.ascontiguousarray(edges, np.int32).reshape(-1, 2)
        g = _f32(guesses).reshape(-1, 6)
        if len(g) != len(e):
            raise ValueError(f"icp_prepare_guess: {len(e)} edges but {len(g)} guesses")
        check(lib().dpg_icp_batch_prepare_guess(self.handle, ptr(e, C.c_int32), len(e), ptr(g, C.c_float), C.byref(p)),
              "dpg_icp_batch_prepare_guess")
        self.n_edges = len(e)

    def icp_batch_guess(self, edges, guesses, params=None, compute_cov=True, trace_iters=0):
        self.icp_prepare_guess(edges, guesses, params)
        self.icp_run(compute_cov, trace_iters)
        return self.icp_fetch(compute_cov)

    def csm_batch(self, edges, poses=None, guesses=None, params=None) -> np.ndarray:
        p = params or _abi.default_csm_params()
        e = np.ascontiguousarray(edges, np.int32).reshape(-1, 2)
        ps = None if poses is None else _f32(poses).reshape(-1, 3)
        g = None if guesses is None else _f32(guesses).reshape(-1, 6)
        if g is not None and len(g) != len(e):
            raise ValueError(f"csm_batch: {len(e)} edges but {len(g)} guesses")
        out = np.zeros(len(e), _abi.CSM_RESULT_DTYPE)
        check(lib().dpg_csm_batch(self.handle, ptr(e, C.c_int32), len(e), ptr(ps, C.c_float), ptr(g, C.c_float),
                                  C.byref(p), vptr(out), len(out)), "dpg_csm_batch")
        return out

    def csm_table(self, node: int, params=None) -> np.ndarray:
        p = params or _abi.default_csm_params()
        w = 2 * max(int(p.half_cells), 0) + 1
        out = np.zeros((w, w), np.uint8)
        check(lib().dpg_csm_table(self.handle, int(node), C.byref(p), ptr(out, C.c_uint8), out.size), "dpg_csm_table")
        return out

    def csm_scores(self, target: int, source: int, guess, params=None) -> np.ndarray:
        p = params or _abi.default_csm_params()
        g = _f32(guess).reshape(6)
        out = np.zeros((2 * max(int(p.half_a), 0) + 1, 2 * max(int(p.half_y), 0) + 1, 2 * max(int(p.half_x), 0) + 1), np.int32)
        check(lib().dpg_csm_scores(self.handle, int(target), int(source), ptr(g, C.c_float), C.byref(p),
                                   ptr(out, C.c_int32), out.size), "dpg_csm_scores")
        return out

    def csm_kernel_ms(self) -> float:
        return float(lib().dpg_csm_kernel_ms(self.handle))

    def icp_kernel_ms(self) -> float:
        return float(lib().dpg_icp_batch_kernel_ms(self.handle))

    def cov_kernel_ms(self) -> float:
        return float(lib().dpg_cov_batch_kernel_ms(self.handle))

    def cov_overlapped(self) -> bool:
        return bool(lib().dpg_cov_batch_overlapped(self.handle))

    def icp_algorithmic_bytes(self) -> float:
        return float(lib().dpg_icp_batch_algorithmic_bytes(self.handle))

    def optimize_graph(self, poses: np.ndarray, factors: np.ndarray, params=None):
        X = _f64(poses).reshape(-1, 3).copy()
        F = np.ascontiguousarray(factors, FACTOR_DTYPE)
        gp = params or _abi.default_gn_params()
        st = _abi.GnStats()
        check(lib().dpg_optimize_graph(self.handle, ptr(X, C.c_double), len(X), vptr(F), len(F), C.byref(gp),
                                       C.byref(st)), "dpg_optimize_graph")
        self._gn_V = len(X)
        return X, st

    def marginals(self, poses: np.ndarray, factors: np.ndarray, nodes=None) -> np.ndarray:
        X = _f64(poses).reshape(-1, 3)
        F = np.ascontiguousarray(factors, FACTOR_DTYPE)
        nd = _node_list(nodes)
        n = len(X) if nd is None else len(nd)
        out = np.empty((n, 3, 3), np.float64)
        check(lib().dpg_marginal_covariances(self.handle, ptr(X, C.c_double), len(X), vptr(F), len(F),
                                             ptr(nd, C.c_int32) if nd is not None else None, n,
                                             ptr(out, C.c_double)), "dpg_marginal_covariances")
        self._gn_V = len(X)
        return out

    def gn_marginals(self, nodes=None) -> np.ndarray:
        nd = _node_list(nodes)
        n = int(getattr(self, "_gn_V", 0) or 0) if nd is None else len(nd)
        out = np.empty((n, 3, 3), np.float64)
        check(lib().dpg_gn_marginals(self.handle, ptr(nd, C.c_int32) if nd is not None else None, n,
                                     ptr(out, C.c_double)), "dpg_gn_marginals")
        return out

    def gn_marginal_pairs(self, pairs) -> np.ndarray:
        pr = _pair_list(pairs)
        out = np.empty((len(pr), 3, 3), np.float64)
        check(lib().dpg_gn_marginal_pairs(self.handle, ptr(pr, C.c_int32), len(pr), ptr(out, C.c_double)),
              "dpg_gn_marginal_pairs")
        return out

    def gn_cross_covariances(self, pairs) -> np.ndarray:
        return _joint_pairs("dpg_gn_cross_covariances", self.handle, pairs)

    def gn_joint_marginal(self, nodes) -> np.ndarray:
        return _joint_nodes("dpg_gn_joint_marginal", self.handle, nodes)

    def gn_relative_covariances(self, pairs) -> np.ndarray:
        return _joint_pairs("dpg_gn_relative_covariances", self.handle, pairs)

    def gn_joint_profile(self, pairs) -> dict:
        pr = _pair_list(pairs)
        out = np.zeros(4, np.float64)
        check(lib().dpg_gn_joint_profile(self.handle, ptr(pr, C.c_int32), len(pr), ptr(out, C.c_double), len(out)),
              "dpg_gn_joint_profile")
        return {"path_ms": float(out[0]), "dot_ms": float(out[1]), "path_fronts": int(out[2]),
                "path_scalars": int(out[3])}

    def gn_marginals_profile(self) -> dict:
        out = np.zeros(4 + 4096, np.float64)
        k = int(lib().dpg_gn_marginals_profile(self.handle, ptr(out, C.c_double), len(out)))
        if k < 0:
            check(k, "dpg_gn_marginals_profile")
        return {"assemble_ms": float(out[0]), "factor_ms": float(out[1]), "levels": int(out[2]),
                "sigma_bytes": int(out[3]), "level_ms": [float(x) for x in out[4:k]]}

    def gn_setup(self, V: int, factors: np.ndarray, shard=(0, None), params=None):
        F = np.ascontiguousarray(factors, FACTOR_DTYPE)
        b, e = shard[0], (len(F) if shard[1] is None else shard[1])
        gp = params or _abi.default_gn_params()
        check(lib().dpg_gn_setup(self.handle, V, vptr(F), len(F), b, e, C.byref(gp)), "dpg_gn_setup")
        self._gn_V = int(V)
        return int(lib().dpg_gn_hb_size(self.handle))

    def gn_take_icp(self, first: int, count: int, n_always: int, params=None):
        p = params or _abi.default_icp_params()
        check(lib().dpg_gn_take_icp_measurements(self.handle, first, count, n_always, C.byref(p)),
              "dpg_gn_take_icp_measurements")

    def gn_set_poses(self, poses):
        X = _f64(poses).reshape(-1, 3)
        check(lib().dpg_gn_set_poses(self.handle, ptr(X, C.c_double)), "dpg_gn_set_poses")

    def gn_setup_profile(self) -> dict:
        out = np.zeros(5, np.float64)
        check(lib().dpg_gn_setup_profile(self.handle, ptr(out, C.c_double)), "dpg_gn_setup_profile")
        return dict(zip(("pattern_lists_bsr", "chol_symbolic", "chol_plan", "wait_alloc_upload", "chol_upload"),
                        (float(x) for x in out)))

    def gn_run(self, V: int | None = None):
        X = np.empty((V, 3), np.float64) if V else None
        st = _abi.GnStats()
        check(lib().dpg_gn_run(self.handle, ptr(X, C.c_double) if X is not None else None, C.byref(st)),
              "dpg_gn_run")
        return {k: getattr(st, k) for k, _ in _abi.GnStats._fields_}, X

    def gn_get_poses(self, V: int) -> np.ndarray:
        X = np.empty((V, 3), np.float64)
        check(lib().dpg_gn_get_poses(self.handle, ptr(X, C.c_double)), "dpg_gn_get_poses")
        return X

    def gn_assemble(self, hb_dev_ptr: int | None = None):
        check(lib().dpg_gn_assemble(self.handle, C.c_void_p(hb_dev_ptr) if hb_dev_ptr else None), "dpg_gn_assemble")

    def gn_solve_retract(self, hb_dev_ptr: int | None = None):
        d, e, it = C.c_double(0), C.c_double(0), C.c_int32(0)
        check(lib().dpg_gn_solve_retract(self.handle, C.c_void_p(hb_dev_ptr) if hb_dev_ptr else None, C.byref(d),
                                         C.byref(e), C.byref(it)), "dpg_gn_solve_retract")
        return d.value, e.value, it.value

    def gn_solve_retract_async(self, hb_dev_ptr: int | None = None):
        check(lib().dpg_gn_solve_retract_async(self.handle, C.c_void_p(hb_dev_ptr) if hb_dev_ptr else None),
              "dpg_gn_solve_retract_async")

    def gn_fetch(self, hb_dev_ptr: int | None = None):
        out = np.zeros(3, np.float64)
        check(lib().dpg_gn_fetch(self.handle, C.c_void_p(hb_dev_ptr) if hb_dev_ptr else None, ptr(out, C.c_double)),
              "dpg_gn_fetch")
        return float(out[0]), float(out[1]), int(out[2])

    def gn_factorizations(self) -> int:
        return int(lib().dpg_gn_factorizations(self.handle))

    def loop_closure_candidates(self, est: np.ndarray, passes: np.ndarray, within: float = 5.0,
                                across: float = 2.0) -> np.ndarray:
        e, ps = _f32(est).reshape(-1, 3), np.ascontiguousarray(passes, np.int32)
        L = lib()
        n = L.dpg_loop_closure_candidates(self.handle, len(e), ptr(ps, C.c_int32), ptr(e, C.c_float), within, across,
                                          None, 0)
        if n < 0:
            check(int(n), "dpg_loop_closure_candidates")
        out = np.zeros((max(n, 1), 2), np.int32)
        n2 = L.dpg_loop_closure_candidates(self.handle, len(e), ptr(ps, C.c_int32), ptr(e, C.c_float), within, across,
                                           ptr(out, C.c_int32), n)
        if n2 < 0:
            check(int(n2), "dpg_loop_closure_candidates")
        return out[:n]

    def get_map(self, est: np.ndarray, display_points_fraction: int = 10) -> np.ndarray:
        e = _f32(est).reshape(-1, 3)
        L = lib()
        n = L.dpg_get_map(self.handle, ptr(e, C.c_float), display_points_fraction, None, 0)
        if n < 0:
            check(int(n), "dpg_get_map")
        out = np.zeros((max(n, 1), 2), np.float32)
        n2 = L.dpg_get_map(self.handle, ptr(e, C.c_float), display_points_fraction, ptr(out, C.c_float), n)
        if n2 < 0:
            check(int(n2), "dpg_get_map")
        return out[:n]

    def get_map_kernel_ms(self) -> float:
        return float(lib().dpg_get_map_kernel_ms(self.handle))

    def reoptimize(self, passes: np.ndarray, est: np.ndarray, odom: np.ndarray, icp_params=None, gn_params=None,
                   reopt_params=None):
        e, o = _f32(est).reshape(-1, 3), _f32(odom).reshape(-1, 3)
        ps = np.ascontiguousarray(passes, np.int32)
        ip = icp_params or _abi.default_icp_params()
        gp = gn_params or _abi.default_gn_params()
        rp = reopt_params or _abi.default_reopt_params()
        X = np.zeros((len(e), 3), np.float64)
        st = _abi.ReoptStats()
        check(lib().dpg_reoptimize(self.handle, len(e), ptr(ps, C.c_int32), ptr(e, C.c_float), ptr(o, C.c_float),
                                   C.byref(ip), C.byref(gp), C.byref(rp), ptr(X, C.c_double), C.byref(st)),
              "dpg_reoptimize")
        self.n_edges = int(st.n_icp_edges)
        return X, st

    def gn_times_ms(self):
        return float(lib().dpg_gn_last_assemble_ms(self.handle)), float(lib().dpg_gn_last_solve_ms(self.handle))


def _ctx_gone(child) -> bool:
    ctx = getattr(child, "ctx", None)
    return ctx is not None and getattr(ctx, "handle", None) is None


class DpgStore:

    def __init__(self, ctx: Context, ranges, geom, offsets=None, params=None):
        r = _f32(ranges)
        if offsets is None:
            V, nb = r.shape
            offsets = np.arange(V + 1, dtype=np.int64) * nb
        off = np.ascontiguousarray(offsets, np.int64)
        self.V = len(off) - 1
        self.B = int(off[-1])
        self.offsets = off.copy()
        g = _f32(geom).reshape(self.V, 3)
        self.params = params or _abi.default_change_params()
        self.ctx = ctx
        self.handle = lib().dpg_dpg_create(ctx.handle, self.V, ptr(off, C.c_int64), ptr(r.reshape(-1), C.c_float),
                                           ptr(g, C.c_float), C.byref(self.params))
# ... 305 lines not shown
```

include/dpg_slam_c.h:

```cpp
#ifndef DPG_SLAM_C_H
#define DPG_SLAM_C_H

#include <stddef.h>
#include <stdint.h>

#ifdef __cplusplus
extern "C" {
#endif

#define DPG_OK 0
#define DPG_ERR_ARG (-1)
#define DPG_ERR_HIP (-2)
#define DPG_ERR_STATE (-3)
#define DPG_ERR_SIZE (-4)
#define DPG_ERR_NUMERIC (-5)
#define DPG_ERR_INTERNAL (-6)

#define DPG_ICP_LANES 512

typedef struct dpg_icp_params {
    int32_t icp_maximum_iterations;
    int32_t icp_use_reciprocal_correspondences;
    double icp_maximum_transformation_epsilon;
    double icp_max_correspondence_distance;
    int32_t ransac_iterations;
    int32_t downsample_icp_points_ratio;
    float laser_x_variance;
    float laser_y_variance;
    float laser_theta_variance;
    int32_t min_number_correspondences;
    double mse_threshold_absolute;
} dpg_icp_params;

typedef struct dpg_icp_result {
    float T[6];
    float z[3];
    int32_t converged;
    int32_t iterations;
    int32_t n_corr;
    int32_t status;
    int32_t pad;
    double fitness;
} dpg_icp_result;

#define DPG_ICP_OK 0
#define DPG_ICP_TOO_FEW_CORR 1
#define DPG_ICP_NON_PLANAR 2
#define DPG_ICP_INTERNAL 3

#define DPG_FACTOR_PRIOR 0
#define DPG_FACTOR_BETWEEN 1
typedef struct dpg_factor {
    int32_t kind;
    int32_t i;
    int32_t j;
    int32_t pad;
    double z[3];
    double info[3];
} dpg_factor;

typedef struct dpg_gn_params {
    int32_t max_iterations;
    int32_t use_error_criteria;
    double delta_tol;
    double relative_error_tol;
    double absolute_error_tol;
    double pcg_rel_tol;
    int32_t pcg_max_iterations;
    int32_t pcg_check_every;
    int32_t linear_solver;
    int32_t reuse_factorization;
    double refactor_delta;
} dpg_gn_params;

#define DPG_SOLVER_CHOLESKY 0
#define DPG_SOLVER_PCG 1

typedef struct dpg_gn_stats {
    int32_t iterations;
    int32_t pcg_iterations;
    double initial_error;
    double final_error;
    double last_delta_inf;
    double ms_total;
    double ms_per_iteration;
} dpg_gn_stats;

typedef struct dpg_ctx dpg_ctx;

const char* dpg_last_error(void);
const char* dpg_version(void);
void dpg_icp_params_default(dpg_icp_params* p);
void dpg_gn_params_default(dpg_gn_params* p);
dpg_ctx* dpg_ctx_create(int device);
void dpg_ctx_destroy(dpg_ctx* ctx);
dpg_ctx* dpg_ctx_create_multi(int32_t n_gpus, const int32_t* devices);
#define DPG_NCCL_ID_BYTES 128
int dpg_nccl_unique_id(void* id_out );
dpg_ctx* dpg_ctx_create_rank(int32_t device, const void* nccl_id, int32_t rank, int32_t world);
typedef struct dpg_coll_ops {
    void* user;
    int (*allreduce_sum_f64)(void* user, double* buf, int64_t n);
    int (*allreduce_sum_f32)(void* user, float* buf, int64_t n);
    int (*allgather)(void* user, const void* send, void* recv, int64_t bytes);
} dpg_coll_ops;
dpg_ctx* dpg_ctx_create_rank_ops(int32_t device, const dpg_coll_ops* ops, int32_t rank, int32_t world);
int dpg_shard_plan(const float* cost, int64_t n_edges, int32_t world, int32_t* owner, int64_t* dispatch,
                   int64_t* counts);
int dpg_shard_reassemble(const int32_t* owner, int64_t n_edges, int32_t world, int64_t slice, int64_t rec_bytes,
                         const void* gathered, void* out);
dpg_ctx* dpg_ctx_create_virtual(int32_t k, int32_t device);
int32_t dpg_ctx_num_gpus(dpg_ctx* ctx);
int32_t dpg_ctx_num_ranks(dpg_ctx* ctx);
int32_t dpg_ctx_rank(dpg_ctx* ctx);
#define DPG_ICP_SCHEDULE_CALLER 0
#define DPG_ICP_SCHEDULE_MEASURED 1
int dpg_ctx_set_icp_schedule(dpg_ctx* ctx, int32_t schedule);
#define DPG_ORDER_AUTO 0
#define DPG_ORDER_MD 1
#define DPG_ORDER_ND 2
typedef struct dpg_solver_options {
    int32_t order;
    int32_t fused;
    int32_t solve_stage;
    int32_t solve_maxseg;
    int32_t solve_dinv;
    int32_t merge_single;
    int32_t max_supernode_cols;
    int32_t solve_inv_cols;
    double relax_fraction;
} dpg_solver_options;
void dpg_solver_options_default(dpg_solver_options* o);
int dpg_ctx_set_solver_options(dpg_ctx* ctx, const dpg_solver_options* o);
int dpg_ctx_set_stream(dpg_ctx* ctx, void* hip_stream);
int dpg_ctx_synchronize(dpg_ctx* ctx);

int64_t dpg_scan_to_cloud(const float* ranges, int64_t n_ranges, float angle_min, float angle_max,
                          float range_max, float laser_x, float laser_y, float laser_theta,
                          float* xy_out);
int64_t dpg_scans_to_clouds(const float* ranges, int64_t n_nodes, int64_t n_beams, float angle_min,
                            float angle_max, float range_max, float laser_x, float laser_y,
                            float laser_theta, float* xy_out, int64_t* offsets_out);
int64_t dpg_downsample_cloud(const float* xy, int64_t n, int32_t ratio, float* xy_out);
void dpg_inverse_transform_point(const float a[3], const float b[3], float out[3]);
void dpg_transform_point(const float p[3], const float frame[3], float out[3]);
void dpg_icp_guess(const float pose_src[3], const float pose_tgt[3], float guess_out[6]);
int dpg_odometry_factor(const float odom_prev[3], const float odom_cur[3], int32_t i_prev, int32_t i_cur,
                        float transl_from_transl, float transl_from_rot, float rot_from_transl,
                        float rot_from_rot, dpg_factor* out);
void dpg_icp_factor(const dpg_icp_result* r, int32_t from_node, int32_t to_node,
                    const dpg_icp_params* p, dpg_factor* out);
int dpg_odometry_factors(const float* odom, int64_t n_odom, const int32_t* i_prev, const int32_t* i_cur, int64_t n,
                         float transl_from_transl, float transl_from_rot, float rot_from_transl, float rot_from_rot,
                         dpg_factor* out);

int64_t dpg_synth_world(uint64_t seed, float world_size, float* segs_out, int64_t max_segs);
int dpg_synth_trajectory(uint64_t seed, int64_t n_nodes, const float* segs, int64_t n_segs,
                         float world_size, float step, double* gt_out );
int dpg_synth_scans(const double* gt, int64_t n_nodes, const float* segs, int64_t n_segs,
                    int32_t n_beams, float angle_min, float angle_max, float range_max,
                    float laser_x, float laser_y, float laser_theta, float noise_sigma,
                    uint64_t seed, int32_t n_threads, float* ranges_out);

int dpg_run_icp(dpg_ctx* ctx, const float* src_xy, int64_t n_src, const float* tgt_xy, int64_t n_tgt,
                const float pose_src[3], const float pose_tgt[3], const dpg_icp_params* params,
                dpg_icp_result* result, double cov_out[9], double hess_out[9]);

int dpg_scans_upload(dpg_ctx* ctx, const float* pts_xy, const int64_t* node_offsets, int64_t n_nodes,
                     int32_t downsample_ratio);
int dpg_icp_batch_prepare(dpg_ctx* ctx, const int32_t* edges, int64_t n_edges, const float* poses,
                          const dpg_icp_params* params);
int dpg_icp_batch_run(dpg_ctx* ctx, int32_t compute_cov, int32_t trace_iters);
int dpg_icp_batch_fetch(dpg_ctx* ctx, dpg_icp_result* results, double* hess , int64_t cap);
int64_t dpg_icp_batch_size(dpg_ctx* ctx);
int dpg_icp_batch_fetch_trace(dpg_ctx* ctx, int32_t* trace , int64_t trace_cap,
                              int64_t* max_src_out);
float dpg_icp_batch_kernel_ms(dpg_ctx* ctx);
float dpg_cov_batch_kernel_ms(dpg_ctx* ctx);
int32_t dpg_cov_batch_overlapped(dpg_ctx* ctx);
float dpg_kdtree_build_ms(dpg_ctx* ctx);
#define DPG_ICP_ANGULAR 3
#define DPG_ICP_KDTREE 2
#define DPG_ICP_GRID 1
int dpg_ctx_set_icp_variant(dpg_ctx* ctx, int32_t variant);
int dpg_ctx_set_icp_defer_cap(dpg_ctx* ctx, int32_t cap);
int dpg_ctx_set_cov_workgroups(dpg_ctx* ctx, int32_t n);
int dpg_ctx_set_icp_kernel_variant(dpg_ctx* ctx, int32_t variant);
double dpg_icp_batch_algorithmic_bytes(dpg_ctx* ctx);

int dpg_optimize_graph(dpg_ctx* ctx, double* poses_inout, int64_t n_nodes, const dpg_factor* factors,
                       int64_t n_factors, const dpg_gn_params* params, dpg_gn_stats* stats);

int dpg_gn_setup(dpg_ctx* ctx, int64_t n_nodes, const dpg_factor* factors, int64_t n_factors,
                 int64_t shard_begin, int64_t shard_end, const dpg_gn_params* params);
int dpg_gn_take_icp_measurements(dpg_ctx* ctx, int64_t first_factor, int64_t count, int64_t n_always,
                                 const dpg_icp_params* params);
int64_t dpg_gn_hb_size(dpg_ctx* ctx);
int dpg_gn_setup_profile(dpg_ctx* ctx, double out[5]);
int dpg_gn_set_poses(dpg_ctx* ctx, const double* poses);
int dpg_gn_get_poses(dpg_ctx* ctx, double* poses);
int dpg_gn_assemble(dpg_ctx* ctx, double* hb_dev);
int dpg_gn_solve_retract(dpg_ctx* ctx, const double* hb_dev, double* delta_inf, double* error,
                         int32_t* pcg_iterations);
int dpg_gn_solve_retract_async(dpg_ctx* ctx, const double* hb_dev);
int dpg_gn_fetch(dpg_ctx* ctx, const double* hb_dev, double out[3]);
int dpg_gn_run(dpg_ctx* ctx, double* poses_out, dpg_gn_stats* stats);
int32_t dpg_gn_factorizations(dpg_ctx* ctx);
float dpg_gn_last_assemble_ms(dpg_ctx* ctx);
float dpg_gn_last_solve_ms(dpg_ctx* ctx);

int dpg_gn_marginals(dpg_ctx* ctx, const int32_t* nodes, int64_t n, double* cov_out );
int dpg_gn_marginal_pairs(dpg_ctx* ctx, const int32_t* pairs , int64_t n, double* cov_out );
int dpg_gn_cross_covariances(dpg_ctx* ctx, const int32_t* pairs , int64_t n, double* cov_out );
int dpg_gn_joint_marginal(dpg_ctx* ctx, const int32_t* nodes, int64_t n, double* cov_out );
int dpg_gn_relative_covariances(dpg_ctx* ctx, const int32_t* pairs , int64_t n, double* cov_out );
int dpg_gn_joint_profile(dpg_ctx* ctx, const int32_t* pairs , int64_t n, double* out, int64_t cap);
int dpg_marginal_covariances(dpg_ctx* ctx, const double* poses, int64_t n_nodes, const dpg_factor* factors,
                             int64_t n_factors, const int32_t* nodes, int64_t n, double* cov_out);
int64_t dpg_gn_marginals_profile(dpg_ctx* ctx, double* out, int64_t cap);

typedef struct dpg_reopt_params {
    float max_node_dist_within_pass;
    float max_node_dist_across_passes;
    float new_pass_std_dev[3];
    float motion_model[4];
    int32_t odometry_constraints;
} dpg_reopt_params;

typedef struct dpg_reopt_stats {
    int64_t n_factors;
    int64_t n_icp_edges;
    int64_t n_candidates;
    int64_t n_loop_closures;
    double ms_candidates;
    double ms_icp;
    double ms_gn;
    dpg_gn_stats gn;
} dpg_reopt_stats;

void dpg_reopt_params_default(dpg_reopt_params* p);

int64_t dpg_loop_closure_candidates(dpg_ctx* ctx, int64_t n_nodes, const int32_t* pass_numbers,
                                    const float* est_poses , float max_dist_within_pass,
                                    float max_dist_across_passes, int32_t* pairs_out , int64_t cap);

int64_t dpg_get_map(dpg_ctx* ctx, const float* est_poses , int32_t display_points_fraction,
                    float* map_out , int64_t cap);
float dpg_get_map_kernel_ms(dpg_ctx* ctx);

int dpg_reoptimize(dpg_ctx* ctx, int64_t n_nodes, const int32_t* pass_numbers, const float* est_poses,
                   const float* odom_only, const dpg_icp_params* icp_params, const dpg_gn_params* gn_params,
                   const dpg_reopt_params* params, double* poses_out, dpg_reopt_stats* stats);

struct dpg_inc;
int dpg_reoptimize_inc(struct dpg_inc* g, int64_t n_nodes, const int32_t* pass_numbers, const float* est_poses,
                       const float* odom_only, const dpg_icp_params* icp_params, const dpg_reopt_params* params,
                       double* poses_out, dpg_reopt_stats* stats);

#define DPG_INC_ISAM2 0
#define DPG_INC_BATCH 1
typedef struct dpg_inc_params {
    int32_t mode;
    int32_t relinearize_skip;
    double relinearize_threshold;
    int32_t duplicate_factors;
    int32_t reorder_every;
    int32_t reorder_lead;
    int32_t full_refactor;
    dpg_gn_params gn;
} dpg_inc_params;

typedef struct dpg_inc_stats {
    int64_t n_nodes, n_factors;
    int64_t nnz_l;
    int32_t reordered;
    int32_t relinearized;
    int32_t gn_iterations;
    int32_t fronts_kept;
    double error;
    double last_delta_inf;
    double ms_total, ms_symbolic, ms_numeric;
} dpg_inc_stats;

typedef struct dpg_inc dpg_inc;
void dpg_inc_params_default(dpg_inc_params* p);
dpg_inc* dpg_inc_create(dpg_ctx* ctx, const dpg_inc_params* params);
void dpg_inc_destroy(dpg_inc* g);
int dpg_inc_reset(dpg_inc* g);
int dpg_inc_update(dpg_inc* g, int64_t n_new, const double* init, const dpg_factor* factors, int64_t n_factors,
                   dpg_inc_stats* stats);
int64_t dpg_inc_num_nodes(const dpg_inc* g);
int dpg_inc_get_poses(dpg_inc* g, double* poses, int64_t n);
int dpg_inc_marginals(dpg_inc* g, const int32_t* nodes, int64_t n, double* cov_out );
int dpg_inc_cross_covariances(dpg_inc* g, const int32_t* pairs , int64_t n, double* cov_out );
int dpg_inc_joint_marginal(dpg_inc* g, const int32_t* nodes, int64_t n, double* cov_out );
int dpg_inc_relative_covariances(dpg_inc* g, const int32_t* pairs , int64_t n, double* cov_out );

int dpg_inc_save(dpg_inc* g, const char* path);
dpg_inc* dpg_inc_load(dpg_ctx* ctx, const char* path);
int64_t dpg_inc_export(dpg_inc* g, int64_t* updates, dpg_factor* factors, int32_t* created, int64_t cap_factors,
                       double* theta, double* est, double* maxd);

int dpg_scans_append(dpg_ctx* ctx, const float* pts_xy, const int64_t* node_offsets, int64_t n_new,
                     int32_t downsample_ratio);

typedef struct dpg_add_node_stats {
    int64_t n_icp_edges;
    int64_t n_loop_closures;
    double ms_icp;
    dpg_inc_stats update;
} dpg_add_node_stats;

int dpg_add_node_pairs(dpg_inc* g, const float* cloud_xy, int64_t n_pts, const float init_pose[3],
                       const dpg_factor* extra, int64_t n_extra, const int32_t* pairs, int64_t n_pairs,
                       int32_t successive, const dpg_icp_params* icp_params, dpg_add_node_stats* stats);
int dpg_add_node(dpg_inc* g, const float* cloud_xy, int64_t n_pts, const int32_t* pass_numbers, const float init_pose[3],
                 const dpg_factor* extra, int64_t n_extra, const dpg_icp_params* icp_params,
                 const dpg_reopt_params* params, int32_t non_successive, dpg_add_node_stats* stats);

enum { DPG_LABEL_STATIC = 0, DPG_LABEL_ADDED = 1, DPG_LABEL_REMOVED = 2, DPG_LABEL_NOT_YET_LABELED = 3,
       DPG_LABEL_MAX_RANGE = 4 };

typedef struct dpg_change_params {
    int32_t num_sectors;
    int32_t current_pose_chain_len;
    int32_t num_bins_for_change_detection;
    int32_t pad;
    double delta_change_threshold;
    double current_pose_graph_coverage_threshold;
    double occ_grid_resolution;
    float minimum_percent_active_sectors;
    float distance_threshold_for_local_submap_nodes;
    float laser[3];
    float pad2;
} dpg_change_params;

typedef struct dpg_change_stats {
    int64_t n_chain;
    int64_t n_candidates;
    int64_t n_submap_nodes;
    int64_t n_chain_cells;
    int64_t n_uncovered;
    int64_t n_added;
    int64_t n_removed;
    int64_t n_committed;
    int64_t n_sectors_deactivated;
    int64_t n_nodes_deactivated;
    int64_t grid_cells;
    int64_t n_samples;
    double ms_total;
    double ms_kernels;
} dpg_change_stats;

typedef struct dpg_dpg dpg_dpg;

void dpg_change_params_default(dpg_change_params* p);
dpg_dpg* dpg_dpg_create(dpg_ctx* ctx, int64_t n_nodes, const int64_t* beam_offsets, const float* ranges,
                        const float* geom , const dpg_change_params* params);
void dpg_dpg_destroy(dpg_dpg* d);
int dpg_dpg_append(dpg_dpg* d, int64_t n_new, const int64_t* beam_offsets, const float* ranges,
                   const float* geom );
int dpg_execute_dpg(dpg_dpg* d, int64_t n_nodes, int64_t current_pass_len, const float* est_poses,
                    dpg_change_stats* stats);
int dpg_execute_dpg_chain(dpg_dpg* d, int64_t n_nodes, int64_t current_pass_len, const float* est_poses,
                          const float* chain_poses, dpg_change_stats* stats);
int dpg_dpg_fetch(dpg_dpg* d, uint8_t* labels, uint8_t* sector_active, uint8_t* node_active);
int dpg_dpg_load(dpg_dpg* d, const uint8_t* labels, const uint8_t* sector_active, const uint8_t* node_active);
int64_t dpg_active_dynamic_points(dpg_dpg* d, int64_t n_nodes, const float* est_poses, float* out,
                                  int64_t cap, int64_t counts[4]);

typedef struct dpg_grid_params {
    double resolution;
    int64_t max_cells;
    int32_t margin_cells;
    int32_t pad;
} dpg_grid_params;

typedef struct dpg_grid_info {
    int32_t x0, y0, w, h;
    double resolution;
    int64_t n_nodes_used;
    int64_t n_beams_used;
    int64_t n_hits;
    int64_t n_samples;
    int64_t n_oob;
    double ms_total, ms_kernels;
    int64_t n_direct;
    int64_t n_flushed;
} dpg_grid_info;

#define DPG_GRID_PARAMS_SIZE 24
#define DPG_GRID_INFO_SIZE 96
#ifdef __cplusplus
 static_assert(sizeof(dpg_grid_params) == DPG_GRID_PARAMS_SIZE && sizeof(dpg_grid_info) == DPG_GRID_INFO_SIZE, "grid ABI structs");
#else
 _Static_assert(sizeof(dpg_grid_params) == DPG_GRID_PARAMS_SIZE && sizeof(dpg_grid_info) == DPG_GRID_INFO_SIZE, "grid ABI structs");
#endif

void dpg_grid_params_default(dpg_grid_params* p);
int dpg_occupancy_grid(dpg_dpg* d, int64_t n_nodes, const float* est_poses, const dpg_grid_params* p,
                       int32_t* hits, int32_t* misses, int8_t* occ, int64_t cap, dpg_grid_info* info);
int dpg_dpg_beam_geometry(dpg_dpg* d, int64_t n_nodes, const float* est_poses, float* lidar_xy, float* end_xy,
                          int64_t cap_beams);
void dpg_occupancy_from_counts(const int32_t* hits, const int32_t* misses, int64_t n, int8_t* occ);
int dpg_grid_box(const float* lidar_xy, const float* r_v, const uint8_t* active, int64_t n, double res,
                 int32_t margin, int32_t box[4]);

typedef struct dpg_csm_params {
    float resolution;
    float sigma;
    int32_t kernel_radius;
    int32_t half_cells;
    int32_t half_x, half_y;
    int32_t half_a;
    float angle_step;
} dpg_csm_params;

#define DPG_CSM_OK 0
#define DPG_CSM_NO_OVERLAP 1
typedef struct dpg_csm_result {
    float guess[6];
    int32_t score;
    int32_t score_at_guess;
    int32_t n_src;
    int32_t best_a, best_dx, best_dy;
    int32_t status;
    int32_t pad[3];
} dpg_csm_result;

#define DPG_CSM_PARAMS_SIZE 32
#define DPG_CSM_RESULT_SIZE 64
#define DPG_CSM_LDS_FIXED 9536
#define DPG_CSM_LDS_BUDGET 163840
#ifdef __cplusplus
 static_assert(sizeof(dpg_csm_params) == DPG_CSM_PARAMS_SIZE && sizeof(dpg_csm_result) == DPG_CSM_RESULT_SIZE, "csm ABI structs");
#else
 _Static_assert(sizeof(dpg_csm_params) == DPG_CSM_PARAMS_SIZE && sizeof(dpg_csm_result) == DPG_CSM_RESULT_SIZE, "csm ABI structs");
#endif

void dpg_csm_params_default(dpg_csm_params* p);
int64_t dpg_csm_lds_bytes(const dpg_csm_params* p);
int dpg_csm_lut(const dpg_csm_params* p, uint8_t* lut_out);
int dpg_csm_rotations(const float guess[6], const dpg_csm_params* p, float* rot_out);
int dpg_csm_batch(dpg_ctx* ctx, const int32_t* edges, int64_t n_edges, const float* poses, const float* guesses,
                  const dpg_csm_params* params, dpg_csm_result* results_out, int64_t cap);
int dpg_csm_table(dpg_ctx* ctx, int32_t node, const dpg_csm_params* params, uint8_t* out, int64_t cap);
int dpg_csm_scores(dpg_ctx* ctx, int32_t target, int32_t source, const float guess[6], const dpg_csm_params* params,
                   int32_t* out, int64_t cap);
float dpg_csm_kernel_ms(dpg_ctx* ctx);
int dpg_icp_batch_prepare_guess(dpg_ctx* ctx, const int32_t* edges, int64_t n_edges, const float* guesses,
                                const dpg_icp_params* params);

typedef struct dpg_loc_params {
    double resolution;
    int64_t max_cells;
    int32_t margin_cells;
    float sigma;
    int32_t kernel_radius;
    int32_t occupied_min;
    int32_t half_x, half_y;
    int32_t half_a;
    float angle_step;
    int32_t coarse_shift;
    int32_t max_refine_blocks;
} dpg_loc_params;

#define DPG_LOC_OK 0
#define DPG_LOC_NO_OVERLAP 1
#define DPG_LOC_UNPROVEN 2
typedef struct dpg_loc_result {
    float pose[3];
    float rot[2];
    int32_t score;
    int32_t score_at_guess;
    int32_t n_pts;
    int32_t best_a, best_dx, best_dy;
    int32_t status;
    int32_t n_seeds;
    int32_t box[4];
    int32_t pad;
    int64_t n_blocks;
    int64_t n_frontier;
    int64_t n_refined_candidates;
    double ms_kernels;
    double ms_field;
    double ms_bound;
    double ms_fine;
} dpg_loc_result;

#define DPG_LOC_PARAMS_SIZE 56
// ... 24 lines not shown
```

Measured before the change: 2.530 million.

## Add register-pipelined TRSM and tiled trailing update paths for fused Cholesky panels

Adds new device routines for the fused supernodal Cholesky. The panel triangular solve becomes a fully unrolled, register-prefetched per-row TRSM, and the next-panel update becomes a register-tiled 2x2 or 2x4 outer-product kernel with double-buffered operand fetches and scheduling barriers. Both are the default (panel_form 0), and a knob can restore the old paths. The aim is to cut LDS latency and raise FMA throughput in the GN factorization, at the cost of higher register pressure. It also adds a spin-timeout that flags status, plus a front-table introspection API.

```diff
diff --git a/dpg-slam_amd/csrc/dpg_chol.h b/dpg-slam_amd/csrc/dpg_chol.h
--- a/dpg-slam_amd/csrc/dpg_chol.h
+++ b/dpg-slam_amd/csrc/dpg_chol.h
@@ -15,6 +15,7 @@
     int32_t solve_maxseg = -1;
     int32_t solve_dinv = 0;
     int32_t solve_inv_cols = 0;
+    int32_t panel_form = 0;
 };
 
 struct dpg_chol_sym {
diff --git a/dpg-slam_amd/csrc/dpg_chol.hip b/dpg-slam_amd/csrc/dpg_chol.hip
--- a/dpg-slam_amd/csrc/dpg_chol.hip
+++ b/dpg-slam_amd/csrc/dpg_chol.hip
@@ -342,6 +342,24 @@
     out[5] = (double)S.n;
 }
 
+extern "C" int64_t dpg_chol_front_table(void* h, int32_t* out, int64_t cap) {
+    const CholDev* c = reinterpret_cast<CholDev*>(h);
+    const int64_t ns = (int64_t)c->plan.sns.size();
+    if (cap < 4) return ns;
+    out[0] = (int32_t)ns;
+    out[1] = c->plan.fused ? 1 : 0;
+    out[2] = c->plan.fused_db ? 1 : 0;
+    out[3] = 0;
+    for (int64_t s = 0; s < ns && 4 * (s + 2) <= cap; ++s) {
+        const SnDev& d = c->plan.sns[(size_t)s];
+        out[4 * (s + 1)] = 3 * (d.k + d.r);
+        out[4 * (s + 1) + 1] = 3 * d.k;
+        out[4 * (s + 1) + 2] = d.nchild;
+        out[4 * (s + 1) + 3] = d.G;
+    }
+    return ns;
+}
+
 #ifdef DPG_CHOL_TIMING
 extern "C" void dpg_chol_tree(void* h, int32_t* parent, int32_t* m3, int32_t* k3) {
     const dpg_chol_sym& S = reinterpret_cast<CholDev*>(h)->sym;
diff --git a/dpg-slam_amd/csrc/dpg_chol_factor.hip b/dpg-slam_amd/csrc/dpg_chol_factor.hip
--- a/dpg-slam_amd/csrc/dpg_chol_factor.hip
+++ b/dpg-slam_amd/csrc/dpg_chol_factor.hip
@@ -1,4 +1,5 @@
 #include "dpg_chol_dev.h"
+#include "dpg_chol_panel.h"
 
 using namespace dpg_chol;
 
@@ -17,6 +18,7 @@
 namespace {
 constexpr int kPF = (kSmall * (kSmall + 1) / 2 + kFT - 1) / kFT;
 constexpr int kPFL = 4;
+constexpr int kOldTrsm = 1, kOldUpd = 2;
 
 __device__ __forceinline__ void tri_ij(int e, int n, int& i, int& j) {
     const float b = 2.0f * (float)n + 1.0f;
@@ -185,8 +187,8 @@
 
 struct Tiles {
     int k3, m3, np, nt;
-    __device__ int c0(int t) const { return t < np ? kFNB * t : k3 + kFNB * (t - np); }
-    __device__ int c1(int t) const { return t < np ? min(kFNB * t + kFNB, k3) : min(k3 + kFNB * (t - np + 1), m3); }
+    __device__ __forceinline__ int c0(int t) const { return t < np ? kFNB * t : k3 + kFNB * (t - np); }
+    __device__ __forceinline__ int c1(int t) const { return t < np ? min(kFNB * t + kFNB, k3) : min(k3 + kFNB * (t - np + 1), m3); }
 };
 
 struct PanelFrame {
@@ -202,7 +204,7 @@
     }
 };
 
-__device__ void factor_lds(int q, int s, const Tiles& T, double* P, double* scr, bool& bad) {
+__device__ __forceinline__ void factor_lds(int q, int s, const Tiles& T, double* P, double* scr, bool& bad, int old, int32_t* status) {
     const int tid = threadIdx.x, lane = tid & 63, wave = __builtin_amdgcn_readfirstlane(tid >> 6);
     const PanelFrame f(T, q);
     const int w = f.w, R = f.R, off = f.off, Rp = f.Rp;
@@ -220,8 +222,14 @@
                 col[r] = (i < w && i >= c) ? P[c * Rp + off + i] : 0.0;
             }
             for (int st = 0; st < wave; ++st) {
-                while (__builtin_amdgcn_readfirstlane(__hip_atomic_load(flg + st, __ATOMIC_RELAXED, __HIP_MEMORY_SCOPE_WORKGROUP)) < ep)
+                unsigned spins = 0;
+                while (__builtin_amdgcn_readfirstlane(__hip_atomic_load(flg + st, __ATOMIC_RELAXED, __HIP_MEMORY_SCOPE_WORKGROUP)) < ep) {
                     __builtin_amdgcn_s_sleep(0);
+                    if (++spins > (1u << 20)) {
+                        if (i == 0) atomicExch(status, 2);
+                        break;
+                    }
+                }
                 __builtin_amdgcn_fence(__ATOMIC_ACQUIRE, "workgroup");
                 const int c0 = 3 * st;
                 const int ii = i < kFNB ? i : 0;
@@ -261,6 +269,13 @@
     }
     __syncthreads();
     PN_MARK(s, q, 6);
+    if (!(old & kOldTrsm)) {
+        trsm_and_copy_thread(tid, P, Rp, off, w, R, Lt, rdg);
+        __syncthreads();
+        PN_MARK(s, q, 7);
+        PN_MARK(s, q, 3);
+        return;
+    }
     for (int i = w + tid; i < R; i += kFT) {
         double a[kFNB];
 #pragma unroll
@@ -292,7 +307,7 @@
     PN_MARK(s, q, 3);
 }
 
-__device__ void publish_panel(int q, int s, const Tiles& T, double* F, const double* P, int32_t* pflag) {
+__device__ __forceinline__ void publish_panel(int q, int s, const Tiles& T, double* F, const double* P, int32_t* pflag) {
     const int tid = threadIdx.x;
     const PanelFrame f(T, q);
     const int R = f.R;
@@ -311,7 +326,7 @@
 }
 
 template <bool SC1>
-__device__ void load_panel(int p, const Tiles& T, double* F, double* P) {
+__device__ __forceinline__ void load_panel(int p, const Tiles& T, double* F, double* P) {
     const int tid = threadIdx.x;
     const PanelFrame f(T, p);
     const int j0 = f.j0, w = f.w, R = f.R, off = f.off, Rp = f.Rp;
@@ -362,7 +377,7 @@
 }
 
 template <bool WT, bool SC1 = false>
-__device__ void update_tile(int t, int p, const Tiles& T, double* F, const double* P) {
+__device__ __forceinline__ void update_tile(int t, int p, const Tiles& T, double* F, const double* P) {
     const int tid = threadIdx.x;
     const PanelFrame f(T, p);
     const int m3 = f.m3, j0 = f.j0, w = f.w, R = f.R, off = f.off, Rp = f.Rp;
@@ -414,8 +429,12 @@
     }
 }
 
-__device__ void update_next_lds(int p, const Tiles& T, const double* Pc, double* Pn) {
+__device__ __forceinline__ void update_next_lds(int p, const Tiles& T, const double* Pc, double* Pn, int old) {
     const int tid = threadIdx.x;
+    if (!(old & kOldUpd) && ((old >> 2) || upd_use_tiles(T.m3 - kFNB * (p + 1), min(kFNB, T.k3 - kFNB * (p + 1))))) {
+        upd_next_thread(tid, p, T.m3, T.k3, Pc, Pn, old >> 2);
+        return;
+    }
     const int j0 = kFNB * p, R = T.m3 - j0, Rp = fused_rp(R, 0);
     const int j1 = j0 + kFNB, w1 = min(kFNB, T.k3 - j1), R1 = R - kFNB;
     const int off1 = (4 - (w1 & 3)) & 3, Rp1 = fused_rp(R1, off1);
@@ -452,7 +471,7 @@
     }
 }
 
-__device__ void rhs_panel(int p, const Tiles& T, const double* P, double* bv) {
+__device__ __forceinline__ void rhs_panel(int p, const Tiles& T, const double* P, double* bv) {
     const int tid = threadIdx.x, lane = tid & 63, wave = tid >> 6;
     const PanelFrame f(T, p);
     const int j0 = f.j0, w = f.w, R = f.R, off = f.off, Rp = f.Rp;
@@ -483,7 +502,7 @@
                             const FTask* __restrict__ ftasks, const FChild* __restrict__ fchild,
                             const double* __restrict__ hb, const double* __restrict__ g,
                             const int32_t* __restrict__ perm, double* fronts, double* __restrict__ ysol,
-                            double* acc, double* sm, int db) {
+                            double* acc, double* sm, int db, int old) {
     const int tid = threadIdx.x;
     const int k3 = 3 * S.k, r3 = 3 * S.r, m3 = k3 + r3, G = S.G;
     double* F = fronts + S.front_off;
@@ -595,7 +614,7 @@
         if (tid < kFNB / 3) reinterpret_cast<int*>(scr + kFNB * kFNB + 8 * (kFNB / 3))[tid] = 0;
         if (!db) load_panel<false>(0, T, F, cur);
         __syncthreads();
-        factor_lds(0, s, T, cur, scr, bad);
+        factor_lds(0, s, T, cur, scr, bad, old, status);
         publish_panel(0, s, T, F, cur, pflag);
         for (int p = 0; p < T.np; ++p) {
             double* nxt = cur == PA ? PB : PA;
@@ -612,7 +631,7 @@
                     load_panel<true>(t, T, F, nxt);
                     __syncthreads();
                     PN_MARK(s, t, 1);
-                    update_next_lds(p, T, cur, nxt);
+                    update_next_lds(p, T, cur, nxt, old);
                 } else {
                     PN_MARK(s, t, 1);
                     update_tile<true, true>(t, p, T, F, cur);
@@ -622,7 +641,7 @@
                 }
                 __syncthreads();
                 PN_MARK(s, t, 2);
-                factor_lds(t, s, T, nxt, scr, bad);
+                factor_lds(t, s, T, nxt, scr, bad, old, status);
                 publish_panel(t, s, T, F, nxt, pflag);
             }
             if (has_b && db) rhs_panel(p, T, cur, bv);
@@ -681,7 +700,7 @@
                                                        const double* __restrict__ hb, const double* __restrict__ g,
                                                        const int32_t* __restrict__ perm, double* fronts,
                                                        double* __restrict__ ysol, double* acc, int ns, int db,
-                                                       const int32_t* gate, const uint8_t* __restrict__ keep) {
+                                                       const int32_t* gate, const uint8_t* __restrict__ keep, int old) {
     extern __shared__ __attribute__((aligned(16))) double smem_f[];
     double* sm = smem_f + 2;
     if (gate_off(gate, 1)) return;
@@ -699,7 +718,7 @@
         small_front(s, S, sync + 1, status, sns, omap, relmap, child_list, hb, g, perm, fronts, ysol, acc, sm);
     else
         large_front(s, mem, S, sync + 1, sync + 1 + ns, sync + 2 + 3 * ns, status, sns, omap, relmap, child_list,
-                    ftasks, fchild, hb, g, perm, fronts, ysol, acc, sm, db);
+                    ftasks, fchild, hb, g, perm, fronts, ysol, acc, sm, db, old);
 }
 
 __global__ __launch_bounds__(256) void chol_copy_runs(const double* __restrict__ src0, const double* __restrict__ src1,
@@ -717,9 +736,11 @@
 
 void dpg_chol::launch_factor(CholDev* c, hipStream_t st, const double* hb, const int32_t* gate, const uint8_t* keep) {
     const CholPlan& P = c->plan;
+    const int form = c->opts.panel_form;
+    const int old = form == 0 ? 0 : form == 1 ? (kOldTrsm | kOldUpd) : form < 6 ? (form - 2) & (kOldTrsm | kOldUpd) : (form - 5) << 2;
     hipLaunchKernelGGL(chol_factor_dag, dim3((unsigned)P.n_tickets), dim3(kFT), P.lds_fused, st, c->order_fac, sync_forward(c),
                        c->status.p, c->sns, c->omap, c->relmap, c->child_list, c->ftasks, c->fchild, hb, hb + 9 * P.nnzb_upper,
-                       c->perm, c->fronts.p, c->ysol.p, c->acc.p, c->sym.ns, P.fused_db ? 1 : 0, gate, keep);
+                       c->perm, c->fronts.p, c->ysol.p, c->acc.p, c->sym.ns, P.fused_db ? 1 : 0, gate, keep, old);
 }
 
 void dpg_chol::launch_copy_runs(CholDev* c, hipStream_t st, const int64_t* gather, const int64_t* scatter, int64_t nruns,
diff --git a/dpg-slam_amd/csrc/dpg_chol_panel.h b/dpg-slam_amd/csrc/dpg_chol_panel.h
--- /dev/null
+++ b/dpg-slam_amd/csrc/dpg_chol_panel.h
@@ -0,0 +1,226 @@
+#ifndef DPG_CHOL_PANEL_H
+#define DPG_CHOL_PANEL_H
+
+#include <math.h>
+
+#include "dpg_chol_plan.h"
+
+namespace dpg_chol {
+
+struct alignas(16) Dbl2 { double x, y; };
+
+#if defined(__HIP_DEVICE_COMPILE__)
+#define DPG_SCHED_FENCE() __builtin_amdgcn_sched_barrier(0)
+#define DPG_PIN(x) asm volatile("" : "+v"(x))
+#else
+#define DPG_SCHED_FENCE() do { } while (0)
+#define DPG_PIN(x) do { } while (0)
+#endif
+#define DPG_INL __attribute__((always_inline)) inline
+
+DPG_HD DPG_INL void trsm_row_any(double* P, int Rp, int off, int w, int i, const double* Lt, const double* rdg) {
+    double a[kFNB];
+#pragma unroll
+    for (int c = 0; c < kFNB; ++c) a[c] = c < w ? P[c * Rp + off + i] : 0.0;
+#pragma unroll
+    for (int b = 0; b < kFNB; b += 3) {
+        if (b < w) {
+            const double* mi = rdg + 2 * b;
+            const double x0 = a[b] * mi[0];
+            const double x1 = fma(a[b], mi[1], a[b + 1] * mi[2]);
+            const double x2 = fma(a[b], mi[3], fma(a[b + 1], mi[4], a[b + 2] * mi[5]));
+            a[b] = x0; a[b + 1] = x1; a[b + 2] = x2;
+#pragma unroll
+            for (int cc = b + 3; cc < kFNB; ++cc)
+                a[cc] = fma(-x2, Lt[(b + 2) * kFNB + cc], fma(-x1, Lt[(b + 1) * kFNB + cc], fma(-x0, Lt[b * kFNB + cc], a[cc])));
+        }
+    }
+#pragma unroll
+    for (int c = 0; c < kFNB; ++c)
+        if (c < w) P[c * Rp + off + i] = a[c];
+}
+
+constexpr int kTC = 3;
+DPG_HD constexpr int trsm_items_before(int b) {
+    int n = 0;
+    for (int q = 0; q < b; q += 3) n += (kFNB - q - 3 + kTC - 1) / kTC;
+    return n;
+}
+template <int B, int C0>
+DPG_HD DPG_INL void trsm_fetch(const double* Lt, double (&L)[3][kTC]) {
+#pragma unroll
+    for (int k = 0; k < kTC; ++k)
+        if (C0 + k < kFNB) {
+            L[0][k] = Lt[B * kFNB + C0 + k];
+            L[1][k] = Lt[(B + 1) * kFNB + C0 + k];
+            L[2][k] = Lt[(B + 2) * kFNB + C0 + k];
+        }
+}
+template <int B, int J>
+DPG_HD DPG_INL void trsm_item(double (&a)[kFNB], double x0, double x1, double x2, const double* Lt, double (&LA)[3][kTC],
+                             double (&LB)[3][kTC]) {
+    constexpr int c0 = B + 3 + kTC * J;
+    if constexpr (c0 < kFNB) {
+        constexpr int par = (trsm_items_before(B) + J) & 1;
+        double (&cur)[3][kTC] = par ? LB : LA;
+        double (&nxt)[3][kTC] = par ? LA : LB;
+        DPG_SCHED_FENCE();
+        if constexpr (c0 + kTC < kFNB) trsm_fetch<B, c0 + kTC>(Lt, nxt);
+        else if constexpr (B + 6 < kFNB) trsm_fetch<B + 3, B + 6>(Lt, nxt);
+#pragma unroll
+        for (int k = 0; k < kTC; ++k)
+            if (c0 + k < kFNB) a[c0 + k] = fma(-x2, cur[2][k], fma(-x1, cur[1][k], fma(-x0, cur[0][k], a[c0 + k])));
+        trsm_item<B, J + 1>(a, x0, x1, x2, Lt, LA, LB);
+    }
+}
+template <int B>
+DPG_HD DPG_INL void trsm_step(double (&a)[kFNB], double (&mi)[6], const double* Lt, const double* rdg, double (&LA)[3][kTC],
+                             double (&LB)[3][kTC]) {
+    if constexpr (B < kFNB) {
+        DPG_SCHED_FENCE();
+        double mn[6];
+#pragma unroll
+        for (int k = 0; k < 6; ++k) mn[k] = B + 3 < kFNB ? rdg[2 * (B + 3) + k] : 0.0;
+        const double x0 = a[B] * mi[0];
+        const double x1 = fma(a[B], mi[1], a[B + 1] * mi[2]);
+        const double x2 = fma(a[B], mi[3], fma(a[B + 1], mi[4], a[B + 2] * mi[5]));
+        a[B] = x0; a[B + 1] = x1; a[B + 2] = x2;
+        trsm_item<B, 0>(a, x0, x1, x2, Lt, LA, LB);
+        trsm_step<B + 3>(a, mn, Lt, rdg, LA, LB);
+    }
+}
+DPG_HD DPG_INL void trsm_row_full(double* P, int Rp, int off, int i, const double* Lt, const double* rdg) {
+    double a[kFNB];
+#pragma unroll
+    for (int c = 0; c < kFNB; ++c) a[c] = P[c * Rp + off + i];
+    double mi[6], LA[3][kTC], LB[3][kTC];
+#pragma unroll
+    for (int k = 0; k < 6; ++k) mi[k] = rdg[k];
+    trsm_fetch<0, 3>(Lt, LA);
+    trsm_step<0>(a, mi, Lt, rdg, LA, LB);
+    DPG_SCHED_FENCE();
+#pragma unroll
+    for (int c = 0; c < kFNB; ++c) P[c * Rp + off + i] = a[c];
+}
+
+DPG_HD inline void trsm_and_copy_thread(int tid, double* P, int Rp, int off, int w, int R, const double* Lt,
+                                        const double* rdg) {
+    if (w == kFNB)
+        for (int i = kFNB + tid; i < R; i += kFT) trsm_row_full(P, Rp, off, i, Lt, rdg);
+    else
+        for (int i = w + tid; i < R; i += kFT) trsm_row_any(P, Rp, off, w, i, Lt, rdg);
+    for (int e = kFT - 1 - tid; e < w * w; e += kFT) {
+        const int c = e / w, r = e - c * w;
+        if (r >= c) P[c * Rp + off + r] = Lt[c * kFNB + r];
+    }
+}
+
+struct UpdShape { int rt, ct; };
+DPG_HD inline int upd_tiles(int R1, int w1, int rt, int ct) { return ((R1 + rt - 1) / rt) * ((w1 + ct - 1) / ct); }
+DPG_HD inline bool upd_use_tiles(int R1, int w1) { return upd_tiles(R1, w1, 2, 4) <= kFT; }
+DPG_HD inline UpdShape upd_shape(int R1, int w1) {
+    return upd_tiles(R1, w1, 2, 2) <= kFT ? UpdShape{2, 2} : UpdShape{2, 4};
+}
+
+template <int RT, int CT, int kG>
+DPG_HD DPG_INL void upd_fetch(const double* col, int Rp, const int (&pi)[RT / 2], const int (&pl)[CT / 2], double (&vi)[kG][RT],
+                              double (&vl)[kG][CT]) {
+#pragma unroll
+    for (int k = 0; k < kG; ++k) {
+        const Dbl2* pc = reinterpret_cast<const Dbl2*>(col + k * Rp);
+#pragma unroll
+        for (int a = 0; a < RT / 2; ++a) {
+            const Dbl2 v = pc[pi[a]];
+            vi[k][2 * a] = v.x;
+            vi[k][2 * a + 1] = v.y;
+        }
+#pragma unroll
+        for (int b = 0; b < CT / 2; ++b) {
+            const Dbl2 v = pc[pl[b]];
+            vl[k][2 * b] = v.x;
+            vl[k][2 * b + 1] = v.y;
+        }
+    }
+}
+template <int RT, int CT, int kG>
+DPG_HD DPG_INL void upd_fmas(const double (&vi)[kG][RT], const double (&vl)[kG][CT], double (&ac)[RT][CT]) {
+#pragma unroll
+    for (int k = 0; k < kG; ++k)
+#pragma unroll
+        for (int a = 0; a < RT; ++a)
+#pragma unroll
+            for (int b = 0; b < CT; ++b) ac[a][b] = fma(vi[k][a], vl[k][b], ac[a][b]);
+}
+
+template <int RT, int CT>
+DPG_HD DPG_INL void upd_next_tile(int q, int nrg, const double* Pc, int Rp, double* Pn, int Rp1, int off1, int w1, int R1) {
+    const int ib = RT * (q % nrg), lb = CT * (q / nrg);
+    if (ib + RT - 1 < lb) return;
+    const int pmax = ((Rp - kFNB) >> 1) - 1;
+    int pi[RT / 2], pl[CT / 2];
+#pragma unroll
+    for (int a = 0; a < RT / 2; ++a) pi[a] = (ib >> 1) + a < pmax ? (ib >> 1) + a : pmax;
+#pragma unroll
+    for (int b = 0; b < CT / 2; ++b) pl[b] = (lb >> 1) + b < pmax ? (lb >> 1) + b : pmax;
+    double ac[RT][CT];
+#pragma unroll
+    for (int a = 0; a < RT; ++a)
+#pragma unroll
+        for (int b = 0; b < CT; ++b) ac[a][b] = 0.0;
+    constexpr int kG = RT * CT >= 16 ? 2 : RT * CT == 8 ? 4 : 6;
+    static_assert(kFNB % kG == 0, "column groups");
+    static_assert((kFNB / kG) % 2 == 0, "pairs of groups");
+    double viA[kG][RT], vlA[kG][CT], viB[kG][RT], vlB[kG][CT];
+    upd_fetch<RT, CT, kG>(Pc + kFNB, Rp, pi, pl, viA, vlA);
+#pragma unroll
+    for (int g = 0; g < kFNB / kG; g += 2) {
+        DPG_SCHED_FENCE();
+        upd_fetch<RT, CT, kG>(Pc + kG * (g + 1) * Rp + kFNB, Rp, pi, pl, viB, vlB);
+        upd_fmas<RT, CT, kG>(viA, vlA, ac);
+        DPG_SCHED_FENCE();
+        if (g + 2 < kFNB / kG) upd_fetch<RT, CT, kG>(Pc + kG * (g + 2) * Rp + kFNB, Rp, pi, pl, viA, vlA);
+        upd_fmas<RT, CT, kG>(viB, vlB, ac);
+    }
+#pragma unroll
+    for (int a = 0; a < RT; ++a)
+#pragma unroll
+        for (int b = 0; b < CT; ++b) DPG_PIN(ac[a][b]);
+    DPG_SCHED_FENCE();
+    double cur[RT][CT];
+#pragma unroll
+    for (int b = 0; b < CT; ++b) {
+        const int l = lb + b < w1 ? lb + b : w1 - 1;
+#pragma unroll
+        for (int a = 0; a < RT; ++a) cur[a][b] = Pn[l * Rp1 + off1 + (ib + a < R1 ? ib + a : R1 - 1)];
+    }
+#pragma unroll
+    for (int a = 0; a < RT; ++a)
+#pragma unroll
+        for (int b = 0; b < CT; ++b) DPG_PIN(cur[a][b]);
+    DPG_SCHED_FENCE();
+#pragma unroll
+    for (int b = 0; b < CT; ++b) {
+        const int l = lb + b;
+#pragma unroll
+        for (int a = 0; a < RT; ++a) {
+            const int i = ib + a;
+            if (l < w1 && i < R1 && i >= l) Pn[l * Rp1 + off1 + i] = cur[a][b] - ac[a][b];
+        }
+    }
+}
+
+DPG_HD inline void upd_next_thread(int tid, int p, int m3, int k3, const double* Pc, double* Pn, int force = 0) {
+    const int j0 = kFNB * p, R = m3 - j0, Rp = fused_rp(R, 0);
+    const int j1 = j0 + kFNB, w1 = k3 - j1 < kFNB ? k3 - j1 : kFNB, R1 = R - kFNB;
+    const int off1 = (4 - (w1 & 3)) & 3, Rp1 = fused_rp(R1, off1);
+    const UpdShape sh = force == 1 ? UpdShape{2, 2} : force == 2 ? UpdShape{2, 4} : upd_shape(R1, w1);
+    const int nrg = (R1 + sh.rt - 1) / sh.rt, nq = nrg * ((w1 + sh.ct - 1) / sh.ct);
+    for (int q = tid; q < nq; q += kFT) {
+        if (sh.rt == 2 && sh.ct == 2) upd_next_tile<2, 2>(q, nrg, Pc, Rp, Pn, Rp1, off1, w1, R1);
+        else upd_next_tile<2, 4>(q, nrg, Pc, Rp, Pn, Rp1, off1, w1, R1);
+    }
+}
+
+}
+
+#endif
diff --git a/dpg-slam_amd/csrc/dpg_ctx.hip b/dpg-slam_amd/csrc/dpg_ctx.hip
--- a/dpg-slam_amd/csrc/dpg_ctx.hip
+++ b/dpg-slam_amd/csrc/dpg_ctx.hip
@@ -282,6 +282,12 @@
     return DPG_OK;
 }
 
+int dpg_ctx_set_chol_panel_form(dpg_ctx* c, int32_t form) {
+    if (!c || form < 0 || form > 7) return fail(DPG_ERR_ARG, "bad panel form");
+    for (int k = 0; k < n_dev(c); ++k) dev_ctx(c, k)->copts.panel_form = form;
+    return DPG_OK;
+}
+
 void dpg_ctx_adopt(dpg_ctx* c, void* child, void (*destroy)(void*)) {
     if (c && child) c->children.emplace_back(child, destroy);
 }
diff --git a/dpg-slam_amd/csrc/dpg_gn_api.hip b/dpg-slam_amd/csrc/dpg_gn_api.hip
--- a/dpg-slam_amd/csrc/dpg_gn_api.hip
+++ b/dpg-slam_amd/csrc/dpg_gn_api.hip
@@ -717,6 +717,13 @@
     return dpg_gn_marginals(c, nodes, n, cov_out);
 }
 
+int64_t dpg_gn_front_table(dpg_ctx* c, int32_t* out, int64_t cap) {
+    if (!c || !c->gn_ready) return fail(DPG_ERR_STATE, "graph not set up");
+    if (!out || cap < 4) return fail(DPG_ERR_ARG, "dpg_gn_front_table: bad arguments");
+    if (!c->gn.v.chol) return fail(DPG_ERR_STATE, "dpg_gn_front_table: the graph has no Cholesky solver");
+    return dpg_chol_front_table(c->gn.v.chol, out, cap);
+}
+
 int64_t dpg_gn_marginals_profile(dpg_ctx* c, double* out, int64_t cap) {
     int rc = gn_marginals_state(c, "dpg_gn_marginals_profile");
     if (rc) return rc;
diff --git a/dpg-slam_amd/csrc/dpg_internal.h b/dpg-slam_amd/csrc/dpg_internal.h
--- a/dpg-slam_amd/csrc/dpg_internal.h
+++ b/dpg-slam_amd/csrc/dpg_internal.h
@@ -135,6 +135,7 @@
 const double* dpg_chol_x_dev(void* chol);
 const int32_t* dpg_chol_status_dev(void* chol);
 void dpg_chol_stats(void* chol, double out[6]);
+int64_t dpg_chol_front_table(void* chol, int32_t* out, int64_t cap);
 int dpg_chol_selinv(void* chol, void* stream);
 int dpg_chol_selinv_timed(void* chol, void* stream, float* level_ms, int cap);
 int dpg_chol_selinv_check(void* chol, const int32_t* nodes, int64_t n, const int32_t* pairs, int64_t n_pairs);
diff --git a/dpg-slam_amd/dpgslam/_abi.py b/dpg-slam_amd/dpgslam/_abi.py
--- a/dpg-slam_amd/dpgslam/_abi.py
+++ b/dpg-slam_amd/dpgslam/_abi.py
@@ -345,6 +345,8 @@
     "dpg_ctx_set_icp_defer_cap": (C.c_int, [P, C.c_int32]),
     "dpg_ctx_set_cov_workgroups": (C.c_int, [P, C.c_int32]),
     "dpg_ctx_set_icp_kernel_variant": (C.c_int, [P, C.c_int32]),
+    "dpg_ctx_set_chol_panel_form": (C.c_int, [P, C.c_int32]),
+    "dpg_gn_front_table": (C.c_int64, [P, I32P, C.c_int64]),
     "dpg_icp_batch_algorithmic_bytes": (C.c_double, [P]),
     "dpg_optimize_graph": (C.c_int, [P, F64P, C.c_int64, P, C.c_int64, C.POINTER(GnParams),
                                      C.POINTER(GnStats)]),
diff --git a/dpg-slam_amd/dpgslam/api.py b/dpg-slam_amd/dpgslam/api.py
--- a/dpg-slam_amd/dpgslam/api.py
+++ b/dpg-slam_amd/dpgslam/api.py
@@ -319,6 +319,18 @@
     def set_icp_kernel_variant(self, v: int):
         check(lib().dpg_ctx_set_icp_kernel_variant(self.handle, int(v)), "dpg_ctx_set_icp_kernel_variant")
 
+    def set_chol_panel_form(self, form: int):
+        check(lib().dpg_ctx_set_chol_panel_form(self.handle, int(form)), "dpg_ctx_set_chol_panel_form")
+
+    def gn_front_table(self) -> dict:
+        head = np.zeros(4, np.int32)
+        ns = int(lib().dpg_gn_front_table(self.handle, ptr(head, C.c_int32), 4))
+        if ns < 0:
+            check(ns, "dpg_gn_front_table")
+        out = np.zeros(4 * (ns + 1), np.int32)
+        check(min(0, int(lib().dpg_gn_front_table(self.handle, ptr(out, C.c_int32), len(out)))), "dpg_gn_front_table")
+        return {"fused": bool(out[1]), "two_buffers": bool(out[2]), "fronts": out[4:].reshape(ns, 4).copy()}
+
     def kdtree_build_ms(self) -> float:
         return float(lib().dpg_kdtree_build_ms(self.handle))
 
diff --git a/include/dpg_slam_c.h b/include/dpg_slam_c.h
--- a/include/dpg_slam_c.h
+++ b/include/dpg_slam_c.h
@@ -186,6 +186,8 @@
 int dpg_ctx_set_icp_defer_cap(dpg_ctx* ctx, int32_t cap);
 int dpg_ctx_set_cov_workgroups(dpg_ctx* ctx, int32_t n);
 int dpg_ctx_set_icp_kernel_variant(dpg_ctx* ctx, int32_t variant);
+int dpg_ctx_set_chol_panel_form(dpg_ctx* ctx, int32_t form);
+int64_t dpg_gn_front_table(dpg_ctx* ctx, int32_t* out, int64_t cap);
 double dpg_icp_batch_algorithmic_bytes(dpg_ctx* ctx);
 
 int dpg_optimize_graph(dpg_ctx* ctx, double* poses_inout, int64_t n_nodes, const dpg_factor* factors,
```

Measured after the change: 2.553 million (median of 4 runs). Within noise of the previous version (+0.9%).
